# Sum02dean/GCN-STRING

Hardware: AMD Instinct MI355X
Metric: graphs/sec (fwd+bwd) on E.coli-sized batches; GCNConv SpMM achieved HBM GB/s (higher is better)
Workload: dtype f32; 1 GPU; config2: E. coli-shaped DisjointLoader batch, B=32 graphs per GPU, F=128, fp32, 2-layer GCNConv(relu)+GlobalSumPool+Dense softmax, CCE (from-logits form of tf.function), SGD; global_graphs=32, nodes_per_gpu=22576, nnz_per_gpu=333676, features=128, hidden=128, parallelism=dp1 (graphs sharded, RCCL all-reduce of 33284 fp32), hip_graph=False, gemm_precision=f32, cce=logits, activation_storage=fp32

## Files before the change

gcn-string_amd/csrc/fused.hip:

```cpp
#include "common.h"

namespace {

typedef float f32x4v __attribute__((ext_vector_type(4)));
typedef float f32x2 __attribute__((ext_vector_type(2)));
typedef __bf16 fbf16x8 __attribute__((ext_vector_type(8)));

constexpr int kFRows = 32;
constexpr int kFCap = 1024;

struct FusedArgs {
  const int32_t* rowptr; const int32_t* colidx; const float* vals;
  const float* x; int64_t ldx;
  int32_t n;
  const float* w; int32_t ldw;
  int32_t nc;
  const float* bias; int act;
  float* s; int64_t lds;
  float* wt_out;
  int w_t;
  float* out; int64_t ldo;
  const int32_t* node_graph; const int32_t* gp; const float* dp; int64_t lddp; int avg;
  const float* mask; int64_t ldmask;
  float* dz2; int64_t lddz2;
  float* colpart;
  float* tp_part; float* tp_cnt;
  const float* hd_part; const float* hd_cnt; int hd_rows; int hd_b;
  float* hd_psum; float* hd_csum;
  const float* hd_w; const float* hd_bias; const float* hd_y; int hd_c; float hd_denom; int hd_fl;
  int dbg;
};

__device__ __forceinline__ float4 fbuf4(__amdgpu_buffer_rsrc_t rs, unsigned off) {
  const f32x4v r = __builtin_bit_cast(f32x4v, __builtin_amdgcn_raw_buffer_load_b128(rs, off, 0, 0));
  return make_float4(r.x, r.y, r.z, r.w);
}
__device__ __forceinline__ float4 f4fma(float v, float4 h, float4 a) {
  const f32x2 w = {v, v};
  const f32x2 lo = __builtin_elementwise_fma(w, f32x2{h.x, h.y}, f32x2{a.x, a.y});
  const f32x2 hi = __builtin_elementwise_fma(w, f32x2{h.z, h.w}, f32x2{a.z, a.w});
  return make_float4(lo[0], lo[1], hi[0], hi[1]);
}
__device__ __forceinline__ float4 f4step(float4 a) {
  const f32x2 big = {0x1p127f, 0x1p127f};
  f32x2 lo = {a.x, a.y}, hi = {a.z, a.w}, t0, t1;
  asm("v_pk_mul_f32 %0, %1, %2" : "=v"(t0) : "v"(lo), "v"(big));
  asm("v_pk_mul_f32 %0, %1, %2" : "=v"(t1) : "v"(hi), "v"(big));
  asm("v_pk_mul_f32 %0, %1, %2 clamp" : "=v"(lo) : "v"(t0), "v"(big));
  asm("v_pk_mul_f32 %0, %1, %2 clamp" : "=v"(hi) : "v"(t1), "v"(big));
  return make_float4(lo[0], lo[1], hi[0], hi[1]);
}

__device__ __forceinline__ void f4acc(float4& a, const float4 q) { a.x += q.x; a.y += q.y; a.z += q.z; a.w += q.w; }

template <int LPR>
__device__ __forceinline__ float2 fused_head_dlogits(const FusedArgs& p, float4 pv, int rows, float4 w0, float4 w1, float b0,
                                                     float b1, float y0, float y1) {
  float sc = 1.0f;
  if (p.avg) { sc = 1.0f / (float)max(rows, 1); pv.x *= sc; pv.y *= sc; pv.z *= sc; pv.w *= sc; }
  const bool two = p.hd_c > 1;
  float z0 = fmaf(pv.w, w0.w, fmaf(pv.z, w0.z, fmaf(pv.y, w0.y, pv.x * w0.x)));
  float z1 = fmaf(pv.w, w1.w, fmaf(pv.z, w1.z, fmaf(pv.y, w1.y, pv.x * w1.x)));
#pragma unroll
  for (int off = 1; off < LPR; off <<= 1) { z0 += __shfl_xor(z0, off); z1 += __shfl_xor(z1, off); }
  z0 += b0;
  z1 = two ? z1 + b1 : -INFINITY;
  const float m = fmaxf(z0, z1), e0 = expf(z0 - m), e1 = expf(z1 - m), sum = e0 + e1;
  const float p0 = e0 / sum, p1 = e1 / sum;
  const bool k0 = p.hd_fl || (p0 > 1e-7f && p0 < 1.0f - 1e-7f), k1 = two && (p.hd_fl || (p1 > 1e-7f && p1 < 1.0f - 1e-7f));
  const float ymsum = (k0 ? y0 : 0.f) + (k1 ? y1 : 0.f);
  const float dl0 = (p0 * ymsum - (k0 ? y0 : 0.f)) / p.hd_denom, dl1 = two ? (p1 * ymsum - (k1 ? y1 : 0.f)) / p.hd_denom : 0.f;
  return make_float2(dl0 * sc, dl1 * sc);
}

template <int K, bool WEIGHTED, bool BWD, bool X3 = false>
__global__ __launch_bounds__(512, 6) void gcn_conv_fused_kernel(FusedArgs p) {
  constexpr int LPR = K / 4;
  constexpr int GW = 64 / LPR;
  constexpr int NG = 8 * GW;
  constexpr int RPG = NG >= kFRows ? 1 : kFRows / NG;
  constexpr int U = 4;
  static_assert(K == 32 || K == 64 || K == 128, "gather width");
  __shared__ __attribute__((aligned(16))) float tile[kFRows][K + 4];
  __shared__ __attribute__((aligned(8))) int2 s_ent[kFCap + 2 * U];
  __shared__ int32_t s_rp[kFRows + 1];
  __shared__ unsigned char s_mb[BWD ? kFRows * 32 : 1];
  __shared__ float2 s_dl[BWD ? kFRows : 1];
  __shared__ __attribute__((aligned(16))) float s_w3[BWD ? 2 : 1][K];
  __shared__ float s_b3[2];
  __shared__ int32_t s_g[BWD ? 1 : kFRows];
  static_assert(!BWD || sizeof(float) * kFRows * (K + 4) >= sizeof(float4) * 2 * 8 * 2 * LPR, "the head's wave partials alias the tile");
#ifdef GCNX_TUNING
  const int dbg = p.dbg;
#else
  constexpr int dbg = 0;
#endif

  const int tid = threadIdx.x, lane = tid & 63, wave = tid >> 6;
  const int ntiles = gridDim.x;
  const int t = gcnx_xcd_remap(blockIdx.x, ntiles);
  const int r0 = t * kFRows, nr = min(p.n - r0, kFRows);
  if (tid <= nr) s_rp[tid] = p.rowptr[r0 + tid];
  if (!BWD && p.tp_part && tid < kFRows)
    s_g[tid] = tid < nr ? min(max(p.node_graph[r0 + tid], 0), p.hd_b - 1) : -1;
  const int e0 = p.rowptr[r0], e1 = p.rowptr[r0 + nr];
  const int staged = min(e1 - e0, kFCap);
  const unsigned ld4 = (unsigned)p.ldx * 4u;
  for (int i = tid; i < staged + 2 * U; i += 512) {
    int2 en = make_int2(0, 0);
    if (i < staged) {
      en.x = (int)((unsigned)p.colidx[e0 + i] * ld4);
      en.y = WEIGHTED ? __float_as_int(p.vals[e0 + i]) : 0x3f800000;
    }
    s_ent[i] = en;
  }
  const int gid = wave * GW + lane / LPR, sub = lane % LPR;
  const __amdgpu_buffer_rsrc_t xr =
      __builtin_amdgcn_make_buffer_rsrc((void*)p.x, (short)0, (int)((unsigned)p.n * (unsigned)p.ldx * 4u), 0x00020000);
  int grow[RPG];
  if (BWD) {
#pragma unroll
    for (int j = 0; j < RPG; ++j) {
      const int r = gid + j * NG;
      grow[j] = (r < nr && gid < kFRows) ? p.node_graph[r0 + r] : -1;
    }
  }
  float4 mrow[2];
  const int mlanes = p.nc >> 2;
  if (BWD) {
#pragma unroll
    for (int q = 0; q < 2; ++q) {
      const int i = tid + 512 * q, row = i / mlanes, c4 = i - row * mlanes;
      mrow[q] = make_float4(0.f, 0.f, 0.f, 0.f);
      if (row < nr && !(dbg & 16)) mrow[q] = *reinterpret_cast<const float4*>(p.mask + (int64_t)(r0 + row) * p.ldmask + 4 * c4);
    }
  }
  float4 (*s_pv)[2][2][LPR] = reinterpret_cast<float4 (*)[2][2][LPR]>(&tile[0][0]);
  const int hsel = lane / LPR, hsub = lane % LPR;
  int g_first = 0;
  if (BWD && p.hd_part) {
    g_first = min(max(__builtin_amdgcn_readfirstlane(p.node_graph[r0]), 0), p.hd_b - 1);
    const int g_last = min(max(__builtin_amdgcn_readfirstlane(p.node_graph[r0 + nr - 1]), g_first), min(g_first + kFRows, p.hd_b) - 1);
    for (int i = tid; i < 2 * K; i += 512) {
      const int cls = i / K, k = i - cls * K;
      s_w3[cls][k] = cls < p.hd_c ? p.hd_w[(int64_t)k * p.hd_c + cls] : 0.f;
    }
    if (tid >= 2 * K && tid < 2 * K + 2) s_b3[tid - 2 * K] = (p.hd_bias && tid - 2 * K < p.hd_c) ? p.hd_bias[tid - 2 * K] : 0.f;
    const unsigned bytes = (unsigned)p.hd_rows * (unsigned)K * 4u;
    const __amdgpu_buffer_rsrc_t pr = __builtin_amdgcn_make_buffer_rsrc((void*)p.hd_part, (short)0, (int)bytes, 0x00020000);
    const __amdgpu_buffer_rsrc_t cr = __builtin_amdgcn_make_buffer_rsrc((void*)p.hd_cnt, (short)0, (int)bytes, 0x00020000);
    for (int gb = g_first; gb <= g_last; gb += 2) {
      if (gb > g_first) __syncthreads();
      int hd_g = 0, hd_n = 0;
      bool hd_desig = false;
      float y0 = 0.f, y1 = 0.f;
      if (hsel < 2) {
        hd_g = min(gb + hsel, g_last);
        const int hd_a = p.gp[hd_g];
        hd_n = p.gp[hd_g + 1] - hd_a;
        hd_desig = hd_a >= r0 && hd_n > 0;
        const int tlo = hd_a / kFRows, thi = hd_n > 0 ? (hd_a + hd_n - 1) / kFRows : tlo - 1;
        float4 ps = make_float4(0.f, 0.f, 0.f, 0.f), pc = ps;
        for (int tb = tlo + wave; __builtin_amdgcn_ballot_w64(tb <= thi) != 0; tb += 32) {
          float4 q[4], c[4];
#pragma unroll
          for (int u = 0; u < 4; ++u) {
            const int tt = tb + 8 * u;
            const unsigned off = tt <= thi ? ((unsigned)(tt + hd_g) * (unsigned)K + (unsigned)hsub * 4u) * 4u : 0xFFFFFFF0u;
            q[u] = fbuf4(pr, off);
            c[u] = fbuf4(cr, hd_desig ? off : 0xFFFFFFF0u);
          }
#pragma unroll
          for (int u = 0; u < 4; ++u) { f4acc(ps, q[u]); f4acc(pc, c[u]); }
        }
        s_pv[wave][0][hsel][hsub] = ps;
        s_pv[wave][1][hsel][hsub] = pc;
        if (wave == 0) {
          y0 = p.hd_y[(int64_t)hd_g * p.hd_c];
          y1 = p.hd_c > 1 ? p.hd_y[(int64_t)hd_g * p.hd_c + 1] : 0.f;
        }
      }
      __syncthreads();
      if (wave == 0 && hsel < 2) {
        float4 pv = make_float4(0.f, 0.f, 0.f, 0.f), pc = pv;
#pragma unroll 2
        for (int w = 0; w < 8; ++w) { f4acc(pv, s_pv[w][0][hsel][hsub]); f4acc(pc, s_pv[w][1][hsel][hsub]); }
        if (hd_desig) {
          *reinterpret_cast<float4*>(p.hd_psum + (int64_t)hd_g * K + hsub * 4) = pv;
          *reinterpret_cast<float4*>(p.hd_csum + (int64_t)hd_g * K + hsub * 4) = pc;
        }
        const float2 dl = fused_head_dlogits<LPR>(p, pv, hd_n, *reinterpret_cast<const float4*>(&s_w3[0][hsub * 4]),
                                                  *reinterpret_cast<const float4*>(&s_w3[1][hsub * 4]),
                                                  s_b3[0], s_b3[1], y0, y1);
        if (hsub == 0) s_dl[hd_g - g_first] = dl;
      }
    }
  } else {
    __syncthreads();
  }
  if (BWD) {
#pragma unroll
    for (int q = 0; q < 2; ++q) {
      const int i = tid + 512 * q, row = i / mlanes, c4 = i - row * mlanes;
      if (row < kFRows)
        s_mb[row * 32 + c4] = (unsigned char)((mrow[q].x > 0.f ? 1u : 0u) | (mrow[q].y > 0.f ? 2u : 0u) | (mrow[q].z > 0.f ? 4u : 0u) |
                                              (mrow[q].w > 0.f ? 8u : 0u));
    }
  }
  float4 acc[RPG];
  int ea[RPG], eb[RPG], ebf[RPG];
  int len = 0;
#pragma unroll
  for (int j = 0; j < RPG; ++j) {
    const int r = gid + j * NG;
    acc[j] = make_float4(0.f, 0.f, 0.f, 0.f);
    const bool live = r < nr && gid < kFRows;
    ea[j] = live ? s_rp[r] - e0 : 0;
    eb[j] = live ? s_rp[r + 1] - e0 : 0;
    ebf[j] = min(eb[j], kFCap);
    ea[j] = min(ea[j], kFCap);
    len = max(len, ebf[j] - ea[j]);
  }
  if (dbg & 1) len = 0;
  const unsigned sub16 = (unsigned)sub * 16u;
  for (int tt = 0; __builtin_amdgcn_ballot_w64(tt < len) != 0; tt += U) {
    float4 hv[RPG][U];
    float wv[RPG][U];
#pragma unroll
    for (int j = 0; j < RPG; ++j) {
      const int eb_ = min(ea[j] + tt, ebf[j]);
#pragma unroll
      for (int u = 0; u < U; ++u) {
        const int e = eb_ + u;
        const int2 en = s_ent[e];
        wv[j][u] = __int_as_float(en.y);
        hv[j][u] = fbuf4(xr, e < ebf[j] ? (unsigned)en.x + sub16 : 0xFFFFFFF0u);
      }
    }
    __builtin_amdgcn_sched_barrier(0);
#pragma unroll
    for (int j = 0; j < RPG; ++j)
#pragma unroll
      for (int u = 0; u < U; ++u) acc[j] = f4fma(wv[j][u], (BWD && !(dbg & 64)) ? f4step(hv[j][u]) : hv[j][u], acc[j]);
  }
  if (e1 - e0 > kFCap) {
#pragma unroll
    for (int j = 0; j < RPG; ++j)
      for (int e = max(eb[j] > 0 ? s_rp[gid + j * NG] - e0 : 0, kFCap); e < eb[j]; ++e) {
        const int c = p.colidx[e0 + e];
        const float v = WEIGHTED ? p.vals[e0 + e] : 1.0f;
        const float4 h = fbuf4(xr, (unsigned)c * ld4 + sub16);
        acc[j] = f4fma(v, BWD ? f4step(h) : h, acc[j]);
      }
  }
  float4 own[RPG], dscale[RPG];
  if (BWD) {
#pragma unroll
    for (int j = 0; j < RPG; ++j) {
      const int r = gid + j * NG;
      own[j] = dscale[j] = make_float4(0.f, 0.f, 0.f, 0.f);
      if (grow[j] >= 0 && (dbg & 32)) dscale[j] = make_float4(1.f, 1.f, 1.f, 1.f);
      if (grow[j] >= 0 && !(dbg & 32) && !p.hd_part) {
        float4 d = *reinterpret_cast<const float4*>(p.dp + (int64_t)grow[j] * p.lddp + sub * 4);
        if (p.avg) {
          const float sc = 1.0f / (float)(p.gp[grow[j] + 1] - p.gp[grow[j]]);
          d.x *= sc; d.y *= sc; d.z *= sc; d.w *= sc;
        }
        dscale[j] = d;
      }
      if (grow[j] >= 0 && p.dz2) own[j] = *reinterpret_cast<const float4*>(p.x + (int64_t)(r0 + r) * p.ldx + sub * 4);
    }
    if (p.hd_part && !(dbg & 32)) {
      __syncthreads();
      const float4 w0 = *reinterpret_cast<const float4*>(&s_w3[0][sub * 4]), w1 = *reinterpret_cast<const float4*>(&s_w3[1][sub * 4]);
#pragma unroll
      for (int j = 0; j < RPG; ++j) {
        if (grow[j] < 0) continue;
        const float2 dl = s_dl[(grow[j] - g_first) & (kFRows - 1)];
        dscale[j] = make_float4(fmaf(dl.y, w1.x, dl.x * w0.x), fmaf(dl.y, w1.y, dl.x * w0.y), fmaf(dl.y, w1.z, dl.x * w0.z),
                                fmaf(dl.y, w1.w, dl.x * w0.w));
      }
    }
  }
  const int c16 = lane & 15, kq = lane >> 4;
  const bool wave_on = 16 * wave < p.nc;
  auto k_of = [&](int e) { return X3 ? 32 * (e / 8) + 8 * kq + (e % 8) : 4 * e + kq; };
  float wreg[K / 4];
  if (wave_on && !(dbg & 4)) {
#pragma unroll
    for (int e = 0; e < K / 4; ++e)
      wreg[e] = (BWD && !p.w_t) ? p.w[(int64_t)(16 * wave + c16) * p.ldw + k_of(e)]
                                : p.w[(int64_t)k_of(e) * p.ldw + 16 * wave + c16];
    if (!BWD && p.wt_out && (int)blockIdx.x < K / 4) {
#pragma unroll
      for (int e = 0; e < K / 4; ++e)
        if (e % ntiles == (int)blockIdx.x) p.wt_out[(int64_t)(16 * wave + c16) * K + k_of(e)] = wreg[e];
    }
  }
  fbf16x8 wh[X3 ? K / 32 : 1], wl[X3 ? K / 32 : 1];
  if (X3) {
#pragma unroll
    for (int st = 0; st < K / 32; ++st)
#pragma unroll
      for (int j = 0; j < 8; ++j) {
        const float v = wave_on ? wreg[st * 8 + j] : 0.f;
        const __bf16 h = (__bf16)v;
        wh[st][j] = h;
        wl[st][j] = (__bf16)(v - (float)h);
      }
  }
  if (gid < kFRows) {
#pragma unroll
    for (int j = 0; j < RPG; ++j) {
      const int r = gid + j * NG;
      float4 a = acc[j];
      if (BWD) {
        a.x *= dscale[j].x; a.y *= dscale[j].y; a.z *= dscale[j].z; a.w *= dscale[j].w;
        if (p.dz2 && r < nr && !(dbg & 8)) {
          const float4 m = f4step(own[j]);
          *reinterpret_cast<float4*>(p.dz2 + (int64_t)(r0 + r) * p.lddz2 + sub * 4) =
              make_float4(m.x * dscale[j].x, m.y * dscale[j].y, m.z * dscale[j].z, m.w * dscale[j].w);
        }
      } else if (p.s && r < nr) {
        *reinterpret_cast<float4*>(p.s + (int64_t)(r0 + r) * p.lds + sub * 4) = a;
      }
      *reinterpret_cast<float4*>(&tile[r][sub * 4]) = a;
    }
  }
  __syncthreads();
  if (!wave_on) return;
  const int col = 16 * wave + c16;
  float mk[8];
  if (BWD) {
#pragma unroll
    for (int r = 0; r < 8; ++r) {
      const int row = 16 * (r >> 2) + 4 * kq + (r & 3);
      mk[r] = (dbg & 16) ? 1.f : (float)((s_mb[row * 32 + (col >> 2)] >> (col & 3)) & 1u);
    }
  }
  const float bcol = (!BWD && p.bias) ? p.bias[col] : 0.f;
  f32x4v c0 = {0.f, 0.f, 0.f, 0.f}, c1 = c0;
  if (X3) {
    if (!(dbg & 2))
#pragma unroll
    for (int st = 0; st < K / 32; ++st) {
#pragma unroll
      for (int hf = 0; hf < 2; ++hf) {
        const float* ap = &tile[16 * hf + c16][32 * st + 8 * kq];
        const float4 x0 = *reinterpret_cast<const float4*>(ap), x1 = *reinterpret_cast<const float4*>(ap + 4);
        const float xv[8] = {x0.x, x0.y, x0.z, x0.w, x1.x, x1.y, x1.z, x1.w};
        fbf16x8 ah, al;
#pragma unroll
        for (int j = 0; j < 8; ++j) {
          const __bf16 h = (__bf16)xv[j];
          ah[j] = h;
          al[j] = (__bf16)(xv[j] - (float)h);
        }
        f32x4v& cc = hf ? c1 : c0;
        cc = __builtin_amdgcn_mfma_f32_16x16x32_bf16(ah, wl[st], cc, 0, 0, 0);
        cc = __builtin_amdgcn_mfma_f32_16x16x32_bf16(al, wh[st], cc, 0, 0, 0);
        cc = __builtin_amdgcn_mfma_f32_16x16x32_bf16(ah, wh[st], cc, 0, 0, 0);
      }
    }
  } else if (!(dbg & 2)) {
#pragma unroll
    for (int kk = 0; kk < K / 4; ++kk) {
      const float a0 = tile[c16][4 * kk + kq];
      const float a1 = tile[16 + c16][4 * kk + kq];
      c0 = __builtin_amdgcn_mfma_f32_16x16x4f32(a0, wreg[kk], c0, 0, 0, 0);
      c1 = __builtin_amdgcn_mfma_f32_16x16x4f32(a1, wreg[kk], c1, 0, 0, 0);
    }
  }
  float cs = 0.f;
  float vout[8];
#pragma unroll
  for (int r = 0; r < 8; ++r) {
    const int row = 16 * (r >> 2) + 4 * kq + (r & 3);
    float v = r < 4 ? c0[r & 3] : c1[r & 3];
    if (BWD) v = mk[r] > 0.f ? v : 0.f;
    else { v += bcol; if (p.act == GCNX_ACT_RELU) v = fmaxf(v, 0.f); }
    if (row < nr) p.out[(int64_t)(r0 + row) * p.ldo + col] = v;
    cs += v;
    vout[r] = v;
  }
  if (!BWD && p.tp_part) {
    int gr[8];
#pragma unroll
    for (int r = 0; r < 8; ++r) gr[r] = s_g[16 * (r >> 2) + 4 * kq + (r & 3)];
    const int g_lo = s_g[0], g_hi = s_g[nr - 1];
    for (int g = g_lo; g <= g_hi; ++g) {
      float sm = 0.f, cn = 0.f;
#pragma unroll
      for (int r = 0; r < 8; ++r) {
        const bool mine = gr[r] == g;
        sm += mine ? vout[r] : 0.f;
        cn += (mine && vout[r] > 0.f) ? 1.f : 0.f;
      }
      sm += __shfl_xor(sm, 16); cn += __shfl_xor(cn, 16);
      sm += __shfl_xor(sm, 32); cn += __shfl_xor(cn, 32);
      if (lane < 16) {
        p.tp_part[(int64_t)(t + g) * p.nc + col] = sm;
        p.tp_cnt[(int64_t)(t + g) * p.nc + col] = cn;
      }
    }
  }
  if (BWD && p.colpart) {
    cs += __shfl_xor(cs, 16);
    cs += __shfl_xor(cs, 32);
    if (lane < 16) p.colpart[(int64_t)t * p.nc + col] = cs;
  }
}

template <bool BWD>
int launch_fused(gcnx_ctx* ctx, const FusedArgs& a_in, int k, bool x3) {
  FusedArgs a = a_in;
#ifdef GCNX_TUNING
  if (const char* e = getenv("GCNX_FUSED_DBG")) a.dbg = atoi(e);
#endif
  const int tiles = gcnx_cdiv(a.n, kFRows);
  int dyn = 0;
#ifdef GCNX_TUNING
  if (const char* e = getenv("GCNX_FUSED_LDS")) dyn = atoi(e);
#endif
#define GCNX_FUSED_LAUNCH(K_)                                                                                         \
  do {                                                                                                                \
    if (x3) {                                                                                                         \
      if (a.vals) hipLaunchKernelGGL((gcn_conv_fused_kernel<K_, true, BWD, true>), dim3(tiles), dim3(512), dyn, ctx->stream, a); \
      else hipLaunchKernelGGL((gcn_conv_fused_kernel<K_, false, BWD, true>), dim3(tiles), dim3(512), dyn, ctx->stream, a);      \
    } else if (a.vals) hipLaunchKernelGGL((gcn_conv_fused_kernel<K_, true, BWD>), dim3(tiles), dim3(512), dyn, ctx->stream, a); \
    else hipLaunchKernelGGL((gcn_conv_fused_kernel<K_, false, BWD>), dim3(tiles), dim3(512), dyn, ctx->stream, a);      \
  } while (0)
  if (k == 128) GCNX_FUSED_LAUNCH(128);
  else if (k == 64) GCNX_FUSED_LAUNCH(64);
  else GCNX_FUSED_LAUNCH(32);
#undef GCNX_FUSED_LAUNCH
  GCNX_LAUNCH_OK(ctx);
  return GCNX_OK;
}

inline bool fal16(const void* p) { return (reinterpret_cast<uintptr_t>(p) & 15) == 0; }
inline int64_t tiles_of(int64_t n) { return (n + kFRows - 1) / kFRows; }

bool fused_shape_ok(int64_t n, int32_t k, int32_t nc, int64_t ldx) {
  return n > 0 && (k == 32 || k == 64 || k == 128) && nc >= 16 && nc <= 128 && nc % 16 == 0 && ldx >= k && ldx % 4 == 0 &&
         (uint64_t)n * (uint64_t)ldx * 4u < 0xFFFFFFF0ull;
}

}

extern "C" {

int gcnx_gcn_conv_fused_ok(int64_t n, int32_t fi, int32_t fo, int64_t ldx) { return fused_shape_ok(n, fi, fo, ldx) ? 1 : 0; }

int gcnx_gcn_conv_fwd_pool(gcnx_ctx* ctx, const int32_t* rowptr, const int32_t* colidx, const float* vals, const float* x,
                           int64_t ldx, int32_t n, int32_t fi, const float* w, int32_t fo, const float* bias, int act, float* s,
                           int64_t lds, float* out, int64_t ldo, float* wt_out, int prec, const int32_t* node_graph, int32_t b,
                           float* tile_part, float* tile_cnt) {
  GCNX_CHECK_CTX(ctx);
  GCNX_RANGE(ctx, "GCNConv forward (one launch)");
  GCNX_REQUIRE(ctx, (!tile_part && !tile_cnt) || (tile_part && tile_cnt && node_graph && b > 0 && fal16(tile_part) && fal16(tile_cnt)),
               "gcnx_gcn_conv_fwd_pool: the pool's partial sums need node_graph, b > 0 and two 16-byte aligned outputs");
  GCNX_REQUIRE(ctx, n >= 0 && fi >= 0 && fo >= 0, "gcnx_gcn_conv_fwd: negative size");
  if (prec != GCNX_PREC_F32 && prec != GCNX_PREC_BF16X3)
    return gcnx_fail(ctx, GCNX_ERR_UNSUPPORTED, "gcnx_gcn_conv_fwd: precision %d (GCNX_PREC_F32 or GCNX_PREC_BF16X3 here)", prec);
  GCNX_REQUIRE(ctx, act == GCNX_ACT_NONE || act == GCNX_ACT_RELU, "gcnx_gcn_conv_fwd: activation %d not supported here", act);
  if (n == 0 || fo == 0) return GCNX_OK;
  if (!fused_shape_ok(n, fi, fo, ldx))
    return gcnx_fail(ctx, GCNX_ERR_UNSUPPORTED, "gcnx_gcn_conv_fwd: needs fi in {32, 64, 128}, fo a multiple of 16 up to 128 and "
                     "n * ldx * 4 < 2^32 (got n=%d fi=%d fo=%d): use gcnx_gemm + gcnx_spmm_csr", n, fi, fo);
  GCNX_REQUIRE(ctx, rowptr && colidx && x && w && out, "gcnx_gcn_conv_fwd: NULL pointer");
  GCNX_REQUIRE(ctx, ldo >= fo && ldo % 4 == 0 && fal16(x) && fal16(out) && (!bias || fal16(bias)) &&
                        (!s || (lds >= fi && lds % 4 == 0 && fal16(s))),
               "gcnx_gcn_conv_fwd: operands must be 16-byte aligned with leading dimensions in multiples of 4 floats");
  GCNX_REQUIRE(ctx, x != out && x != s, "gcnx_gcn_conv_fwd: in-place aggregation is not possible");
  FusedArgs a{};
  a.rowptr = rowptr; a.colidx = colidx; a.vals = vals; a.x = x; a.ldx = ldx; a.n = n; a.w = w; a.ldw = fo; a.nc = fo;
  a.bias = bias; a.act = act; a.s = s; a.lds = lds; a.out = out; a.ldo = ldo; a.wt_out = wt_out;
  a.node_graph = node_graph; a.tp_part = tile_part; a.tp_cnt = tile_cnt; a.hd_b = b;
  return launch_fused<false>(ctx, a, fi, prec == GCNX_PREC_BF16X3);
}

int gcnx_gcn_conv_fwd(gcnx_ctx* ctx, const int32_t* rowptr, const int32_t* colidx, const float* vals, const float* x,
                      int64_t ldx, int32_t n, int32_t fi, const float* w, int32_t fo, const float* bias, int act, float* s,
                      int64_t lds, float* out, int64_t ldo, float* wt_out, int prec) {
  return gcnx_gcn_conv_fwd_pool(ctx, rowptr, colidx, vals, x, ldx, n, fi, w, fo, bias, act, s, lds, out, ldo, wt_out, prec,
                                nullptr, 0, nullptr, nullptr);
}

int64_t gcnx_gcn_conv_bwd_scratch_floats(int64_t n, int32_t f1) { return n <= 0 || f1 <= 0 ? 0 : (int64_t)gcnx_cdiv(n, kFRows) * f1; }

int gcnx_gcn_conv_bwd_pool(gcnx_ctx* ctx, const int32_t* rowptr_t, const int32_t* colidx_t, const float* vals_t,
                           const float* y2, int64_t ldy2, const int32_t* node_graph, const int32_t* graph_ptr, int32_t b,
                           const float* dpooled, int64_t lddp, int mode, int32_t n, int32_t f2, const float* w2, int32_t f1,
                           int w2_transposed, const float* y1, int64_t ldy1, float* dz2, int64_t lddz2, float* dz1, int64_t lddz1, float* db1,
                           float* scratch, int64_t scratch_floats, gcnx_pending_reduce* pending, int prec,
                           const gcnx_head_args* head) {
  GCNX_CHECK_CTX(ctx);
  GCNX_RANGE(ctx, "GCNConv backward (one launch)");
  if (prec != GCNX_PREC_F32 && prec != GCNX_PREC_BF16X3)
    return gcnx_fail(ctx, GCNX_ERR_UNSUPPORTED, "gcnx_gcn_conv_bwd_pool: precision %d (GCNX_PREC_F32 or GCNX_PREC_BF16X3 here)", prec);
  if (pending) *pending = gcnx_pending_reduce{nullptr, 0, 0, nullptr, nullptr, 0, 0, nullptr};
  GCNX_REQUIRE(ctx, n >= 0 && f1 >= 0 && f2 >= 0 && b >= 0, "gcnx_gcn_conv_bwd_pool: negative size");
  GCNX_REQUIRE(ctx, mode == GCNX_POOL_SUM || mode == GCNX_POOL_AVG,
               "gcnx_gcn_conv_bwd_pool: pool mode %d has no folded form", mode);
  if (n == 0 || f1 == 0) {
    if (db1 && f1 > 0) GCNX_HIP(ctx, hipMemsetAsync(db1, 0, (size_t)f1 * 4, ctx->stream));
    return GCNX_OK;
  }
  if (!fused_shape_ok(n, f2, f1, ldy2))
    return gcnx_fail(ctx, GCNX_ERR_UNSUPPORTED, "gcnx_gcn_conv_bwd_pool: needs f2 in {32, 64, 128}, f1 a multiple of 16 up to 128 "
                     "and n * ldy2 * 4 < 2^32 (got n=%d f1=%d f2=%d)", n, f1, f2);
  GCNX_REQUIRE(ctx, b > 0 && rowptr_t && colidx_t && y2 && node_graph && graph_ptr && (dpooled || head) && w2 && y1 && dz1,
               "gcnx_gcn_conv_bwd_pool: NULL pointer");
  GCNX_REQUIRE(ctx, (head || (lddp >= f2 && lddp % 4 == 0 && fal16(dpooled))) && ldy1 >= f1 && ldy1 % 4 == 0 && lddz1 >= f1 &&
                        lddz1 % 4 == 0 && fal16(y2) && fal16(y1) && fal16(dz1) &&
                        (!dz2 || (fal16(dz2) && lddz2 >= f2 && lddz2 % 4 == 0)),
               "gcnx_gcn_conv_bwd_pool: operands must be 16-byte aligned with leading dimensions in multiples of 4 floats");
  if (head) {
    GCNX_REQUIRE(ctx, head->tile_part && head->tile_cnt && head->pool_sum && head->pool_cnt && head->w && head->y &&
                          head->tile_rows >= tiles_of(n) + b && head->tile_rows * f2 * 4 < 0xFFFFFFF0ll && head->b == b &&
                          head->h == f2 && head->c >= 1 && head->denom > 0.f && fal16(head->tile_part) && fal16(head->tile_cnt) &&
                          fal16(head->pool_sum) && fal16(head->pool_cnt) && head->pool_mode == mode &&
                          (head->cce_mode == GCNX_CCE_PROBS || head->cce_mode == GCNX_CCE_LOGITS),
                 "gcnx_gcn_conv_bwd_pool: inconsistent head arguments");
    if (head->c > 2)
      return gcnx_fail(ctx, GCNX_ERR_UNSUPPORTED, "gcnx_gcn_conv_bwd_pool: the in-kernel head serves one or two classes (got %d)", head->c);
  }
  GCNX_REQUIRE(ctx, y2 != dz1 && y2 != dz2 && y1 != dz1, "gcnx_gcn_conv_bwd_pool: outputs must not alias the saved activations");
  const int64_t tiles = gcnx_cdiv(n, kFRows);
  float* colpart = nullptr;
  bool defer = false;
  if (db1) {
    GCNX_REQUIRE(ctx, fal16(db1) && f1 % 4 == 0, "gcnx_gcn_conv_bwd_pool: db1 must be 16-byte aligned");
    defer = pending && scratch && fal16(scratch) && scratch_floats >= tiles * f1 && tiles <= 4096;
    if (defer) colpart = scratch;
    else {
      int rc = gcnx_ws_reserve(ctx, gcnx_colsum_partials_ws(tiles, f1));
      if (rc) return rc;
      colpart = (float*)ctx->ws;
    }
  }
  FusedArgs a{};
  a.rowptr = rowptr_t; a.colidx = colidx_t; a.vals = vals_t; a.x = y2; a.ldx = ldy2; a.n = n; a.w = w2; a.ldw = w2_transposed ? f1 : f2; a.w_t = w2_transposed ? 1 : 0; a.nc = f1;
  a.out = dz1; a.ldo = lddz1; a.node_graph = node_graph; a.gp = graph_ptr; a.dp = dpooled; a.lddp = lddp;
  a.avg = mode == GCNX_POOL_AVG ? 1 : 0; a.mask = y1; a.ldmask = ldy1; a.dz2 = dz2; a.lddz2 = lddz2; a.colpart = colpart;
  if (head) {
    a.hd_part = head->tile_part; a.hd_cnt = head->tile_cnt; a.hd_rows = (int)head->tile_rows; a.hd_b = head->b;
    a.hd_psum = head->pool_sum; a.hd_csum = head->pool_cnt; a.hd_w = head->w; a.hd_bias = head->bias; a.hd_y = head->y;
    a.hd_c = head->c; a.hd_denom = head->denom; a.hd_fl = head->cce_mode == GCNX_CCE_LOGITS ? 1 : 0;
  }
  int rc = launch_fused<true>(ctx, a, f2, prec == GCNX_PREC_BF16X3);
  if (rc) return rc;
  if (db1) {
    if (defer) *pending = gcnx_pending_reduce{colpart, tiles, f1, db1, nullptr, 0, 0, nullptr};
    else return gcnx_colsum_partials(ctx, tiles, f1, db1);
  }
  return GCNX_OK;
}

}
```

gcn-string_amd/gcnx/_lib.py:

```python
from __future__ import annotations

import ctypes as C
import os

_HERE = os.path.dirname(os.path.abspath(__file__))
LIB_PATH = os.environ.get("GCNX_LIB") or os.path.join(_HERE, "libgcnx.so")

OK = 0
ERR_UNSUPPORTED = 5
ACT_NONE, ACT_RELU, ACT_PRELU, ACT_PRELU_SHARED = 0, 1, 2, 3
POOL_SUM, POOL_AVG, POOL_MAX = 0, 1, 2
PREC_F32, PREC_BF16, PREC_BF16X3 = 0, 1, 2
NORM_SPEKTRAL, NORM_PYG = 0, 1
RED_SUM, RED_MAX = 0, 1
CCE_PROBS, CCE_LOGITS = 0, 1
CSR_SYMMETRIC, CSR_BLOCK_DIAGONAL, CSR_GRAPH_PTR_OK = 1, 2, 4
UNIQUE_ID_BYTES = 128

ACTS = {None: ACT_NONE, "linear": ACT_NONE, "none": ACT_NONE, "relu": ACT_RELU, "prelu": ACT_PRELU,
        "prelu_shared": ACT_PRELU_SHARED}
POOLS = {"sum": POOL_SUM, "avg": POOL_AVG, "mean": POOL_AVG, "max": POOL_MAX}
CCES = {"probs": CCE_PROBS, "eager": CCE_PROBS, "logits": CCE_LOGITS, "graph": CCE_LOGITS}
PRECS = {"f32": PREC_F32, "fp32": PREC_F32, "bf16": PREC_BF16, "bf16x3": PREC_BF16X3}

_vp, _i32, _i64, _f32, _sz = C.c_void_p, C.c_int32, C.c_int64, C.c_float, C.c_size_t
_int = C.c_int

SIGNATURES = {
    "gcnx_version": [],
    "gcnx_set_lr_source": [_vp, _vp],
    "gcnx_device_count": [C.POINTER(_int)],
    "gcnx_ctx_create": [_int, C.POINTER(_vp)],
    "gcnx_ctx_destroy": [_vp],
    "gcnx_last_error": [_vp],
    "gcnx_device_info": [_vp, C.c_char_p, _int, C.POINTER(_int), C.POINTER(_sz)],
    "gcnx_malloc": [_vp, _sz, C.POINTER(_vp)],
    "gcnx_free": [_vp, _vp],
    "gcnx_memset": [_vp, _vp, _int, _sz],
    "gcnx_h2d": [_vp, _vp, _vp, _sz],
    "gcnx_h2d_async": [_vp, _vp, _vp, _sz],
    "gcnx_d2h": [_vp, _vp, _vp, _sz],
    "gcnx_d2d": [_vp, _vp, _vp, _sz],
    "gcnx_sync": [_vp],
    "gcnx_side_begin": [_vp],
    "gcnx_side_end": [_vp],
    "gcnx_side_join": [_vp],
    "gcnx_event_create": [_vp, C.POINTER(_vp)],
    "gcnx_event_record": [_vp, _vp],
    "gcnx_event_elapsed_ms": [_vp, _vp, _vp, C.POINTER(_f32)],
    "gcnx_event_destroy": [_vp, _vp],
    "gcnx_capture_begin": [_vp],
    "gcnx_capture_end": [_vp, C.POINTER(_vp)],
    "gcnx_graph_launch": [_vp, _vp],
    "gcnx_graph_destroy": [_vp, _vp],
    "gcnx_coo_to_csr": [_vp, _vp, _vp, _i64, _i64, _vp, _vp],
    "gcnx_collate": [_vp, _vp, _i32, _vp, _vp, _vp, _vp, _vp, _i64, _i32, _vp, _i32, _vp, _vp, _vp, _vp, _i64, _vp, _vp, _vp],
    "gcnx_gcn_norm": [_vp, _vp, _vp, _vp, _i32, _int, _vp],
    "gcnx_set_tuning": [_vp, C.c_char_p, _int],
    "gcnx_csr_inspect": [_vp, _vp, _vp, _vp, _i32, _vp, _i32, C.POINTER(C.c_int)],
    "gcnx_csr_transpose": [_vp, _vp, _vp, _vp, _i32, _i32, _vp, _vp, _vp],
    "gcnx_csr_transpose_perm": [_vp, _vp, _vp, _i32, _i32, _vp, _vp, _vp],
    "gcnx_ecc_expand": [_vp, _vp, _vp, _vp, _vp, _i64, _i32, _vp, _i64, _i32, _vp, _i64, _i32, _i32, _int],
    "gcnx_ecc_bwd": [_vp, _vp, _vp, _vp, _i64, _i32, _vp, _i64, _vp, _i64, _vp, _i64, _i32, _vp, _i64, _vp, _i64, _i32, _i32],
    "gcnx_gemm": [_vp, _vp, _i64, _vp, _vp, _vp, _i64, _i64, _i32, _i32, _int, _int, _vp],
    "gcnx_spmm_plan_create": [_vp, _vp, _i32, C.POINTER(_vp)],
    "gcnx_spmm_plan_destroy": [_vp, _vp],
    "gcnx_spmm_plan_bind": [_vp, _vp, _vp, _i32],
    "gcnx_spmm_csr": [_vp, _vp, _vp, _vp, _vp, _i64, _vp, _vp, _i64, _i32, _i32, _int, _vp],
    "gcnx_segment_pool": [_vp, _vp, _vp, _i64, _vp, _i32, _i32, _int, _vp],
    "gcnx_softmax_cce": [_vp, _vp, _vp, _i32, _i32, _f32, _vp, _vp, _vp, _int],
    "gcnx_dense_softmax_cce": [_vp, _vp, _i64, _vp, _vp, _vp, _i32, _i32, _i32, _f32, _vp, _vp, _vp, _vp, _vp, _i64, _int],
    "gcnx_pool_dense_softmax_cce": [_vp, _vp, _vp, _i64, _int, _vp, _vp, _i64, _vp, _vp, _vp, _i32, _i32, _i32, _f32, _vp,
                                    _vp, _vp, _vp, _vp, _i64, _vp, _int],
    "gcnx_act_bias_grad": [_vp, _vp, _i64, _vp, _i64, _vp, _i64, _i64, _i32, _int, _vp, _vp, _vp],
    "gcnx_gemm_dw": [_vp, _vp, _i64, _vp, _i64, _vp, _i64, _i32, _i32, _int],
    "gcnx_wimage_elems": [_i32, _i32, _int, _int],
    "gcnx_wimage_prepare": [_vp, _i32, _vp],
    "gcnx_gemm_wimage": [_vp, _vp, _i64, _vp, _i32, _i32, _int, _vp, _vp, _i64, _i64, _int, _int, _vp, _vp],
    "gcnx_gemm_wimage_parts": [_vp, _i64],
    "gcnx_bn_finalize_parts": [_vp, _vp, _i32, _i32, _f32, _f32, _vp, _vp, _vp, _vp],
    "gcnx_gemm_dx": [_vp, _vp, _i64, _vp, _vp, _i64, _i64, _i32, _i32, _int, _int, _vp, _i64, _vp],
    "gcnx_gemm_relu_bits": [_vp, _vp, _i64, _vp, _vp, _vp, _i64, _i64, _i32, _i32, _int, _vp],
    "gcnx_gemm_dx_bits": [_vp, _vp, _i64, _vp, _vp, _i64, _i64, _i32, _i32, _int, _vp, _vp],
    "gcnx_spmm_csr_bf16out": [_vp, _vp, _vp, _vp, _vp, _i64, _vp, _vp, _i64, _i32, _i32, _int, _vp],
    "gcnx_spmm_csr_pool_bwd_bf16out": [_vp, _vp, _vp, _vp, _vp, _i64, _vp, _i32, _vp, _i64, _vp, _i64, _i32, _i32, _int, _vp, _vp],
    "gcnx_gemm_fwd_bf16": [_vp, _vp, _i64, _vp, _vp, _vp, _i64, _int, _i64, _i32, _i32, _int, _vp, _vp],
    "gcnx_gemm_dx_bf16": [_vp, _vp, _i64, _vp, _vp, _i64, _int, _i64, _i32, _i32, _vp, _vp, _vp],
    "gcnx_gemm_stream_images": [_vp, _i32, _vp],
    "gcnx_gemm_dw_bf16": [_vp, _vp, _i64, _vp, _i64, _vp, _i64, _i32, _i32],
    "gcnx_dense_bwd": [_vp, _vp, _i64, _vp, _i64, _vp, _i64, _i32, _i32, _int, _vp, _i64, _vp, _i64, _vp, _vp],
    "gcnx_segment_pool_bwd": [_vp, _vp, _vp, _vp, _i64, _i32, _i32, _i32, _int, _vp, _vp, _i64, _vp],
    "gcnx_spmm_csr_pool_bwd": [_vp, _vp, _vp, _vp, _vp, _i64, _vp, _i32, _vp, _i64, _vp, _i64, _i32, _i32, _int, _vp, _vp],
    "gcnx_spmm_csr_relu_bits": [_vp, _vp, _vp, _vp, _vp, _i64, _vp, _vp, _i64, _i32, _i32, _vp, _vp],
    "gcnx_pooled_dense_softmax_cce": [_vp, _vp, _int, _vp, _i64, _vp, _vp, _vp, _vp, _i32, _i32, _i32, _f32, _vp, _vp, _vp, _vp, _vp, _i64, _vp, _int],
    "gcnx_spmm_csr_relu_bits_pool": [_vp, _vp, _vp, _vp, _vp, _i64, _vp, _vp, _i64, _i32, _i32, _vp, _vp, _vp, _i32, _int, _vp, _i64, _vp],
    "gcnx_pool_bwd_colsum": [_vp, _vp, _i32, _vp, _i64, _vp, _i64, _i32, _int, _vp],
    "gcnx_bn_stats": [_vp, _vp, _i64, _i64, _i32, _vp, _vp],
    "gcnx_bn_finalize": [_vp, _vp, _f32, _i32, _f32, _f32, _vp, _vp, _vp, _vp, _vp],
    "gcnx_bn_moments": [_vp, _vp, _i64, _i64, _i32, _f32, _f32, _vp, _vp, _vp, _vp],
    "gcnx_bn_act": [_vp, _vp, _i64, _i64, _i32, _vp, _vp, _vp, _vp, _int, _vp, _vp, _i64],
    "gcnx_bn_act_bwd": [_vp, _vp, _i64, _vp, _i64, _i64, _i32, _vp, _vp, _vp, _vp, _int, _vp, _int, _vp, _i64, _vp, _vp, _vp,
                        _vp],
    "gcnx_bn_act_bwd_stats": [_vp, _vp, _i64, _vp, _i64, _i64, _i32, _vp, _vp, _vp, _vp, _int, _vp, _vp, _vp, _vp, _vp],
    "gcnx_bn_act_bwd_apply": [_vp, _vp, _i64, _vp, _i64, _i64, _i32, _vp, _vp, _vp, _vp, _int, _vp, _vp, _f32, _int, _vp, _i64],
    "gcnx_bn_act_pool": [_vp, _vp, _i32, _vp, _i64, _i32, _vp, _vp, _vp, _vp, _int, _vp, _int, _vp, _i64, _vp],
    "gcnx_bn_act_pool_bwd": [_vp, _vp, _i32, _vp, _i64, _vp, _vp, _i64, _i64, _i32, _vp, _vp, _vp, _vp, _int, _vp, _int, _vp, _i64,
                             _vp, _vp, _vp],
    "gcnx_bce_head_scratch_floats": [_i32, _i32],
    "gcnx_bn_prelu_bce_head": [_vp, _vp],
    "gcnx_bn_act_pool_bwd_stats": [_vp, _vp, _i32, _vp, _i64, _vp, _vp, _i64, _i32, _vp, _vp, _vp, _vp, _int, _vp, _int, _vp,
                                   _vp, _vp, _vp],
    "gcnx_bn_act_pool_bwd_apply": [_vp, _vp, _i32, _vp, _i64, _vp, _vp, _i64, _i32, _vp, _vp, _vp, _vp, _int, _vp, _int, _vp,
                                   _f32, _vp, _i64],
    "gcnx_bce_head_phase_scratch_floats": [_i32, _i32],
    "gcnx_bce_head_phase_red_floats": [_i32],
    "gcnx_bce_head_phase": [_vp, _vp, _i32, _f32, _vp],
    "gcnx_sgd": [_vp, _vp, _vp, _i64, _f32],
    "gcnx_dropout": [_vp, _vp, _i64, _i64, _i32, _f32, C.c_uint32, C.c_uint32, _vp, _vp, _i64],
    "gcnx_counter_add": [_vp, _vp, C.c_uint32],
    "gcnx_add": [_vp, _vp, _i64, _vp, _i64, _vp, _i64, _i64, _i32],
    "gcnx_spmm_csr_minmax": [_vp, _vp, _vp, _vp, _i64, _vp, _i64, _vp, _i64, _i32, _i32, _int],
    "gcnx_spmm_csr_minmax_bwd": [_vp, _vp, _vp, _vp, _i64, _vp, _i64, _vp, _i64, _vp, _i64, _vp, _i64, _i32, _i32],
    "gcnx_spmm_csr_prod": [_vp, _vp, _vp, _vp, _i64, _vp, _i64, _vp, _i64, _i32, _i32],
    "gcnx_spmm_csr_prod_bwd": [_vp, _vp, _vp, _vp, _i64, _vp, _i64, _vp, _i64, _vp, _i64, _vp, _i64, _i32, _i32],
    "gcnx_gemm_dw_sgd": [_vp, _vp, _i64, _vp, _i64, _vp, _i64, _i32, _i32, _int, _vp, _vp, _i64, _f32, _vp],
    "gcnx_dense_bwd_scratch_floats": [_vp, _i64, _i32, _i32],
    "gcnx_dense_bwd_deferred": [_vp, _vp, _i64, _vp, _i64, _vp, _i64, _i32, _i32, _int, _vp, _i64, _vp, _i64, _vp, _vp, _vp,
                                _i64, _vp],
    "gcnx_gcn_conv_fused_ok": [_i64, _i32, _i32, _i64],
    "gcnx_gcn_conv_fwd": [_vp, _vp, _vp, _vp, _vp, _i64, _i32, _i32, _vp, _i32, _vp, _int, _vp, _i64, _vp, _i64, _vp, _int],
    "gcnx_gcn_conv_bwd_scratch_floats": [_i64, _i32],
    "gcnx_gcn_conv_bwd_pool": [_vp, _vp, _vp, _vp, _vp, _i64, _vp, _vp, _i32, _vp, _i64, _int, _i32, _i32, _vp, _i32, _int, _vp, _i64,
                               _vp, _i64, _vp, _i64, _vp, _vp, _i64, _vp, _int, _vp],
    "gcnx_spmm_csr_bf16": [_vp, _vp, _vp, _vp, _vp, _i64, _vp, _vp, _i64, _i32, _i32, _int],
    "gcnx_f32_to_bf16": [_vp, _vp, _vp, _i64],
    "gcnx_bf16_to_f32": [_vp, _vp, _vp, _i64],
    "gcnx_gcn_conv_fwd_pool": [_vp, _vp, _vp, _vp, _vp, _i64, _i32, _i32, _vp, _i32, _vp, _int, _vp, _i64, _vp, _i64, _vp, _int,
                               _vp, _i32, _vp, _vp],
    "gcnx_gemm_dw2": [_vp, _vp, _i64, _vp, _i64, _vp, _i32, _i32, _vp, _i64, _vp, _i64, _vp, _i32, _i32, _i64, _int, _vp, _vp,
                      _i64, _f32, _vp, _vp],
    "gcnx_comm_unique_id": [C.c_char_p],
    "gcnx_comm_init_rank": [_vp, C.c_char_p, _int, _int, C.POINTER(_vp)],
    "gcnx_comm_destroy": [_vp],
    "gcnx_allreduce_f32": [_vp, _vp, _vp, _i64, _int],
}
_RESTYPE = {"gcnx_last_error": C.c_char_p, "gcnx_dense_bwd_scratch_floats": C.c_int64, "gcnx_bce_head_scratch_floats": C.c_int64,
            "gcnx_bce_head_phase_scratch_floats": C.c_int64, "gcnx_bce_head_phase_red_floats": C.c_int64,
            "gcnx_gcn_conv_bwd_scratch_floats": C.c_int64, "gcnx_wimage_elems": C.c_int64, "gcnx_gemm_wimage_parts": C.c_int64}


class WimageJob(C.Structure):
    _fields_ = [("w", C.c_void_p), ("img", C.c_void_p), ("fi", C.c_int32), ("fo", C.c_int32), ("transpose", C.c_int32),
                ("prec", C.c_int32)]


class StreamImageJob(C.Structure):
    _fields_ = [("w", C.c_void_p), ("fi", C.c_int32), ("fo", C.c_int32), ("transpose", C.c_int32), ("img", C.c_void_p)]


STREAM_IMAGE_BYTES = 131072


class PendingReduce(C.Structure):
    _fields_ = [("colpart", C.c_void_p), ("crows", C.c_int64), ("cf", C.c_int32), ("cout", C.c_void_p),
                ("slabs", C.c_void_p), ("total", C.c_int64), ("nsplit", C.c_int32), ("out", C.c_void_p)]

class HeadArgs(C.Structure):
    _fields_ = [("tile_part", C.c_void_p), ("tile_cnt", C.c_void_p), ("tile_rows", C.c_int64),
                ("pool_sum", C.c_void_p), ("pool_cnt", C.c_void_p),
                ("graph_ptr", C.c_void_p), ("b", C.c_int32), ("h", C.c_int32), ("pool_mode", C.c_int),
                ("w", C.c_void_p), ("bias", C.c_void_p), ("y", C.c_void_p), ("c", C.c_int32), ("denom", C.c_float), ("cce_mode", C.c_int),
                ("probs", C.c_void_p), ("loss_acc", C.c_void_p), ("dw", C.c_void_p), ("db", C.c_void_p), ("db_relu", C.c_void_p),
                ("pooled", C.c_void_p), ("dpooled", C.c_void_p)]


class BceHeadArgs(C.Structure):
    _fields_ = [("pooled", C.c_void_p), ("ldp", C.c_int64), ("b", C.c_int32), ("h", C.c_int32),
                ("w3", C.c_void_p), ("b3", C.c_void_p), ("gamma3", C.c_void_p), ("beta3", C.c_void_p), ("alpha3", C.c_void_p),
                ("w4", C.c_void_p), ("b4", C.c_void_p), ("gamma4", C.c_void_p), ("beta4", C.c_void_p), ("alpha4", C.c_void_p),
                ("eps", C.c_float), ("denom", C.c_float),
                ("y", C.c_void_p), ("y_stride", C.c_int32), ("y_col", C.c_int32), ("grads", C.c_int32),
                ("out", C.c_void_p), ("probs", C.c_void_p), ("loss_acc", C.c_void_p),
                ("dpooled", C.c_void_p), ("lddp", C.c_int64),
                ("dw3", C.c_void_p), ("db3", C.c_void_p), ("dgamma3", C.c_void_p), ("dbeta3", C.c_void_p), ("dalpha3", C.c_void_p),
                ("dw4", C.c_void_p), ("db4", C.c_void_p), ("dgamma4", C.c_void_p), ("dbeta4", C.c_void_p), ("dalpha4", C.c_void_p),
                ("scratch", C.c_void_p), ("scratch_floats", C.c_int64)]


_lib = None


class GcnxError(RuntimeError):
    def __init__(self, code, message):
        super().__init__(f"libgcnx error {code}: {message}")
        self.code = code


def load():
    global _lib
    if _lib is not None:
        return _lib
    if not os.path.exists(LIB_PATH):
        raise GcnxError(-1, f"{LIB_PATH} not found: build it with `python __graft_entry__.py` "
                            "(make -C gcn-string_amd/csrc); there is no CPU fallback")
    lib = C.CDLL(LIB_PATH)
    for name, argtypes in SIGNATURES.items():
        try:
            fn = getattr(lib, name)
        except AttributeError:
            if os.environ.get("GCNX_LIB") and name in ("gcnx_spmm_plan_bind",):
                setattr(lib, name, lambda *a: OK)
                continue
            raise
        fn.argtypes = argtypes
        fn.restype = _RESTYPE.get(name, _int)
    _lib = lib
    return lib


def last_error(ctx_handle=None):
    msg = load().gcnx_last_error(ctx_handle)
    return msg.decode() if msg else ""


def check(rc, ctx_handle=None):
    if rc != OK:
        raise GcnxError(rc, last_error(ctx_handle))
```

gcn-string_amd/gcnx/device.py:

```python
from __future__ import annotations

import ctypes as C
import os

import numpy as np

from . import _lib as L


class _Side:
    def __init__(self, ctx):
        self.ctx = ctx

    def __enter__(self):
        self.ctx._ck(self.ctx.lib.gcnx_side_begin(self.ctx.h))
        return self

    def __exit__(self, *exc):
        self.ctx._ck(self.ctx.lib.gcnx_side_end(self.ctx.h))
        return False


_DEFAULT_CTX = None

# ... 302 lines not shown
                         self.symmetric, self.max_block_rows)

    def transpose(self):
        if self.symmetric:
            return self
        if self._t is None:
            ctx = self.ctx
            rp = ctx.empty(self.n + 1, np.int32)
            ci = ctx.empty(max(self.nnz, 1), np.int32)
            v = ctx.empty(max(self.nnz, 1), np.float32) if self.vals is not None else None
            ctx._ck(ctx.lib.gcnx_csr_transpose(ctx.h, self.rowptr.ptr, self.colidx.ptr,
                                               self.vals.ptr if self.vals is not None else None, self.n, self.nnz,
                                               rp.ptr, ci.ptr, v.ptr if v is not None else None))
            self._t = DeviceCSR(ctx, self.n, self.nnz, rp, ci, v, self.block_ptr, self.n_blocks, False, self.max_block_rows)
        return self._t

    def transpose_perm(self):
        if getattr(self, "_tperm", None) is None:
            ctx = self.ctx
            rp, ci, pm = ctx.empty(self.n + 1, np.int32), ctx.empty(max(self.nnz, 1), np.int32), ctx.empty(max(self.nnz, 1), np.int32)
            ctx._ck(ctx.lib.gcnx_csr_transpose_perm(ctx.h, self.rowptr.ptr, self.colidx.ptr, self.n, self.nnz, rp.ptr, ci.ptr, pm.ptr))
            self._tperm = (rp, ci, pm)
        return self._tperm

    def row_mean(self):
        if getattr(self, "_row_mean", None) is None:
            deg = np.diff(self.rowptr.numpy()).astype(np.int64)
            vals = np.repeat(np.where(deg > 0, 1.0 / np.maximum(deg, 1), 0.0).astype(np.float32), deg)
            self._row_mean = DeviceCSR(self.ctx, self.n, self.nnz, self.rowptr, self.colidx, self.ctx.to_device(vals), self.block_ptr,
                                       self.n_blocks, False, self.max_block_rows)
        return self._row_mean

    def unweighted(self):
        if self.vals is None:
            return self
        if getattr(self, "_unweighted", None) is None:
            self._unweighted = DeviceCSR(self.ctx, self.n, self.nnz, self.rowptr, self.colidx, None, self.block_ptr, self.n_blocks,
                                         self.symmetric, self.max_block_rows)
        return self._unweighted


def _max_block(graph_ptr):
    gp = np.asarray(graph_ptr) if graph_ptr is not None else None
    return int(np.diff(gp).max()) if gp is not None and gp.size > 1 else 0


class _Plan:
    def __init__(self, ctx, h):
        self.ctx, self.h = ctx, h
        self.bound = set()

    def __del__(self):
        try:
            if self.h and self.ctx._live:
                self.ctx.lib.gcnx_spmm_plan_destroy(self.ctx.h, self.h)
        except Exception:
            pass


class Segments:

    def __init__(self, ctx, graph_ptr_host):
        gp = np.asarray(graph_ptr_host, dtype=np.int32)
        self.ctx, self.n_graphs, self.n = ctx, len(gp) - 1, int(gp[-1])
        self.host = gp
        self.dev = ctx.to_device(gp, np.int32)

    @classmethod
    def from_device(cls, ctx, dev, graph_ptr_host):
        self = cls.__new__(cls)
        gp = np.asarray(graph_ptr_host, dtype=np.int32)
        self.ctx, self.n_graphs, self.n, self.host, self.dev = ctx, len(gp) - 1, int(gp[-1]), gp, dev
        return self

    @property
    def has_empty(self):
        if getattr(self, "_has_empty", None) is None:
            self._has_empty = bool(self.n_graphs) and bool(np.any(np.diff(self.host) <= 0))
        return self._has_empty

    @property
    def ids(self):
        if getattr(self, "_ids", None) is None:
            self._ids = self.ctx.to_device(np.repeat(np.arange(self.n_graphs, dtype=np.int32), np.diff(self.host)), np.int32)
        return self._ids

    @classmethod
    def from_ids(cls, ctx, i, n_graphs=None):
        i = np.asarray(i)
        b = int(i.max()) + 1 if n_graphs is None and i.size else (n_graphs or 0)
        if i.size and np.any(np.diff(i) < 0):
            raise ValueError("segment ids must be sorted (DisjointLoader order)")
        gp = np.zeros(b + 1, dtype=np.int64)
        np.cumsum(np.bincount(i, minlength=b), out=gp[1:])
        return cls(ctx, gp)



def _p(a):
    if a is None:
        return None
    if a.dtype != np.float32 and a.dtype != np.int32:
        raise TypeError(f"libgcnx operands are float32/int32, got {a.dtype}")
    return a.ptr


def gemm(ctx, x, w, bias, out, act=None, prec="f32", alpha=None):
    n, fi = x.shape
    fo = w.shape[1]
    assert w.shape[0] == fi and out.shape == (n, fo)
    ctx._ck(ctx.lib.gcnx_gemm(ctx.h, _p(x), x.ld, _p(w), _p(bias), _p(out), out.ld, n, fi, fo, L.PRECS[prec],
                              L.ACTS[act], _p(alpha)))
    return out


def gemm_relu_bits(ctx, x, w, bias, out, bits, prec="bf16"):
    n, fi = x.shape
    fo = w.shape[1]
    assert w.shape[0] == fi and out.shape == (n, fo) and bits.nbytes >= n * 64
    rc = ctx.lib.gcnx_gemm_relu_bits(ctx.h, _p(x), x.ld, _p(w), _p(bias), _p(out), out.ld, n, fi, fo, L.PRECS[prec], bits.ptr)
    if rc == L.ERR_UNSUPPORTED:
        return False
    ctx._ck(rc)
    return True


def _is16(a):
    return a.dtype == np.uint16


def spmm_bf16out(ctx, a, h, bias, out16, act=None):
    n, f = h.shape
    assert a.n == n and out16.shape == (n, f) and _is16(out16)
    rc = ctx.lib.gcnx_spmm_csr_bf16out(ctx.h, a.rowptr.ptr, a.colidx.ptr, _p(a.vals), _p(h), h.ld, _p(bias), out16.ptr, out16.ld,
                                       n, f, L.ACTS[act], a.plan)
    if rc == L.ERR_UNSUPPORTED:
        return False
    ctx._ck(rc)
    return True


def spmm_pool_bwd_bf16out(ctx, at, y, seg, dpooled, out16, mode="sum", y_bits=None):
    n, f = y.shape
    assert at.n == n and out16.shape == (n, f) and _is16(out16) and dpooled.shape == (seg.n_graphs, f)
    if y_bits is None or at.n_blocks != seg.n_graphs:
        return False
    rc = ctx.lib.gcnx_spmm_csr_pool_bwd_bf16out(ctx.h, at.rowptr.ptr, at.colidx.ptr, _p(at.vals), _p(y), y.ld, seg.dev.ptr,
                                                seg.n_graphs, _p(dpooled), dpooled.ld, out16.ptr, out16.ld, n, f, L.POOLS[mode],
                                                at.plan, _p(y_bits))
    if rc == L.ERR_UNSUPPORTED:
        return False
    ctx._ck(rc)
    return True


def stream_images(ctx, jobs, storage):
    assert storage.dtype == np.uint16 and storage.size >= len(jobs) * (L.STREAM_IMAGE_BYTES // 2) and len(jobs) <= 4
    arr = (L.StreamImageJob * len(jobs))()
    ptrs = []
    for i, (w, tr) in enumerate(jobs):
        assert w.shape == (256, 256) and w.contiguous
        ptrs.append(storage.ptr + i * L.STREAM_IMAGE_BYTES)
        arr[i] = L.StreamImageJob(w.ptr, 256, 256, 1 if tr else 0, ptrs[-1])
    ctx._ck(ctx.lib.gcnx_gemm_stream_images(ctx.h, len(jobs), C.cast(arr, C.c_void_p)))
    return ptrs


def gemm_fwd_bf16(ctx, x16, w, bias, out, act=None, bits=None, wimg=None):
    n, fi = x16.shape
    fo = w.shape[1]
    assert _is16(x16) and w.shape[0] == fi and out.shape == (n, fo) and (bits is None or bits.nbytes >= n * 64)
    rc = ctx.lib.gcnx_gemm_fwd_bf16(ctx.h, x16.ptr, x16.ld, _p(w), _p(bias), out.ptr, out.ld, int(_is16(out)), n, fi, fo, L.ACTS[act],
                                    _p(bits), wimg)
    if rc == L.ERR_UNSUPPORTED:
        return False
    ctx._ck(rc)
    return True


def gemm_dx_bf16(ctx, dh16, w, dx, mask_bits=None, db=None, wimg=None):
    n, fo = dh16.shape
    fi = w.shape[0]
    assert _is16(dh16) and w.shape[1] == fo and dx.shape == (n, fi)
    rc = ctx.lib.gcnx_gemm_dx_bf16(ctx.h, dh16.ptr, dh16.ld, _p(w), dx.ptr, dx.ld, int(_is16(dx)), n, fi, fo, _p(mask_bits), _p(db), wimg)
    if rc == L.ERR_UNSUPPORTED:
        return False
    ctx._ck(rc)
    return True


def gemm_dw_bf16(ctx, x16, dh16, dw):
    n, fi = x16.shape
    fo = dh16.shape[1]
    assert _is16(x16) and _is16(dh16) and dh16.shape[0] == n and dw.shape == (fi, fo)
    rc = ctx.lib.gcnx_gemm_dw_bf16(ctx.h, x16.ptr, x16.ld, dh16.ptr, dh16.ld, _p(dw), n, fi, fo)
    if rc == L.ERR_UNSUPPORTED:
        return False
    ctx._ck(rc)
    return True


def spmm(ctx, a, h, bias, out, act=None):
    n, f = h.shape
    assert a.n == n and out.shape == (n, f)
    ctx._ck(ctx.lib.gcnx_spmm_csr(ctx.h, a.rowptr.ptr, a.colidx.ptr, _p(a.vals), _p(h), h.ld, _p(bias), _p(out),
                                  out.ld, n, f, L.ACTS[act], a.plan))
    return out


def ecc_expand(ctx, a, u, x, scat, root=False, identity_perm=False):
    n, f = x.shape
    sp = u.shape[1] if u is not None else 0
    assert a.n == n and scat.shape[0] == n and scat.shape[1] >= (sp + 1 + bool(root)) * f and (u is None or u.shape[0] == a.nnz)
    rp, ci, pm = (a.rowptr, a.colidx, None) if identity_perm else a.transpose_perm()
    ctx._ck(ctx.lib.gcnx_ecc_expand(ctx.h, rp.ptr, ci.ptr, pm.ptr if pm is not None else None, _p(u), u.ld if u is not None else 0, sp,
                                    _p(x), x.ld, f, _p(scat), scat.ld, n, a.nnz, 1 if root else 0))
    return scat


def ecc_bwd(ctx, a, u, x, dscat, dx_root=None, dx=None, du=None):
    n, f = a.n, (x.shape[1] if x is not None else dx.shape[1])
    sp = u.shape[1] if u is not None else 0
    assert dscat.shape == (n, (sp + 1) * f) and (du is None or du.shape == (a.nnz, sp))
    ctx._ck(ctx.lib.gcnx_ecc_bwd(ctx.h, a.rowptr.ptr, a.colidx.ptr, _p(u), u.ld if u is not None else 0, sp, _p(x),
                                 x.ld if x is not None else 0, _p(dscat), dscat.ld, _p(dx_root), dx_root.ld if dx_root is not None else 0,
                                 f, _p(dx), dx.ld if dx is not None else 0, _p(du), du.ld if du is not None else 0, n, a.nnz))
    return dx, du


def segment_pool(ctx, seg, x, pooled, mode="sum", argmax=None):
    ctx._ck(ctx.lib.gcnx_segment_pool(ctx.h, seg.dev.ptr, _p(x), x.ld, _p(pooled), seg.n_graphs, x.shape[1],
                                      L.POOLS[mode], _p(argmax)))
    return pooled


def segment_pool_bwd(ctx, seg, dpooled, dx, mode="sum", argmax=None, y=None, db=None):
    n, f = dx.shape
    ctx._ck(ctx.lib.gcnx_segment_pool_bwd(ctx.h, seg.dev.ptr, _p(dpooled), _p(dx), dx.ld, n, seg.n_graphs, f,
                                          L.POOLS[mode], _p(argmax), _p(y), y.ld if y is not None else 0, _p(db)))
    return dx


def pool_dense_softmax_cce(ctx, seg, x, pooled, w, bias, y, probs, loss_acc=None, denom=None, dw=None, db=None,
                           dpooled=None, mode="sum", argmax=None, db_relu=None, cce="logits"):
    b, h = pooled.shape
    c = w.shape[1]
    assert x.shape[1] == h and seg.n_graphs == b
    ctx._ck(ctx.lib.gcnx_pool_dense_softmax_cce(ctx.h, seg.dev.ptr, _p(x), x.ld, L.POOLS[mode], _p(argmax), _p(pooled),
                                                pooled.ld, _p(w), _p(bias), _p(y), b, h, c,
                                                float(denom if denom else max(b, 1)), _p(probs), _p(loss_acc), _p(dw),
                                                _p(db), _p(dpooled), dpooled.ld if dpooled is not None else 0,
                                                _p(db_relu), L.CCES[cce]))
    return probs


def pooled_dense_softmax_cce(ctx, seg, pooled, cnt, w, bias, y, probs, loss_acc=None, denom=None, dw=None, db=None, dpooled=None,
                             mode="sum", db_relu=None, cce="logits"):
    b, h = pooled.shape
    c = w.shape[1]
    assert seg.n_graphs == b and (cnt is None or cnt.shape == (b, h))
    ctx._ck(ctx.lib.gcnx_pooled_dense_softmax_cce(ctx.h, seg.dev.ptr, L.POOLS[mode], _p(pooled), pooled.ld, _p(cnt), _p(w), _p(bias), _p(y),
                                                  b, h, c, float(denom if denom else max(b, 1)), _p(probs), _p(loss_acc), _p(dw), _p(db),
                                                  _p(dpooled), dpooled.ld if dpooled is not None else 0, _p(db_relu), L.CCES[cce]))
    return probs


def spmm_relu_bits(ctx, a, h, bias, out, bits):
    n, f = h.shape
    assert a.n == n and out.shape == (n, f) and bits.size >= (f // 32) * n
    rc = ctx.lib.gcnx_spmm_csr_relu_bits(ctx.h, a.rowptr.ptr, a.colidx.ptr, _p(a.vals), _p(h), h.ld, _p(bias), _p(out), out.ld,
                                         n, f, a.plan, _p(bits))
    if rc == L.ERR_UNSUPPORTED:
        return False
    ctx._ck(rc)
    return True


def spmm_pool_bwd(ctx, at, y, seg, dpooled, out, mode="sum", y_bits=None):
    n, f = y.shape
    assert at.n == n and out.shape == (n, f) and dpooled.shape == (seg.n_graphs, f)
    ctx._ck(ctx.lib.gcnx_spmm_csr_pool_bwd(ctx.h, at.rowptr.ptr, at.colidx.ptr, _p(at.vals), _p(y), y.ld, seg.dev.ptr,
                                           seg.n_graphs, _p(dpooled), dpooled.ld, _p(out), out.ld, n, f, L.POOLS[mode],
                                           at.plan if at.n_blocks == seg.n_graphs else None, _p(y_bits)))
    return out


def spmm_relu_bits_pool(ctx, a, h, bias, out, bits, seg, pooled, cnt, mode="sum"):
    n, f = h.shape
    assert a.n == n and out.shape == (n, f) and pooled.shape == (seg.n_graphs, f) and cnt.shape == (seg.n_graphs, f)
    if a.plan is None or a.n_blocks != seg.n_graphs:
        return False
    rc = ctx.lib.gcnx_spmm_csr_relu_bits_pool(ctx.h, a.rowptr.ptr, a.colidx.ptr, _p(a.vals), _p(h), h.ld, _p(bias), _p(out), out.ld, n, f,
                                              a.plan, bits.ptr, seg.dev.ptr, seg.n_graphs, L.POOLS[mode], _p(pooled), pooled.ld, _p(cnt))
    if rc == L.ERR_UNSUPPORTED:
        return False
    ctx._ck(rc)
    return True


def gcn_conv_fused_ok(ctx, n, fi, fo, ldx=None):
    return bool(ctx.lib.gcnx_gcn_conv_fused_ok(int(n), int(fi), int(fo), int(ldx if ldx is not None else fi)))


def gcn_conv_fwd(ctx, a, x, w, bias, out, act="relu", s=None, wt=None, prec="f32", pool=None):
    n, fi = x.shape
    fo = w.shape[1]
    assert a.n == n and w.shape[0] == fi and w.contiguous and out.shape == (n, fo) and (s is None or s.shape == (n, fi))
    if pool is None:
        ctx._ck(ctx.lib.gcnx_gcn_conv_fwd(ctx.h, a.rowptr.ptr, a.colidx.ptr, _p(a.vals), _p(x), x.ld, n, fi, _p(w), fo, _p(bias),
                                          L.ACTS[act], _p(s), s.ld if s is not None else 0, _p(out), out.ld, _p(wt), L.PRECS[prec]))
        return out
    seg, tp, tc = pool
    assert tp.shape == tc.shape == (pool_tile_rows(n, seg.n_graphs), fo) and tp.contiguous and tc.contiguous
    ctx._ck(ctx.lib.gcnx_gcn_conv_fwd_pool(ctx.h, a.rowptr.ptr, a.colidx.ptr, _p(a.vals), _p(x), x.ld, n, fi, _p(w), fo, _p(bias),
                                           L.ACTS[act], _p(s), s.ld if s is not None else 0, _p(out), out.ld, _p(wt), L.PRECS[prec],
                                           seg.ids.ptr, seg.n_graphs, _p(tp), _p(tc)))
    return out


def to_bf16(ctx, x):
    assert x.contiguous and x.dtype == np.float32
    y = ctx.empty(x.shape, np.uint16)
    ctx._ck(ctx.lib.gcnx_f32_to_bf16(ctx.h, x.ptr, y.ptr, x.size))
    return y


def to_bf16_into(ctx, x, y16):
    assert x.contiguous and y16.contiguous and x.dtype == np.float32 and y16.dtype == np.uint16 and x.shape == y16.shape
    ctx._ck(ctx.lib.gcnx_f32_to_bf16(ctx.h, x.ptr, y16.ptr, x.size))
    return y16


def from_bf16(ctx, x):
    assert x.contiguous and x.dtype == np.uint16
    y = ctx.empty(x.shape, np.float32)
    ctx._ck(ctx.lib.gcnx_bf16_to_f32(ctx.h, x.ptr, y.ptr, x.size))
    return y


def spmm_bf16(ctx, a, h, bias, out, act=None):
    n, f = h.shape
    assert a.n == n and out.shape == (n, f) and h.dtype == np.uint16 and out.dtype == np.uint16
    ctx._ck(ctx.lib.gcnx_spmm_csr_bf16(ctx.h, a.rowptr.ptr, a.colidx.ptr, _p(a.vals), h.ptr, h.ld, _p(bias), out.ptr, out.ld, n, f,
                                       L.ACTS[act]))
    return out


def pool_tile_rows(n, b):
    return (int(n) + 31) // 32 + int(b)


def head_args(seg, tile_part, tile_cnt, pool_sum, pool_cnt, w, bias, y, denom, probs, loss_acc, dw, db, db_relu, pooled, dpooled,
              mode="sum", cce="logits"):
    b, h = seg.n_graphs, w.shape[0]
    c = w.shape[1]
    assert w.contiguous and pooled.contiguous and dpooled.contiguous and pooled.shape == (b, h) and dpooled.shape == (b, h)
    assert tile_part.shape[1] == h and tile_cnt.shape == tile_part.shape and tile_part.contiguous and tile_cnt.contiguous
    assert pool_sum.shape == (b, h) and pool_cnt.shape == (b, h) and pool_sum.contiguous and pool_cnt.contiguous
    return L.HeadArgs(_p(tile_part), _p(tile_cnt), tile_part.shape[0], _p(pool_sum), _p(pool_cnt), seg.dev.ptr, b, h, L.POOLS[mode],
                      _p(w), _p(bias), _p(y), c, float(denom), L.CCES[cce], _p(probs), _p(loss_acc), _p(dw), _p(db), _p(db_relu),
                      _p(pooled), _p(dpooled))


def gcn_conv_bwd_pool(ctx, at, y2, seg, dpooled, w2, y1, dz2, dz1, db1=None, mode="sum", scratch=None, w2t=None, prec="f32",
                      head=None):
    n, f2 = y2.shape
    f1 = w2.shape[0]
    assert at.n == n and w2.shape == (f1, f2) and w2.contiguous and y1.shape == (n, f1) and dz1.shape == (n, f1)
    assert (head is not None or dpooled.shape == (seg.n_graphs, f2)) and (dz2 is None or dz2.shape == (n, f2))
    pend = L.PendingReduce()
    ctx._ck(ctx.lib.gcnx_gcn_conv_bwd_pool(ctx.h, at.rowptr.ptr, at.colidx.ptr, _p(at.vals), _p(y2), y2.ld, seg.ids.ptr,
                                           seg.dev.ptr, seg.n_graphs, _p(dpooled), dpooled.ld if dpooled is not None else 0,
                                           L.POOLS[mode], n, f2,
                                           _p(w2t if w2t is not None else w2), f1, 1 if w2t is not None else 0, _p(y1), y1.ld, _p(dz2), dz2.ld if dz2 is not None else 0, _p(dz1), dz1.ld, _p(db1),
                                           _p(scratch), scratch.size if scratch is not None else 0,
                                           C.byref(pend) if scratch is not None else None, L.PRECS[prec],
                                           C.byref(head) if head is not None else None))
    return pend


def gcn_conv_bwd_scratch_floats(ctx, n, f1):
    return int(ctx.lib.gcnx_gcn_conv_bwd_scratch_floats(int(n), int(f1)))


def gemm_dw2(ctx, xa, dha, dwa, xb, dhb, dwb, prec="f32", params=None, grads=None, lr=0.0, pending=None, leaf=None):
    n, fia = xa.shape
    foa = dha.shape[1]
    fib, fob = xb.shape[1], dhb.shape[1]
    assert xb.shape[0] == n and dha.shape[0] == n and dhb.shape[0] == n and dwa.shape == (fia, foa) and dwb.shape == (fib, fob)
    ctx._ck(ctx.lib.gcnx_gemm_dw2(ctx.h, _p(xa), xa.ld, _p(dha), dha.ld, _p(dwa), fia, foa, _p(xb), xb.ld, _p(dhb), dhb.ld,
                                  _p(dwb), fib, fob, n, L.PRECS[prec], _p(params), _p(grads),
                                  params.size if params is not None else (grads.size if grads is not None else 0), float(lr),
                                  C.byref(pending) if pending is not None else None, C.byref(leaf) if leaf is not None else None))


def pool_bwd_colsum(ctx, seg, dpooled, y, db, mode="sum"):
    ctx._ck(ctx.lib.gcnx_pool_bwd_colsum(ctx.h, seg.dev.ptr, seg.n_graphs, _p(dpooled), dpooled.ld, _p(y), y.ld,
                                         y.shape[1], L.POOLS[mode], _p(db)))
    return db


def softmax_cce(ctx, logits, y, probs, loss_acc, dlogits=None, denom=None, cce="logits"):
    b, c = logits.shape
    ctx._ck(ctx.lib.gcnx_softmax_cce(ctx.h, _p(logits), _p(y), b, c, float(denom if denom else b), _p(probs),
                                     _p(loss_acc), _p(dlogits), L.CCES[cce]))


def dense_softmax_cce(ctx, pooled, w, bias, y, probs, loss_acc=None, denom=None, dw=None, db=None, dpooled=None,
                      cce="logits"):
    b, h = pooled.shape
    c = w.shape[1]
    ctx._ck(ctx.lib.gcnx_dense_softmax_cce(ctx.h, _p(pooled), pooled.ld, _p(w), _p(bias), _p(y), b, h, c,
                                           float(denom if denom else max(b, 1)), _p(probs), _p(loss_acc), _p(dw), _p(db),
                                           _p(dpooled), dpooled.ld if dpooled is not None else 0, L.CCES[cce]))
    return probs


def act_bias_grad(ctx, dy, y, dz, act, db=None, alpha=None, dalpha=None):
    n, f = dy.shape
    ctx._ck(ctx.lib.gcnx_act_bias_grad(ctx.h, _p(dy), dy.ld, _p(y), y.ld if y is not None else 0, _p(dz), dz.ld, n,
                                       f, L.ACTS[act], _p(alpha), _p(db), _p(dalpha)))
    return dz


def gemm_dw(ctx, x, dh, dw, prec="f32"):
    n, fi = x.shape
    fo = dh.shape[1]
    assert dh.shape[0] == n and dw.shape == (fi, fo) and dw.contiguous
    ctx._ck(ctx.lib.gcnx_gemm_dw(ctx.h, _p(x), x.ld, _p(dh), dh.ld, _p(dw), n, fi, fo, L.PRECS[prec]))
    return dw


def gemm_dx(ctx, dh, w, dx, prec="f32", accumulate=False, y_mask=None, db=None, mask_bits=None):
    n, fo = dh.shape
    fi = w.shape[0]
    assert w.shape[1] == fo and dx.shape == (n, fi)
    if mask_bits is not None:
        assert not accumulate
        ctx._ck(ctx.lib.gcnx_gemm_dx_bits(ctx.h, _p(dh), dh.ld, _p(w), _p(dx), dx.ld, n, fi, fo, L.PRECS[prec], mask_bits.ptr, _p(db)))
        return dx
    ctx._ck(ctx.lib.gcnx_gemm_dx(ctx.h, _p(dh), dh.ld, _p(w), _p(dx), dx.ld, n, fi, fo, L.PRECS[prec],
                                 1 if accumulate else 0, _p(y_mask), y_mask.ld if y_mask is not None else 0, _p(db)))
    return dx


def gemm_dw_sgd(ctx, x, dh, dw, params, grads, lr, prec="f32", pending=None):
    n, fi = x.shape
    fo = dh.shape[1]
    assert dh.shape[0] == n and dw.shape == (fi, fo) and dw.contiguous and params.size == grads.size
    ctx._ck(ctx.lib.gcnx_gemm_dw_sgd(ctx.h, _p(x), x.ld, _p(dh), dh.ld, _p(dw), n, fi, fo, L.PRECS[prec], _p(params),
                                     _p(grads), params.size, float(lr), C.byref(pending) if pending is not None else None))


def dense_bwd_scratch_floats(ctx, n, fi, fo):
    return int(ctx.lib.gcnx_dense_bwd_scratch_floats(ctx.h, n, fi, fo))


def dense_bwd_deferred(ctx, x, dh, w, dx, dw, scratch, prec="f32", y_mask=None, db_prev=None):
    n, fo = dh.shape
    fi = w.shape[0]
    assert w.shape[1] == fo and dx.shape == (n, fi) and x.shape == (n, fi) and dw.shape == (fi, fo) and w.contiguous
    pend = L.PendingReduce()
    ctx._ck(ctx.lib.gcnx_dense_bwd_deferred(ctx.h, _p(x), x.ld, _p(dh), dh.ld, _p(w), n, fi, fo, L.PRECS[prec], _p(dx), dx.ld,
                                            _p(y_mask), y_mask.ld if y_mask is not None else 0, _p(db_prev), _p(dw),
                                            _p(scratch), scratch.size if scratch is not None else 0, C.byref(pend)))
    return pend


def dense_bwd(ctx, x, dh, w, dx, dw, prec="f32", y_mask=None, db_prev=None):
    n, fo = dh.shape
    fi = w.shape[0]
    assert w.shape[1] == fo and dx.shape == (n, fi) and x.shape == (n, fi) and dw.shape == (fi, fo) and w.contiguous
    ctx._ck(ctx.lib.gcnx_dense_bwd(ctx.h, _p(x), x.ld, _p(dh), dh.ld, _p(w), n, fi, fo, L.PRECS[prec], _p(dx), dx.ld,
                                   _p(y_mask), y_mask.ld if y_mask is not None else 0, _p(db_prev), _p(dw)))
    return dx


def sgd(ctx, params, grads, lr):
    ctx._ck(ctx.lib.gcnx_sgd(ctx.h, _p(params), _p(grads), params.size, float(lr)))


BN_EPS, BN_MOMENTUM = 1e-3, 0.99


def bn_stats(ctx, z, sums, shift=None):
    n, f = z.shape
    ctx._ck(ctx.lib.gcnx_bn_stats(ctx.h, _p(z), z.ld, n, f, _p(shift), _p(sums)))


def bn_finalize(ctx, sums, count, mean, inv, moving_mean=None, moving_var=None, shift=None, momentum=BN_MOMENTUM, eps=BN_EPS):
    ctx._ck(ctx.lib.gcnx_bn_finalize(ctx.h, _p(sums), float(count), mean.size, momentum, eps, _p(shift), _p(mean), _p(inv),
                                     _p(moving_mean), _p(moving_var)))


def bn_moments(ctx, z, sums, mean, inv, moving_mean=None, moving_var=None, momentum=BN_MOMENTUM, eps=BN_EPS):
    n, f = z.shape
    ctx._ck(ctx.lib.gcnx_bn_moments(ctx.h, _p(z), z.ld, n, f, momentum, eps, _p(mean), _p(inv), _p(moving_mean),
                                    _p(moving_var)))


def wimage_elems(ctx, fi, fo, transpose, prec):
    return int(ctx.lib.gcnx_wimage_elems(int(fi), int(fo), 1 if transpose else 0, L.PRECS[prec]))


def wimage_prepare(ctx, jobs):
    if not jobs:
        return
    arr = (L.WimageJob * len(jobs))()
    for k, (w, img, transpose, prec) in enumerate(jobs):
        fi, fo = w.shape
        arr[k] = L.WimageJob(w.ptr, img.ptr, fi, fo, 1 if transpose else 0, L.PRECS[prec])
    ctx._ck(ctx.lib.gcnx_wimage_prepare(ctx.h, len(jobs), C.cast(arr, C.c_void_p)))


def gemm_wimage(ctx, x, img, fi, fo, out, transpose=False, bias=None, prec="bf16x3", accumulate=False, bn_parts=None):
    n = x.shape[0]
    nparts = C.c_int32(0)
    rc = ctx.lib.gcnx_gemm_wimage(ctx.h, _p(x), x.ld, img.ptr, int(fi), int(fo), 1 if transpose else 0, _p(bias), _p(out), out.ld, n,
                                  L.PRECS[prec], 1 if accumulate else 0, _p(bn_parts), C.byref(nparts) if bn_parts is not None else None)
    if rc == L.ERR_UNSUPPORTED:
        return None
    ctx._ck(rc)
    return nparts.value


def gemm_wimage_parts(ctx, n):
    return int(ctx.lib.gcnx_gemm_wimage_parts(ctx.h, int(n)))


def bn_finalize_parts(ctx, parts, nparts, mean, inv, moving_mean=None, moving_var=None, momentum=BN_MOMENTUM, eps=BN_EPS):
    ctx._ck(ctx.lib.gcnx_bn_finalize_parts(ctx.h, _p(parts), int(nparts), mean.size, momentum, eps, _p(mean), _p(inv),
                                           _p(moving_mean), _p(moving_var)))


def bn_act(ctx, z, mean, inv, gamma, beta, y, act=None, alpha=None):
    n, f = z.shape
    ctx._ck(ctx.lib.gcnx_bn_act(ctx.h, _p(z), z.ld, n, f, _p(mean), _p(inv), _p(gamma), _p(beta), L.ACTS[act], _p(alpha),
                                _p(y), y.ld))
    return y


def bn_act_bwd(ctx, dy, z, mean, inv, gamma, beta, dz, scratch, act=None, alpha=None, training=True, dgamma=None, dbeta=None,
               dalpha=None):
    n, f = z.shape
    ctx._ck(ctx.lib.gcnx_bn_act_bwd(ctx.h, _p(dy), dy.ld, _p(z), z.ld, n, f, _p(mean), _p(inv), _p(gamma), _p(beta),
                                    L.ACTS[act], _p(alpha), 1 if training else 0, _p(dz), dz.ld, _p(dgamma), _p(dbeta),
                                    _p(dalpha), _p(scratch)))
    return dz


def bn_act_bwd_stats(ctx, dy, z, mean, inv, gamma, beta, scratch, act=None, alpha=None, dgamma=None, dbeta=None, dalpha=None):
    n, f = z.shape
    ctx._ck(ctx.lib.gcnx_bn_act_bwd_stats(ctx.h, _p(dy), dy.ld, _p(z), z.ld, n, f, _p(mean), _p(inv), _p(gamma), _p(beta),
                                          L.ACTS[act], _p(alpha), _p(scratch), _p(dgamma), _p(dbeta), _p(dalpha)))


def bn_act_bwd_apply(ctx, dy, z, mean, inv, gamma, beta, sums, count, dz, act=None, alpha=None, training=True):
    n, f = z.shape
    ctx._ck(ctx.lib.gcnx_bn_act_bwd_apply(ctx.h, _p(dy), dy.ld, _p(z), z.ld, n, f, _p(mean), _p(inv), _p(gamma), _p(beta),
                                          L.ACTS[act], _p(alpha), _p(sums), float(count), 1 if training else 0, _p(dz), dz.ld))
    return dz


def dropout(ctx, x, rate, seed, stream_id, step=None, out=None):
    out = x if out is None else out
    n, f = x.shape
    assert out.shape == (n, f)
    ctx._ck(ctx.lib.gcnx_dropout(ctx.h, _p(x), x.ld, n, f, float(rate), int(seed) & 0xFFFFFFFF, int(stream_id) & 0xFFFFFFFF, _p(step),
                                 _p(out), out.ld))
    return out


def counter_add(ctx, counter, inc=1):
    ctx._ck(ctx.lib.gcnx_counter_add(ctx.h, _p(counter), int(inc)))


def add(ctx, a, b, out):
    n, f = a.shape
    assert b.shape == (n, f) and out.shape == (n, f)
    ctx._ck(ctx.lib.gcnx_add(ctx.h, _p(a), a.ld, _p(b), b.ld, _p(out), out.ld, n, f))
    return out


def spmm_minmax(ctx, a, h, out, cnt=None, mode="max"):
    n, f = h.shape
    assert a.n == n and out.shape == (n, f) and mode in ("max", "min", "prod")
    if mode == "prod":
        ctx._ck(ctx.lib.gcnx_spmm_csr_prod(ctx.h, a.rowptr.ptr, a.colidx.ptr, _p(h), h.ld, _p(out), out.ld, _p(cnt),
                                           cnt.ld if cnt is not None else 0, n, f))
        return out
    ctx._ck(ctx.lib.gcnx_spmm_csr_minmax(ctx.h, a.rowptr.ptr, a.colidx.ptr, _p(h), h.ld, _p(out), out.ld, _p(cnt),
                                         cnt.ld if cnt is not None else 0, n, f, 1 if mode == "min" else 0))
    return out


def spmm_minmax_bwd(ctx, at, h, out, cnt, dy, dh, mode="max"):
    n, f = h.shape
    assert at.n == n and out.shape == (n, f) and cnt.shape == (n, f) and dy.shape == (n, f) and dh.shape == (n, f)
    if mode == "prod":
        ctx._ck(ctx.lib.gcnx_spmm_csr_prod_bwd(ctx.h, at.rowptr.ptr, at.colidx.ptr, _p(h), h.ld, _p(out), out.ld, _p(cnt), cnt.ld,
                                               _p(dy), dy.ld, _p(dh), dh.ld, n, f))
        return dh
    ctx._ck(ctx.lib.gcnx_spmm_csr_minmax_bwd(ctx.h, at.rowptr.ptr, at.colidx.ptr, _p(h), h.ld, _p(out), out.ld, _p(cnt), cnt.ld,
                                             _p(dy), dy.ld, _p(dh), dh.ld, n, f))
    return dh


TORCH_BN_EPS = 1e-5


def bn_act_pool(ctx, seg, z, mean, inv, gamma, beta, pooled, argmax, act="prelu_shared", alpha=None, mode="max"):
    n, f = z.shape
    ctx._ck(ctx.lib.gcnx_bn_act_pool(ctx.h, seg.dev.ptr, seg.n_graphs, _p(z), z.ld, f, _p(mean), _p(inv), _p(gamma), _p(beta),
                                     L.ACTS[act], _p(alpha), L.POOLS[mode], _p(pooled), pooled.ld, argmax.ptr))
    return pooled


def bn_act_pool_bwd(ctx, seg, dpooled, argmax, z, mean, inv, gamma, beta, dz, act="prelu_shared", alpha=None, dgamma=None,
                    dbeta=None, dalpha=None, mode="max"):
    n, f = z.shape
    ctx._ck(ctx.lib.gcnx_bn_act_pool_bwd(ctx.h, seg.dev.ptr, seg.n_graphs, _p(dpooled), dpooled.ld, argmax.ptr, _p(z), z.ld, n, f,
                                         _p(mean), _p(inv), _p(gamma), _p(beta), L.ACTS[act], _p(alpha), L.POOLS[mode], _p(dz),
                                         dz.ld, _p(dgamma), _p(dbeta), _p(dalpha)))
    return dz


def bn_act_pool_bwd_stats(ctx, seg, dpooled, argmax, z, mean, inv, gamma, beta, sums, act="prelu_shared", alpha=None, dgamma=None,
                          dbeta=None, dalpha=None, mode="max"):
    f = z.shape[1]
    ctx._ck(ctx.lib.gcnx_bn_act_pool_bwd_stats(ctx.h, seg.dev.ptr, seg.n_graphs, _p(dpooled), dpooled.ld, argmax.ptr, _p(z), z.ld, f,
                                               _p(mean), _p(inv), _p(gamma), _p(beta), L.ACTS[act], _p(alpha), L.POOLS[mode],
                                               _p(sums), _p(dgamma), _p(dbeta), _p(dalpha)))


def bn_act_pool_bwd_apply(ctx, seg, dpooled, argmax, z, mean, inv, gamma, beta, sums, count, dz, act="prelu_shared", alpha=None,
                          mode="max"):
    f = z.shape[1]
    ctx._ck(ctx.lib.gcnx_bn_act_pool_bwd_apply(ctx.h, seg.dev.ptr, seg.n_graphs, _p(dpooled), dpooled.ld, argmax.ptr, _p(z), z.ld, f,
                                               _p(mean), _p(inv), _p(gamma), _p(beta), L.ACTS[act], _p(alpha), L.POOLS[mode],
                                               _p(sums), float(count), _p(dz), dz.ld))
    return dz


def bce_head_scratch_floats(ctx, b, h):
    return int(ctx.lib.gcnx_bce_head_scratch_floats(int(b), int(h)))


def bce_head_args(pooled, p, scratch, out, probs, y=None, loss_acc=None, denom=None, g=None, dpooled=None, eps=TORCH_BN_EPS):
    b, h = pooled.shape
    if y is not None:
        stride = y.shape[1] if len(y.shape) == 2 else 1
        col = 1 if stride == 2 else 0
        if stride > 2:
            raise ValueError(f"binary labels are [B], [B, 1] or one-hot [B, 2], got {tuple(y.shape)}")
    else:
        stride, col = 1, 0
    gp = (lambda k: _p(g[k])) if g is not None else (lambda k: None)
    return L.BceHeadArgs(
        _p(pooled), pooled.ld, b, h, _p(p["w3"]), _p(p["b3"]), _p(p["g3"]), _p(p["be3"]), _p(p["a3"]),
        _p(p["w4"]), _p(p["b4"]), _p(p["g4"]), _p(p["be4"]), _p(p["a4"]), float(eps), float(denom if denom else b),
        _p(y), stride, col, 1 if g is not None else 0, _p(out), _p(probs), _p(loss_acc),
        _p(dpooled), dpooled.ld if dpooled is not None else 0,
        gp("w3"), gp("b3"), gp("g3"), gp("be3"), gp("a3"), gp("w4"), gp("b4"), gp("g4"), gp("be4"), gp("a4"),
        _p(scratch), scratch.size)


def bn_prelu_bce_head(ctx, args):
    ctx._ck(ctx.lib.gcnx_bn_prelu_bce_head(ctx.h, C.byref(args)))


def bce_head_phase_scratch_floats(ctx, b, h):
    return int(ctx.lib.gcnx_bce_head_phase_scratch_floats(int(b), int(h)))


# ... 11 lines not shown
```

gcn-string_amd/gcnx/models.py:

```python
from __future__ import annotations

import os

import numpy as np

from . import device as D
from .layers import glorot_uniform
from .loader import SparseTensor


class DeviceBatch:

    _next_uid = 0

    def __init__(self, ctx, x, a, seg, y=None, e=None):
        self.ctx, self.x, self.a, self.seg, self.y, self.e = ctx, x, a, seg, y, e
        DeviceBatch._next_uid += 1
        self.uid = DeviceBatch._next_uid
        self.n, self.f = x.shape
        self.n_graphs = seg.n_graphs

    @classmethod
    def from_host(cls, ctx, inputs, y=None, normalize=None, weighted=True, symmetric=None):
        e = None
        if len(inputs) == 4:
            x, a, e, i = inputs
        else:
            x, a, i = inputs
        n = x.shape[0]
        seg = i if isinstance(i, D.Segments) else D.Segments.from_ids(ctx, i)
        dx = ctx.to_device(x, np.float32)
        if isinstance(a, D.DeviceCSR):
            csr = a
        else:
            if not isinstance(a, SparseTensor):
                from .loader import sp_matrix_to_sp_tensor
                a = sp_matrix_to_sp_tensor(a)
            csr = D.DeviceCSR.from_coo(ctx, a.indices, a.values, n, graph_ptr=seg.host, symmetric=symmetric,
                                       weighted=weighted)
        if normalize:
            csr = csr.gcn_norm(normalize)
        dy = ctx.to_device(y, np.float32) if y is not None else None
        de = None
        if e is not None:
            e = np.asarray(e)
            if e.ndim != 2 or e.shape[0] != csr.nnz:
                raise ValueError(f"edge features e have shape {e.shape}: expected one row per stored entry of the adjacency "
                                 f"({csr.nnz} entries, row-major; from_networkx(use_edge_data='entries') builds them so)")
            de = ctx.to_device(e, np.float32) if e.shape[0] else ctx.empty((0, e.shape[1]))
        return cls(ctx, dx, csr, seg, dy, de)


def _without_e(inputs):
    return (inputs[0], inputs[1], inputs[-1]) if len(inputs) == 4 else inputs


class _Capacity:

    def __init__(self, ctx):
        self.ctx, self.store = ctx, {}

    def view(self, name, rows, width, dtype=np.float32, zero=False):
        need = int(rows) * int(width)
        cur = self.store.get(name)
        if cur is None or cur.size < need or cur.dtype != np.dtype(dtype):
            size = max(need, int(1.25 * cur.size) if cur is not None else 0, 1)
            cur = (self.ctx.zeros if zero else self.ctx.empty)(size, dtype)
            self.store[name] = cur
        return D.DeviceArray._view(cur, 0, (int(rows), int(width)))


class _GraphRunner:

    use_graph = True

    def _bind(self, batch):
        if getattr(self, "_bound_uid", None) != batch.uid:
            for tag in [t for t in self._graphs if t[0] != "sgd"]:
                g = self._graphs.pop(tag)
                if not isinstance(g, str):
                    g.destroy()
            self._bound_uid = batch.uid

    def _run(self, tag, fn):
        if not self.use_graph:
            fn()
            return
        st = self._graphs.get(tag)
        if st is None:
            fn()
            self._graphs[tag] = "warm"
        elif st == "warm":
            self._graphs[tag] = self.ctx.capture(fn)
            self._graphs[tag].launch()
        else:
            st.launch()

    _MRING = 1024

    def stash_metrics(self, n_graphs):
        if getattr(self, "_mring", None) is None:
            self._mring, self._mcount, self._mdone = self.ctx.zeros(2 * self._MRING), [], []
        if len(self._mcount) == self._MRING:
            self._mdone.extend(self._read_ring())
        k = len(self._mcount)
        self.ctx._ck(self.ctx.lib.gcnx_d2d(self.ctx.h, self._mring.ptr + 8 * k, self.loss_acc.ptr, 8))
        self._mcount.append(float(n_graphs))

    def _read_ring(self):
        la = self._mring.numpy().reshape(-1, 2)[:len(self._mcount)]
        out = [(float(l), float(h) / n) for (l, h), n in zip(la, self._mcount)]
        self._mcount = []
        return out

    def collect_metrics(self):
        if getattr(self, "_mring", None) is None:
            return []
        out = self._mdone + self._read_ring()
        self._mdone = []
        return out

    lr_on_device = os.environ.get("GCNX_LR_DEVICE", "1") != "0"

    def _lr_key(self, lr):
        if not self.lr_on_device or lr is None:
            self.ctx.set_lr_source(None)
            return lr
        if getattr(self, "_lr_buf", None) is None:
            self._lr_buf, self._lr_val = self.ctx.zeros(1), None
        self.ctx.set_lr_source(self._lr_buf)
        if self._lr_val != float(lr):
            self._lr_buf.copy_from_host(np.asarray([lr], np.float32), wait=False)
            self._lr_val = float(lr)
        return "dev"

    def _drop_graphs(self):
        for g in getattr(self, "_graphs", {}).values():
            if not isinstance(g, str):
                g.destroy()
        self._graphs = {}


class GCN2(_GraphRunner):
    PARAM_ORDER = ("w1", "b1", "w2", "b2", "w3", "b3")

    @D.with_default_context
    def __init__(self, ctx, n_labels=2, hidden=None, pool="sum", prec="f32", seed=0, comm=None, use_graph="auto",
                 cce_train="logits", cce_eval="probs"):
        self.ctx, self.n_labels, self.hidden, self.pool, self.prec = ctx, int(n_labels), hidden, pool, prec
        self.cce_train, self.cce_eval = cce_train, cce_eval
        self.comm = comm
        self._graph_opt = use_graph
        self.use_graph = use_graph is not False
        self._knob = {"fold": os.environ.get("GCNX_FOLD", "1") != "0", "duo": os.environ.get("GCNX_DUO", "1") != "0",
                      "fused": os.environ.get("GCNX_FUSED", "1") != "0", "side": int(os.environ.get("GCNX_SIDE", "1")),
                      "head_late": os.environ.get("GCNX_HEAD_LATE", "1") != "0",
                      "s_order": os.environ.get("GCNX_S_ORDER", "1") != "0",
                      "buckets": os.environ.get("GCNX_COMM_BUCKETS", "1") != "0",
                      "act16": os.environ.get("GCNX_ACT16", "1") != "0",
                      "pool_in_spmm": os.environ.get("GCNX_POOL_IN_SPMM", "1") != "0"}
        self._rng = np.random.default_rng(seed)
        self.built = False
        self._bufs = None
        self._graphs = {}

    def build(self, f_in):
        h = self.hidden or f_in
        c = self.n_labels
        self.f_in, self.hidden = f_in, h
        shapes = {"w1": (f_in, h), "b1": (h,), "w2": (h, h), "b2": (h,), "w3": (h, c), "b3": (c,)}
        self.n_params = sum(int(np.prod(s)) for s in shapes.values())
        self.flat_p = self.ctx.zeros(self.n_params)
        self.flat_g = self.ctx.zeros(self.n_params + 2)
        self.p, self.g = {}, {}
        off = 0
        for k in self.PARAM_ORDER:
            n = int(np.prod(shapes[k]))
            self.p[k] = self.flat_p.flat(off, n, shapes[k])
            self.g[k] = self.flat_g.flat(off, n, shapes[k])
            off += n
        self.loss_acc = self.flat_g.flat(off, 2)
        init = {"w1": glorot_uniform(self._rng, f_in, h), "w2": glorot_uniform(self._rng, h, h),
                "w3": glorot_uniform(self._rng, h, c)}
        for k, v in init.items():
            self.p[k].copy_from_host(v)
        self.built = True

    def get_weights(self):
        return [self.p[k].numpy() for k in self.PARAM_ORDER]

    def set_weights(self, weights):
        for k, w in zip(self.PARAM_ORDER, weights):
            self.p[k].copy_from_host(np.asarray(w, np.float32).reshape(self.p[k].shape))

    @property
    def trainable_variables(self):
        return [self.p[k] for k in self.PARAM_ORDER]

    @property
    def losses(self):
        return []

    def _ensure(self, batch):
        if not self.built:
            self.build(batch.f)
        key = (batch.n, batch.n_graphs)
        if self._bufs is not None and self._bufs["key"] == key:
            return self._bufs
        n, b, h, c = batch.n, batch.n_graphs, self.hidden, self.n_labels
        self._drop_graphs()
        if getattr(self, "_cap", None) is None:
            self._cap = _Capacity(self.ctx)
        v = self._cap.view
        self._bufs = {"key": key}
        for k in ("h", "y1", "y2", "dz", "h2", "dz2"):
            self._bufs[k] = v(k, n, h)
        if self._fused(batch):
            self._bufs["s1"], self._bufs["s2"] = v("s1", n, self.f_in), v("s2", n, h)
            self._bufs["w2t"] = v("w2t", h, h)
            tr = D.pool_tile_rows(n, b)
            self._bufs["tp_part"], self._bufs["tp_cnt"] = v("tp_part", tr, h), v("tp_cnt", tr, h)
            self._bufs["pool_sum"], self._bufs["pool_cnt"] = v("pool_sum", b, h), v("pool_cnt", b, h)
        elif self._s_order():
            self._bufs["s1"] = v("s1", n, self.f_in)
        for k, w in (("pooled", h), ("probs", c), ("dpooled", h)):
            self._bufs[k] = v(k, b, w)
        self._bufs["arg"] = v("arg", b, h, np.int32) if self.pool == "max" else None
        return self._bufs

    def _forward(self, batch, bufs, with_loss, denom):
        ctx, p, prec = self.ctx, self.p, self.prec
        if self._fused(batch):
            keep = with_loss == "grads"
            late = keep and self._head_late(batch)
            D.gcn_conv_fwd(ctx, batch.a, batch.x, p["w1"], p["b1"], bufs["y1"], act="relu", s=bufs["s1"] if keep else None,
                           prec=prec)
            D.gcn_conv_fwd(ctx, batch.a, bufs["y1"], p["w2"], p["b2"], bufs["y2"], act="relu", s=bufs["s2"] if keep else None,
                           wt=bufs["w2t"] if keep else None, prec=prec,
                           pool=(batch.seg, bufs["tp_part"], bufs["tp_cnt"]) if late else None)
        else:
            bufs["act16"] = False
            if self._s_order() and self._act16_try(batch, with_loss):
                s16 = self._cap.view("s1_16", batch.n, self.f_in, np.uint16)
                if D.spmm_bf16out(ctx, batch.a, batch.x, None, s16):
                    y16 = self._cap.view("y1_16", batch.n, self.hidden, np.uint16)
                    bufs["y1bits"] = self._cap.view("y1bits", batch.n, 16, np.int32) if with_loss == "grads" else None
                    bufs["wimg"] = D.stream_images(ctx, [(p["w1"], True), (p["w2"], True), (p["w2"], False)],
                                                   self._cap.view("wimg", 3, 65536, np.uint16))
                    if not (D.gemm_fwd_bf16(ctx, s16, p["w1"], p["b1"], y16, act="relu", bits=bufs["y1bits"], wimg=bufs["wimg"][0])
                            and D.gemm_fwd_bf16(ctx, y16, p["w2"], None, bufs["h"], wimg=bufs["wimg"][1])):
                        raise RuntimeError("gcnx: the streaming bf16 GEMM refused a shape the bf16-storage path was chosen for")
                    bufs["act16"], bufs["y1bits_ok"], bufs["s1_16"], bufs["y1_16"] = True, with_loss == "grads", s16, y16
            if bufs["act16"]:
                pass
            elif self._s_order():
                D.spmm(ctx, batch.a, batch.x, None, bufs["s1"])
                bufs["y1bits_ok"] = False
                if (with_loss == "grads" and prec in ("bf16", "bf16x3") and self.hidden == 256 and self.f_in == 256
                        and batch.n >= 32768):
                    bufs["y1bits"] = self._cap.view("y1bits", batch.n, 16, np.int32)
                    bufs["y1bits_ok"] = D.gemm_relu_bits(ctx, bufs["s1"], p["w1"], p["b1"], bufs["y1"], bufs["y1bits"], prec=prec)
                if not bufs["y1bits_ok"]:
                    D.gemm(ctx, bufs["s1"], p["w1"], p["b1"], bufs["y1"], act="relu", prec=prec)
            else:
                D.gemm(ctx, batch.x, p["w1"], None, bufs["h"], prec=prec)
                D.spmm(ctx, batch.a, bufs["h"], p["b1"], bufs["y1"], act="relu")
            if not bufs["act16"]:
                D.gemm(ctx, bufs["y1"], p["w2"], None, bufs["h"], prec=prec)
            bufs["y2bits_ok"] = bufs["pool_done"] = False
            if (self._fold(batch) and batch.a.plan is not None and self.hidden % 32 == 0
                    and (with_loss == "grads" or self._knob["pool_in_spmm"])):
                bufs["y2bits"] = self._cap.view("y2bits", batch.n, self.hidden // 32, np.int32)
                if self._knob["pool_in_spmm"] and not self._head_late(batch):
                    bufs["pool_cnt2"] = self._cap.view("pool_cnt2", batch.n_graphs, self.hidden)
                    bufs["pool_done"] = D.spmm_relu_bits_pool(ctx, batch.a, bufs["h"], p["b2"], bufs["y2"], bufs["y2bits"], batch.seg,
                                                              bufs["pooled"], bufs["pool_cnt2"], self.pool)
                bufs["y2bits_ok"] = bufs["pool_done"] or (with_loss == "grads" and
                                                          D.spmm_relu_bits(ctx, batch.a, bufs["h"], p["b2"], bufs["y2"], bufs["y2bits"]))
            if not bufs["y2bits_ok"]:
                D.spmm(ctx, batch.a, bufs["h"], p["b2"], bufs["y2"], act="relu")
        head = dict(mode=self.pool, argmax=bufs["arg"])
        bufs["_head_late"] = None
        if with_loss == "grads" and self._head_late(batch):
            bufs["_head_late"] = D.head_args(batch.seg, bufs["tp_part"], bufs["tp_cnt"], bufs["pool_sum"], bufs["pool_cnt"], p["w3"],
                                             p["b3"], batch.y, denom, bufs["probs"], self.loss_acc, self.g["w3"], self.g["b3"],
                                             self.g["b2"], bufs["pooled"], bufs["dpooled"], mode=self.pool, cce=self.cce_train)
        elif with_loss == "grads" and bufs.get("pool_done"):
            D.pooled_dense_softmax_cce(ctx, batch.seg, bufs["pooled"], bufs["pool_cnt2"], p["w3"], p["b3"], batch.y, bufs["probs"],
                                       self.loss_acc, denom, dw=self.g["w3"], db=self.g["b3"], dpooled=bufs["dpooled"], mode=self.pool,
                                       db_relu=self.g["b2"], cce=self.cce_train)
        elif with_loss == "grads":
            D.pool_dense_softmax_cce(ctx, batch.seg, bufs["y2"], bufs["pooled"], p["w3"], p["b3"], batch.y, bufs["probs"],
                                     self.loss_acc, denom, dw=self.g["w3"], db=self.g["b3"], dpooled=bufs["dpooled"],
                                     db_relu=self.g["b2"] if self._fold(batch) else None, cce=self.cce_train, **head)
        elif bufs.get("pool_done"):
            D.pooled_dense_softmax_cce(ctx, batch.seg, bufs["pooled"], None, p["w3"], p["b3"], batch.y if with_loss else None, bufs["probs"],
                                       self.loss_acc if with_loss else None, denom, mode=self.pool, cce=self.cce_eval)
        elif with_loss:
            D.pool_dense_softmax_cce(ctx, batch.seg, bufs["y2"], bufs["pooled"], p["w3"], p["b3"], batch.y, bufs["probs"],
                                     self.loss_acc, denom, cce=self.cce_eval, **head)
        else:
            D.pool_dense_softmax_cce(ctx, batch.seg, bufs["y2"], bufs["pooled"], p["w3"], p["b3"], None, bufs["probs"], **head)

    def _backward(self, batch, bufs, lr=None, buckets=False):
        ctx, p, g, prec = self.ctx, self.p, self.g, self.prec
        self._reduced_in_backward = False
        at = batch.a.transpose()
        side = self._knob["side"]
        if side != 1:
            return self._backward_knob(batch, bufs, 0 if side == 0 else 7)
        fold = self._fold(batch)
        if self._fused(batch):
            ha = bufs.get("_head_late")
            pend = D.gcn_conv_bwd_pool(ctx, at, bufs["y2"], batch.seg, None if ha is not None else bufs["dpooled"], p["w2"], bufs["y1"],
                                       bufs["dz"], bufs["dz2"], db1=g["b1"], mode=self.pool, scratch=self._defer_scratch(batch),
                                       w2t=bufs["w2t"], prec=prec, head=ha)
            if lr is None:
                D.gemm_dw2(ctx, bufs["s1"], bufs["dz2"], g["w1"], bufs["s2"], bufs["dz"], g["w2"], prec="f32",
                           grads=self.flat_g.flat(0, self.n_params), pending=pend, leaf=ha)
                return False
            D.gemm_dw2(ctx, bufs["s1"], bufs["dz2"], g["w1"], bufs["s2"], bufs["dz"], g["w2"], prec="f32", params=self.flat_p,
                       grads=self.flat_g.flat(0, self.n_params), lr=lr, pending=pend, leaf=ha)
            return True
        act16 = bool(bufs.get("act16"))
        dh16 = self._cap.view("dh2_16", batch.n, self.hidden, np.uint16) if act16 else None
        dh16_done = False
        if fold and act16 and bufs.get("y2bits_ok"):
            dh16_done = D.spmm_pool_bwd_bf16out(ctx, at, bufs["y2"], batch.seg, bufs["dpooled"], dh16, self.pool, y_bits=bufs["y2bits"])
        if dh16_done:
            pass
        elif fold:
            D.spmm_pool_bwd(ctx, at, bufs["y2"], batch.seg, bufs["dpooled"], bufs["h"], self.pool,
                            y_bits=bufs["y2bits"] if bufs.get("y2bits_ok") else None)
        else:
            D.segment_pool_bwd(ctx, batch.seg, bufs["dpooled"], bufs["dz"], self.pool, bufs["arg"], y=bufs["y2"])
            D.spmm(ctx, at, bufs["dz"], None, bufs["h"])
        if fold and batch.a.plan is None and self._knob["duo"]:
            if lr is None:
                D.dense_bwd(ctx, bufs["y1"], bufs["h"], p["w2"], bufs["dz2"], g["w2"], prec=prec, y_mask=bufs["y1"],
                            db_prev=g["b1"])
                if buckets:
                    self._allreduce_tail_bucket()
                xs, dh1 = self._layer1_dw_operands(batch, bufs, at)
                D.gemm_dw(ctx, xs, dh1, g["w1"], prec=prec)
                if buckets:
                    self._allreduce_head_bucket()
                return False
            pend = D.dense_bwd_deferred(ctx, bufs["y1"], bufs["h"], p["w2"], bufs["dz2"], g["w2"], self._defer_scratch(batch),
                                        prec=prec, y_mask=bufs["y1"], db_prev=g["b1"])
            xs, dh1 = self._layer1_dw_operands(batch, bufs, at)
            D.gemm_dw_sgd(ctx, xs, dh1, g["w1"], self.flat_p, self.flat_g.flat(0, self.n_params), lr, prec=prec,
                          pending=pend)
            return True
        import contextlib
        if act16 and not dh16_done:
            D.to_bf16_into(ctx, bufs["h"], dh16)
        with (contextlib.nullcontext() if "s1" in bufs else ctx.side()):
            if not fold:
                D.act_bias_grad(ctx, bufs["dz"], None, bufs["dz"], None, db=g["b2"])
            if act16:
                self._must(D.gemm_dw_bf16(ctx, bufs["y1_16"], dh16, g["w2"]))
            else:
                D.gemm_dw(ctx, bufs["y1"], bufs["h"], g["w2"], prec=prec)
        if buckets:
            ctx.join()
            self._allreduce_tail_bucket()
        if act16:
            dz16 = self._cap.view("dz1_16", batch.n, self.hidden, np.uint16)
            self._must(D.gemm_dx_bf16(ctx, dh16, p["w2"], dz16, mask_bits=bufs["y1bits"], db=g["b1"], wimg=bufs["wimg"][2]))
            self._must(D.gemm_dw_bf16(ctx, bufs["s1_16"], dz16, g["w1"]))
        else:
            D.gemm_dx(ctx, bufs["h"], p["w2"], bufs["dz2"], prec=prec, y_mask=bufs["y1"], db=g["b1"],
                      mask_bits=bufs["y1bits"] if bufs.get("y1bits_ok") else None)
            xs, dh1 = self._layer1_dw_operands(batch, bufs, at)
            D.gemm_dw(ctx, xs, dh1, g["w1"], prec=prec)
        ctx.join()
        if buckets:
            self._allreduce_head_bucket()

    @staticmethod
    def _must(ok):
        if not ok:
            raise RuntimeError("gcnx: a bf16-storage kernel refused a shape its producer had accepted")

    def _act16_try(self, batch, with_loss):
        return (self.prec == "bf16" and self._knob["act16"] and self.hidden == 256 and self.f_in == 256
                and batch.n >= 32768 and batch.a.plan is not None and batch.a.vals is not None and self._knob["side"] == 1)

    def _allreduce_tail_bucket(self):
        import contextlib
        off = self._bucket_split()
        tail = self.flat_g.flat(off, self.n_params + 2 - off)
        with (self.ctx.side() if getattr(self.comm, "capturable", False) else contextlib.nullcontext()):
            self.comm.allreduce_sum(tail)

    def _allreduce_head_bucket(self):
        self.ctx.join()
        self.comm.allreduce_sum(self.flat_g.flat(0, self._bucket_split()))
        self._reduced_in_backward = True

    def _bucket_split(self):
        return int(np.prod(self.p["w1"].shape)) + int(np.prod(self.p["b1"].shape))

    def _s_order(self):
        return self._knob["s_order"] and self.built and self.f_in <= self.hidden

    def _layer1_dw_operands(self, batch, bufs, at):
        if "s1" in bufs and not self._fused(batch):
            return bufs["s1"], bufs["dz2"]
        D.spmm(self.ctx, at, bufs["dz2"], None, bufs["h2"])
        return batch.x, bufs["h2"]

    def _defer_scratch(self, batch):
        need = max(D.dense_bwd_scratch_floats(self.ctx, batch.n, self.hidden, self.hidden),
                   D.gcn_conv_bwd_scratch_floats(self.ctx, batch.n, self.hidden))
        cur = getattr(self, "_defer_buf", None)
        if cur is None or cur.size < need:
            self._defer_buf = self.ctx.empty(max(need, 4))
        return self._defer_buf

    def _fold(self, batch):
        return (self.pool in ("sum", "avg") and self.hidden % 4 == 0 and (batch.a.plan is None or self.hidden % 32 == 0)
                and self._knob["fold"] and self._knob["side"] == 1)

    def _fused(self, batch):
        route = batch.__dict__.setdefault("_route", {})
        key = ("fused", id(self), self.prec, self.built, batch.a.plan is None)
        if key not in route:
            route[key] = bool(self.built and self._fold(batch) and self.prec in ("f32", "bf16x3") and self._knob["fused"]
                              and self._knob["duo"] and self.f_in in (32, 64, 128) and self.hidden in (32, 64, 128)
                              and D.gcn_conv_fused_ok(self.ctx, batch.n, self.f_in, self.hidden)
                              and D.gcn_conv_fused_ok(self.ctx, batch.n, self.hidden, self.hidden))
        return route[key]

    def _head_late(self, batch):
        return (self._knob["head_late"] and self._fused(batch) and self.n_labels <= 2 and batch.y is not None
                and not batch.seg.has_empty)

    def _backward_knob(self, batch, bufs, side):
        import contextlib
        ctx, p, g, prec = self.ctx, self.p, self.g, self.prec
        at = batch.a.transpose()
        sec = lambda on: ctx.side() if on else contextlib.nullcontext()
        D.segment_pool_bwd(ctx, batch.seg, bufs["dpooled"], bufs["dz"], self.pool, bufs["arg"], y=bufs["y2"])
        with sec(side & 1):
            D.act_bias_grad(ctx, bufs["dz"], None, bufs["dz"], None, db=g["b2"])
        D.spmm(ctx, at, bufs["dz"], None, bufs["h"])
        ctx.join()
        with sec(side & 2):
            D.gemm_dw(ctx, bufs["y1"], bufs["h"], g["w2"], prec=prec)
        D.gemm_dx(ctx, bufs["h"], p["w2"], bufs["dz"], prec=prec, y_mask=bufs["y1"])
        ctx.join()
        with sec(side & 4):
            D.act_bias_grad(ctx, bufs["dz"], None, bufs["dz"], None, db=g["b1"])
        D.spmm(ctx, at, bufs["dz"], None, bufs["h"])
        D.gemm_dw(ctx, batch.x, bufs["h"], g["w1"], prec=prec)
        ctx.join()

    def _world(self):
        return self.comm.world_size if self.comm is not None else 1

    def _as_batch(self, inputs, target=None):
        if isinstance(inputs, DeviceBatch):
            if target is not None and inputs.y is None:
                inputs.y = self.ctx.to_device(target, np.float32)
            return inputs
        return DeviceBatch.from_host(self.ctx, _without_e(inputs), target)

    def __call__(self, inputs, training=False):
        batch = self._as_batch(inputs)
        bufs = self._ensure(batch)
        self._bind(batch)
        self._run(("fwd", batch.uid), lambda: self._forward(batch, bufs, False, None))
        return bufs["probs"].numpy()

    def _comm_in_graph(self):
        return (self.use_graph and self._world() > 1 and getattr(self.comm, "capturable", False)
                and not getattr(self, "_comm_capture_failed", False))

    def loss_and_grads(self, inputs, target, global_batch=None, _lr=None):
        batch = self._as_batch(inputs, target)
        bufs = self._ensure(batch)
        denom = float(global_batch or batch.n_graphs)
        multi = self._world() > 1
        if self._graph_opt == "auto":
            self.use_graph = bool(multi or not (self._fused(batch) and self._head_late(batch)))
        fused_comm = multi and _lr is not None and self._comm_in_graph()

        buckets = multi and self._knob["buckets"] and (fused_comm or not self.use_graph)

        def seq():
            self._forward(batch, bufs, "grads", denom)
            if self._backward(batch, bufs, None if multi else _lr, buckets=buckets):
                return
            if fused_comm and not self._reduced_in_backward:
                self.comm.allreduce_sum(self.flat_g)
            if _lr is not None and (fused_comm or not multi):
                D.sgd(self.ctx, self.flat_p, self.flat_g.flat(0, self.n_params), _lr)
        self._bind(batch)
        self._step_applied = fused_comm or not multi
        lr_key = self._lr_key(_lr)
        try:
            self._run(("grad", batch.uid, denom, lr_key if self._step_applied else None), seq)
        except Exception as e:
            if not fused_comm:
                raise
            import sys
            print(f"gcnx: RCCL all-reduce could not be captured into the step graph ({e}); falling back to an eager "
                  f"collective between two graphs", file=sys.stderr)
            self._comm_capture_failed = True
            self._drop_graphs()
            return self.loss_and_grads(batch, None, global_batch, _lr)
        if multi and not fused_comm and not self._reduced_in_backward:
            self.comm.allreduce_sum(self.flat_g)
        self._last_batch = batch
        self.ctx.set_lr_source(None)
        return batch

    def train_step(self, inputs, target=None, lr=0.02, global_batch=None, fetch=True):
        batch = self.loss_and_grads(inputs, target, global_batch, _lr=float(lr))
        if not self._step_applied:
            self._run(("sgd", self._lr_key(float(lr))), lambda: D.sgd(self.ctx, self.flat_p, self.flat_g.flat(0, self.n_params), lr))
            self.ctx.set_lr_source(None)
        if fetch == "stash":
            self.stash_metrics(global_batch or batch.n_graphs)
            return None
        if not fetch:
            return None
        return self.fetch_metrics(global_batch or batch.n_graphs)

    def fetch_metrics(self, n_graphs):
        la = self.loss_acc.numpy()
        return float(la[0]), float(la[1]) / float(n_graphs)

    def evaluate_batch(self, inputs, target):
        batch = self._as_batch(inputs, target)
        bufs = self._ensure(batch)
        self._forward(batch, bufs, True, float(batch.n_graphs))
        la = self.loss_acc.numpy()
        return float(la[0]), float(la[1]) / batch.n_graphs, bufs["probs"].numpy()

    def gradients(self):
        return {k: self.g[k].numpy() for k in self.PARAM_ORDER}


def evaluate(model, loader, normalize=None):
    from .train import evaluate as _evaluate
    return _evaluate(model, loader, normalize)


class GeneralGNN(_GraphRunner):

    @D.with_default_context
    def __init__(self, ctx, output, activation=None, hidden=256, message_passing=4, pre_process=2, post_process=2,
                 connectivity="cat", batch_norm=True, dropout=0.0, aggregate="sum", hidden_activation="prelu", pool="sum",
                 prec="f32", seed=0, use_graph=True, comm=None, cce_train="logits", cce_eval="probs"):
        self.use_graph, self._graphs = use_graph, {}
        self.cce_train, self.cce_eval = cce_train, cce_eval
        self.comm = comm
        if activation == "linear":
            activation = None
        if activation not in ("softmax", None):
            raise NotImplementedError(f"GeneralGNN(activation={activation!r}): 'softmax' (gcn.py:320) and None are built")
        self.activation = activation
        if activation is None:
            self.cce_train = self.cce_eval = "logits"
        if connectivity not in ("cat", "sum"):
            raise NotImplementedError(f"GeneralGNN(connectivity={connectivity!r}): 'cat' (gcn.py:320) and 'sum' are built")
        if hidden_activation == "linear":
            hidden_activation = None
        if hidden_activation not in ("prelu", "relu", None):
            raise NotImplementedError(f"GeneralGNN(hidden_activation={hidden_activation!r}): 'prelu' (gcn.py:320), 'relu' and None are built")
        if not 0.0 <= float(dropout) < 1.0:
            raise ValueError(f"GeneralGNN(dropout={dropout!r}): a rate in [0, 1)")
        self.connectivity, self.batch_norm, self.dropout = connectivity, bool(batch_norm), float(dropout)
        self.hidden_activation, self.seed = hidden_activation, int(seed)
        if aggregate not in ("sum", "mean", "max", "min", "prod"):
            raise ValueError(f"GeneralGNN(aggregate={aggregate!r}): Spektral's aggregations are 'sum' (gcn.py:320), 'mean', 'max', 'min', 'prod'")
        if pool not in ("sum", "avg", "max"):
            raise NotImplementedError(f"GeneralGNN(pool={pool!r}): 'sum' (gcn.py:320), 'avg' and 'max' are built")
        self.aggregate, self.pool = aggregate, pool
        self.ctx, self.output, self.hidden, self.mp = ctx, int(output), int(hidden), int(message_passing)
        self.n_pre, self.n_post, self.prec = int(pre_process), int(post_process), prec
        self._rng = np.random.default_rng(seed)
        self.built = False
        self._bufs = None
        self._images_fresh, self._img_jobs = False, []

    def build(self, f_in):
        h, mp = self.hidden, self.mp
        dims = []
        w = f_in
        for _ in range(self.n_pre):
            dims.append(("pre", w, h, True)); w = h
        cat, bn, prelu = self.connectivity == "cat", self.batch_norm, self.hidden_activation == "prelu"
        for k in range(mp):
            dims.append(("gnn", h * (k + 1) if cat else h, h, True))
        w = self._wpool = h * (mp + 1) if cat else h
        for k in range(self.n_post):
            last = k == self.n_post - 1
            dims.append(("post", w, self.output if last else h, not last)); w = h
        n_train = sum(fi * fo + fo + (2 * fo if bn else 0) + (fo if pr and prelu else 0) for _, fi, fo, pr in dims)
        n_state = sum(2 * fo for _, _, fo, _ in dims) if bn else 0
        self.n_params = n_train
        ctx = self.ctx
        self.flat_p, self.flat_g = ctx.zeros(n_train), ctx.zeros(n_train + 2)
        self.flat_s = ctx.zeros(max(n_state, 1))
        self.loss_acc = self.flat_g.flat(n_train, 2)
        self.layers = []
        self._step_dev = ctx.zeros(1, np.int32)
        off = soff = 0
        for grp, fi, fo, pr in dims:
            L = {"group": grp, "fi": fi, "fo": fo, "act": self.hidden_activation if pr else None, "index": len(self.layers)}
            for name, shape in (("kernel", (fi, fo)), ("bias", (fo,))) + ((("gamma", (fo,)), ("beta", (fo,))) if bn else ()) + \
                    ((("alpha", (fo,)),) if pr and prelu else ()):
                n = int(np.prod(shape))
                L[name] = self.flat_p.flat(off, n, shape)
                L["g_" + name] = self.flat_g.flat(off, n, shape)
                off += n
            L["sums"], L["scratch"] = ctx.zeros(2 * fo), ctx.zeros(3 * fo)
            from .layers import glorot_uniform
            L["kernel"].copy_from_host(glorot_uniform(self._rng, fi, fo))
            if bn:
                L["moving_mean"] = self.flat_s.flat(soff, fo); L["moving_var"] = self.flat_s.flat(soff + fo, fo); soff += 2 * fo
                L["mean"], L["inv"] = ctx.zeros(fo), ctx.zeros(fo)
                L["gamma"].copy_from_host(np.ones(fo, np.float32))
                L["moving_var"].copy_from_host(np.ones(fo, np.float32))
                L["bn_gamma"], L["bn_beta"], L["bn_g_gamma"], L["bn_g_beta"] = L["gamma"], L["beta"], L["g_gamma"], L["g_beta"]
            else:
                L["mean"], L["inv"] = ctx.zeros(fo), ctx.to_device(np.ones(fo, np.float32))
                L["bn_gamma"], L["bn_beta"] = L["inv"], L["mean"]
                L["bn_g_gamma"], L["bn_g_beta"] = ctx.zeros(fo), ctx.zeros(fo)
            self.layers.append(L)
        self.f_in, self.built = f_in, True
        self._alloc_images()

    def _alloc_images(self):
        self._img_jobs = []
        self._img_prec = self.prec
        if self.prec == "f32":
            return
        ctx = self.ctx
        for i, L in enumerate(self.layers):
            L.pop("img_fwd", None); L.pop("img_bwd", None)
            if L["group"] == "post" or L["fo"] % 16 or L["fi"] % 4:
                continue
            ef = D.wimage_elems(ctx, L["fi"], L["fo"], False, self.prec)
            L["img_fwd"] = ctx.empty(ef, np.uint16)
            self._img_jobs.append((L["kernel"], L["img_fwd"], False, self.prec))
            if i > 0 and L["fi"] % 16 == 0:
                L["img_bwd"] = ctx.empty(D.wimage_elems(ctx, L["fi"], L["fo"], True, self.prec), np.uint16)
                self._img_jobs.append((L["kernel"], L["img_bwd"], True, self.prec))

    WEIGHT_ORDER = ("kernel", "bias", "gamma", "beta", "moving_mean", "moving_var", "alpha")
    GNN_ORDERS = {"layer": WEIGHT_ORDER,
                  "keras": ("kernel", "bias", "alpha", "gamma", "beta", "moving_mean", "moving_var"),
                  "keras_children_first": ("alpha", "gamma", "beta", "kernel", "bias", "moving_mean", "moving_var")}

    def _weight_keys(self, L, order):
        keys = self.GNN_ORDERS[order] if L["group"] == "gnn" else self.WEIGHT_ORDER
        return [k for k in keys if k in L]

    def get_weights(self, order="keras"):
        return [L[k].numpy() for L in self.layers for k in self._weight_keys(L, order)]

    def set_weights(self, weights, order="keras"):
        it = iter(weights)
        for L in self.layers:
            for k in self._weight_keys(L, order):
                L[k].copy_from_host(np.asarray(next(it), np.float32).reshape(L[k].shape))

    @property
    def trainable_variables(self):
        return [L[k] for L in self.layers for k in ("kernel", "bias", "gamma", "beta", "alpha") if k in L]

    @property
    def losses(self):
        return []

    def _ensure(self, batch):
        if not self.built:
            self.build(batch.f)
        key = (batch.n, batch.n_graphs)
        if self._bufs is not None and self._bufs["key"] == key:
            return self._bufs
        ctx, n, b, h = self.ctx, batch.n, batch.n_graphs, self.hidden
        self._drop_graphs()
        wcat = h * (self.mp + 1)
        if getattr(self, "_cap", None) is None:
            self._cap = _Capacity(ctx)
        v = self._cap.view
        wp = self._wpool
        bufs = {"key": key, "cat": v("cat", n, wcat), "dcat": v("dcat", n, wcat), "h": v("h", n, h), "dh": v("dh", n, h),
                "pooled": v("pooled", b, wp), "dpooled": v("dpooled", b, wp), "probs": v("probs", b, self.output),
                "dlogits": v("dlogits", b, self.output), "zy": v("zy", b, self.output, zero=True)}
        for i, L in enumerate(self.layers):
            rows = b if L["group"] == "post" else n
            bufs[f"z{i}"] = v(f"z{i}", rows, L["fo"])
            bufs[f"y{i}"] = v(f"y{i}", rows, L["fo"])
        self._bufs = bufs
        return bufs

    def _multi(self):
        return self.comm is not None and self.comm.world_size > 1

    def _drop(self, L, t):
        seed = self.seed + (0x9E37 * self.comm.rank if self._multi() else 0)
        D.dropout(self.ctx, t, self.dropout, seed, L["index"], self._step_dev)

    def _dense_bn(self, L, x, z, y, training):
        self._dense_bn_core(L, x, z, y, training)
        if training and self.dropout > 0.0:
            self._drop(L, y)

    def _dense_bn_core(self, L, x, z, y, training):
        ctx = self.ctx
        if not self.batch_norm:
            if not ("img_fwd" in L and self._images_fresh and
                    D.gemm_wimage(ctx, x, L["img_fwd"], L["fi"], L["fo"], z, bias=L["bias"], prec=self.prec) is not None):
                D.gemm(ctx, x, L["kernel"], L["bias"], z, prec=self._prec_of(L))
            D.bn_act(ctx, z, L["mean"], L["inv"], L["bn_gamma"], L["bn_beta"], y, act=L["act"], alpha=L.get("alpha"))
            return
        if "img_fwd" in L and self._images_fresh:
            fused_bn = training and not self._multi() and L["fo"] <= 256
            parts = self._bn_parts(x.shape[0], L["fo"]) if fused_bn else None
            nparts = D.gemm_wimage(ctx, x, L["img_fwd"], L["fi"], L["fo"], z, bias=L["bias"], prec=self.prec, bn_parts=parts)
            if nparts is not None:
                if fused_bn:
                    D.bn_finalize_parts(ctx, parts, nparts, L["mean"], L["inv"], L["moving_mean"], L["moving_var"])
                    D.bn_act(ctx, z, L["mean"], L["inv"], L["gamma"], L["beta"], y, act=L["act"], alpha=L.get("alpha"))
                    return
            else:
                D.gemm(ctx, x, L["kernel"], L["bias"], z, prec=self._prec_of(L))
        else:
            D.gemm(ctx, x, L["kernel"], L["bias"], z, prec=self._prec_of(L))
        if training and self._multi():
            count = self._counts["b" if L["group"] == "post" else "n"]
            D.bn_stats(ctx, z, L["sums"])
            self.comm.allreduce_sum(L["sums"])
            D.bn_finalize(ctx, L["sums"], count, L["mean"], L["inv"])
            D.bn_stats(ctx, z, L["sums"], shift=L["mean"])
            self.comm.allreduce_sum(L["sums"])
            D.bn_finalize(ctx, L["sums"], count, L["mean"], L["inv"], L["moving_mean"], L["moving_var"], shift=L["mean"])
        elif training:
            D.bn_moments(ctx, z, L["sums"], L["mean"], L["inv"], L["moving_mean"], L["moving_var"])
        else:
            D.bn_finalize(ctx, None, 1, L["mean"], L["inv"], L["moving_mean"], L["moving_var"])
        D.bn_act(ctx, z, L["mean"], L["inv"], L["gamma"], L["beta"], y, act=L["act"], alpha=L.get("alpha"))

    def _agg_operator(self, batch):
        return batch.a.row_mean() if self.aggregate == "mean" else batch.a.unweighted()

    def _forward(self, batch, bufs, training):
        h, mp = self.hidden, self.mp
        cat = bufs["cat"]
        a = self._agg_operator(batch)
        x = batch.x
        li = 0
        for k in range(self.n_pre):
            L = self.layers[li]
            y = cat.cols(mp * h, (mp + 1) * h) if k == self.n_pre - 1 else bufs[f"y{li}"]
            self._dense_bn(L, x, bufs[f"z{li}"], y, training)
            x = y; li += 1
        sumc = self.connectivity == "sum"
        for k in range(mp):
            L = self.layers[li]
            inp = cat.cols((mp - k) * h, (mp - k + 1) * h if sumc else (mp + 1) * h)
            minmax = self.aggregate in ("max", "min", "prod")
            hk = self._tmp(bufs, f"msg{li}", (batch.n, h)) if minmax else bufs["h"]
            self._dense_bn(L, inp, bufs[f"z{li}"], hk, training)
            new = cat.cols((mp - k - 1) * h, (mp - k) * h)
            if minmax:
                ck = self._tmp(bufs, f"aggcnt{li}", (batch.n, h))
                zk = self._tmp(bufs, f"agg{li}", (batch.n, h)) if sumc else new
                D.spmm_minmax(self.ctx, a, hk, zk, ck, self.aggregate)
                if sumc:
                    D.add(self.ctx, zk, inp, new)
            else:
                D.spmm(self.ctx, a, bufs["h"], None, new)
                if sumc:
                    D.add(self.ctx, new, inp, new)
            li += 1
        if self.pool == "max":
            if getattr(self, "_cap", None) is None:
                self._cap = _Capacity(self.ctx)
            bufs["pool_arg"] = self._cap.view("pool_arg", bufs["pooled"].shape[0], bufs["pooled"].shape[1], np.int32)
        D.segment_pool(self.ctx, batch.seg, cat.cols(0, h) if sumc else cat, bufs["pooled"], self.pool,
                       bufs.get("pool_arg") if self.pool == "max" else None)
        x = bufs["pooled"]
        for k in range(self.n_post):
            L = self.layers[li]
            self._dense_bn(L, x, bufs[f"z{li}"], bufs[f"y{li}"], training)
            x = bufs[f"y{li}"]; li += 1
        return x

# ... 711 lines not shown
```

include/gcnx.h:

```cpp
#ifndef GCNX_H
#define GCNX_H

#include <stddef.h>
#include <stdint.h>

#if defined(__GNUC__)
#define GCNX_API __attribute__((visibility("default")))
#else
#define GCNX_API
#endif

#ifdef __cplusplus
extern "C" {
#endif

typedef struct gcnx_ctx gcnx_ctx;
typedef struct gcnx_comm gcnx_comm;
typedef struct gcnx_graph gcnx_graph;
typedef struct gcnx_event gcnx_event;
typedef struct gcnx_spmm_plan gcnx_spmm_plan;

typedef enum {
  GCNX_OK = 0,
  GCNX_ERR_INVALID = 1,
  GCNX_ERR_HIP = 2,
  GCNX_ERR_RCCL = 3,
  GCNX_ERR_NOMEM = 4,
  GCNX_ERR_UNSUPPORTED = 5,
  GCNX_ERR_DATA = 6
} gcnx_status;

typedef enum { GCNX_ACT_NONE = 0, GCNX_ACT_RELU = 1, GCNX_ACT_PRELU = 2, GCNX_ACT_PRELU_SHARED = 3 } gcnx_act;
typedef enum { GCNX_POOL_SUM = 0, GCNX_POOL_AVG = 1, GCNX_POOL_MAX = 2 } gcnx_pool;
typedef enum { GCNX_PREC_F32 = 0, GCNX_PREC_BF16 = 1, GCNX_PREC_BF16X3 = 2 } gcnx_prec;
typedef enum { GCNX_NORM_SPEKTRAL = 0, GCNX_NORM_PYG = 1 } gcnx_norm_mode;
typedef enum { GCNX_RED_SUM = 0, GCNX_RED_MAX = 1 } gcnx_redop;
typedef enum { GCNX_CCE_PROBS = 0, GCNX_CCE_LOGITS = 1 } gcnx_cce_mode;

#define GCNX_UNIQUE_ID_BYTES 128

GCNX_API int gcnx_version(void);
GCNX_API int gcnx_device_count(int* n);
GCNX_API int gcnx_ctx_create(int device, gcnx_ctx** out);
GCNX_API int gcnx_ctx_destroy(gcnx_ctx* ctx);
GCNX_API const char* gcnx_last_error(gcnx_ctx* ctx);
GCNX_API int gcnx_device_info(gcnx_ctx* ctx, char* name, int len, int* cus, size_t* hbm_bytes);

GCNX_API int gcnx_set_tuning(gcnx_ctx* ctx, const char* key, int value);

GCNX_API int gcnx_malloc(gcnx_ctx* ctx, size_t bytes, void** dptr);
GCNX_API int gcnx_free(gcnx_ctx* ctx, void* dptr);
GCNX_API int gcnx_memset(gcnx_ctx* ctx, void* dptr, int value, size_t bytes);
GCNX_API int gcnx_h2d(gcnx_ctx* ctx, void* dst, const void* src, size_t bytes);
GCNX_API int gcnx_h2d_async(gcnx_ctx* ctx, void* dst, const void* src, size_t bytes);
GCNX_API int gcnx_d2h(gcnx_ctx* ctx, void* dst, const void* src, size_t bytes);
GCNX_API int gcnx_d2d(gcnx_ctx* ctx, void* dst, const void* src, size_t bytes);
GCNX_API int gcnx_sync(gcnx_ctx* ctx);
GCNX_API int gcnx_side_begin(gcnx_ctx* ctx);
GCNX_API int gcnx_side_end(gcnx_ctx* ctx);
GCNX_API int gcnx_side_join(gcnx_ctx* ctx);

GCNX_API int gcnx_event_create(gcnx_ctx* ctx, gcnx_event** out);
GCNX_API int gcnx_event_record(gcnx_ctx* ctx, gcnx_event* ev);
GCNX_API int gcnx_event_elapsed_ms(gcnx_ctx* ctx, gcnx_event* start, gcnx_event* stop, float* ms);
GCNX_API int gcnx_event_destroy(gcnx_ctx* ctx, gcnx_event* ev);

GCNX_API int gcnx_capture_begin(gcnx_ctx* ctx);
GCNX_API int gcnx_capture_end(gcnx_ctx* ctx, gcnx_graph** out);
GCNX_API int gcnx_graph_launch(gcnx_ctx* ctx, gcnx_graph* g);
GCNX_API int gcnx_graph_destroy(gcnx_ctx* ctx, gcnx_graph* g);

GCNX_API int gcnx_coo_to_csr(gcnx_ctx* ctx, const int64_t* rows, const int64_t* cols, int64_t nnz,
                    int64_t n, int32_t* rowptr, int32_t* colidx);
GCNX_API int gcnx_collate(gcnx_ctx* ctx, const int32_t* desc, int32_t b, const int32_t* node_ptr, const int32_t* rowptr,
                 const int32_t* colidx, const float* vals, const float* x, int64_t ldx, int32_t f, const float* y,
                 int32_t c, int32_t* o_rowptr, int32_t* o_colidx, float* o_vals, float* o_x, int64_t ldo, float* o_y,
                 int32_t* o_graph_ptr, int32_t* o_node_graph);
GCNX_API int gcnx_gcn_norm(gcnx_ctx* ctx, const int32_t* rowptr, const int32_t* colidx,
                  const float* vals_in, int32_t n, int mode, float* vals_out);
#define GCNX_CSR_SYMMETRIC 1
#define GCNX_CSR_BLOCK_DIAGONAL 2
#define GCNX_CSR_GRAPH_PTR_OK 4
GCNX_API int gcnx_csr_inspect(gcnx_ctx* ctx, const int32_t* rowptr, const int32_t* colidx, const float* vals, int32_t n,
                     const int32_t* graph_ptr, int32_t b, int* props);
GCNX_API int gcnx_csr_transpose(gcnx_ctx* ctx, const int32_t* rowptr, const int32_t* colidx,
                       const float* vals, int32_t n, int32_t nnz, int32_t* rowptr_t,
                       int32_t* colidx_t, float* vals_t);
GCNX_API int gcnx_csr_transpose_perm(gcnx_ctx* ctx, const int32_t* rowptr, const int32_t* colidx, int32_t n, int32_t nnz,
                            int32_t* rowptr_t, int32_t* colidx_t, int32_t* perm_t);

GCNX_API int gcnx_ecc_expand(gcnx_ctx* ctx, const int32_t* rowptr_t, const int32_t* colidx_t, const int32_t* eperm, const float* u,
                    int64_t ldu, int32_t sp, const float* x, int64_t ldx, int32_t f, float* scat, int64_t ld, int32_t n,
                    int32_t nnz, int root);
GCNX_API int gcnx_ecc_bwd(gcnx_ctx* ctx, const int32_t* rowptr, const int32_t* colidx, const float* u, int64_t ldu, int32_t sp,
                 const float* x, int64_t ldx, const float* dscat, int64_t ldd, const float* dx_root, int64_t lddr, int32_t f,
                 float* dx, int64_t lddx, float* du, int64_t lddu, int32_t n, int32_t nnz);

GCNX_API int gcnx_gemm(gcnx_ctx* ctx, const float* x, int64_t ldx, const float* w, const float* bias,
              float* out, int64_t ldo, int64_t n, int32_t fi, int32_t fo, int prec, int act,
              const float* alpha);
typedef struct gcnx_wimage_job {
  const float* w;
  void* img;
  int32_t fi, fo;
  int32_t transpose, prec;
} gcnx_wimage_job;
GCNX_API int64_t gcnx_wimage_elems(int32_t fi, int32_t fo, int transpose, int prec);
GCNX_API int gcnx_wimage_prepare(gcnx_ctx* ctx, int32_t njobs, const gcnx_wimage_job* jobs);
GCNX_API int gcnx_gemm_wimage(gcnx_ctx* ctx, const float* x, int64_t ldx, const void* img, int32_t fi, int32_t fo, int transpose,
                     const float* bias, float* out, int64_t ldo, int64_t n, int prec, int accumulate, float* bn_parts,
                     int32_t* n_parts);
GCNX_API int64_t gcnx_gemm_wimage_parts(gcnx_ctx* ctx, int64_t n);
GCNX_API int gcnx_bn_finalize_parts(gcnx_ctx* ctx, const float* parts, int32_t nparts, int32_t f, float momentum, float eps,
                           float* mean, float* inv, float* moving_mean, float* moving_var);
GCNX_API int gcnx_spmm_plan_create(gcnx_ctx* ctx, const int32_t* block_ptr, int32_t nblocks,
                                   gcnx_spmm_plan** out);
GCNX_API int gcnx_spmm_plan_destroy(gcnx_ctx* ctx, gcnx_spmm_plan* plan);
GCNX_API int gcnx_spmm_plan_bind(gcnx_ctx* ctx, gcnx_spmm_plan* plan, const int32_t* rowptr, int32_t n);
GCNX_API int gcnx_spmm_csr(gcnx_ctx* ctx, const int32_t* rowptr, const int32_t* colidx,
                  const float* vals, const float* h, int64_t ldh, const float* bias, float* out,
                  int64_t ldo, int32_t n, int32_t f, int act, const gcnx_spmm_plan* plan);
GCNX_API int gcnx_segment_pool(gcnx_ctx* ctx, const int32_t* graph_ptr, const float* x, int64_t ldx,
                      float* pooled, int32_t b, int32_t f, int mode, int32_t* argmax);
GCNX_API int gcnx_softmax_cce(gcnx_ctx* ctx, const float* logits, const float* y, int32_t b, int32_t c,
                     float denom, float* probs, float* loss_acc, float* dlogits, int cce_mode);

GCNX_API int gcnx_dense_softmax_cce(gcnx_ctx* ctx, const float* pooled, int64_t ldp, const float* w, const float* bias,
                           const float* y, int32_t b, int32_t h, int32_t c, float denom, float* probs,
                           float* loss_acc, float* dw, float* db, float* dpooled, int64_t lddp, int cce_mode);

GCNX_API int gcnx_pool_dense_softmax_cce(gcnx_ctx* ctx, const int32_t* graph_ptr, const float* x, int64_t ldx, int pool_mode,
                                int32_t* argmax, float* pooled, int64_t ldp, const float* w, const float* bias,
                                const float* y, int32_t b, int32_t h, int32_t c, float denom, float* probs,
                                float* loss_acc, float* dw, float* db, float* dpooled, int64_t lddp,
                                float* db_relu, int cce_mode);

GCNX_API int gcnx_act_bias_grad(gcnx_ctx* ctx, const float* dy, int64_t lddy, const float* y, int64_t ldy,
                       float* dz, int64_t lddz, int64_t n, int32_t f, int act,
                       const float* alpha, float* db, float* dalpha);
GCNX_API int gcnx_gemm_dw(gcnx_ctx* ctx, const float* x, int64_t ldx, const float* dh, int64_t lddh,
                 float* dw, int64_t n, int32_t fi, int32_t fo, int prec);
GCNX_API int gcnx_spmm_csr_bf16out(gcnx_ctx* ctx, const int32_t* rowptr, const int32_t* colidx, const float* vals, const float* h,
                          int64_t ldh, const float* bias, void* out16, int64_t ldo, int32_t n, int32_t f, int act,
                          const gcnx_spmm_plan* plan);
GCNX_API int gcnx_spmm_csr_pool_bwd_bf16out(gcnx_ctx* ctx, const int32_t* rowptr, const int32_t* colidx, const float* vals,
                          const float* y, int64_t ldy, const int32_t* graph_ptr, int32_t b, const float* dpooled, int64_t lddp,
                          void* out16, int64_t ldo, int32_t n, int32_t f, int mode, const gcnx_spmm_plan* plan, const void* y_bits);
GCNX_API int gcnx_gemm_fwd_bf16(gcnx_ctx* ctx, const void* x16, int64_t ldx, const float* w, const float* bias, void* out, int64_t ldo,
                          int out_bf16, int64_t n, int32_t fi, int32_t fo, int act, void* relu_bits, const void* wimg);
GCNX_API int gcnx_gemm_dx_bf16(gcnx_ctx* ctx, const void* dh16, int64_t lddh, const float* w, void* dx, int64_t lddx, int dx_bf16,
                          int64_t n, int32_t fi, int32_t fo, const void* mask_bits, float* db, const void* wimg);
#define GCNX_STREAM_IMAGE_BYTES 131072
typedef struct gcnx_stream_image_job {
  const float* w; int32_t fi, fo;
  int32_t transpose;
  void* img;
} gcnx_stream_image_job;
GCNX_API int gcnx_gemm_stream_images(gcnx_ctx* ctx, int32_t njobs, const gcnx_stream_image_job* jobs);
GCNX_API int gcnx_gemm_dw_bf16(gcnx_ctx* ctx, const void* x16, int64_t ldx, const void* dh16, int64_t lddh, float* dw, int64_t n,
                          int32_t fi, int32_t fo);
GCNX_API int gcnx_gemm_relu_bits(gcnx_ctx* ctx, const float* x, int64_t ldx, const float* w, const float* bias, float* out,
                        int64_t ldo, int64_t n, int32_t fi, int32_t fo, int prec, void* bits);
GCNX_API int gcnx_gemm_dx_bits(gcnx_ctx* ctx, const float* dh, int64_t lddh, const float* w, float* dx, int64_t lddx,
                      int64_t n, int32_t fi, int32_t fo, int prec, const void* mask_bits, float* db);
GCNX_API int gcnx_gemm_dx(gcnx_ctx* ctx, const float* dh, int64_t lddh, const float* w, float* dx,
                 int64_t lddx, int64_t n, int32_t fi, int32_t fo, int prec, int accumulate,
                 const float* y_mask, int64_t ldy, float* db);
GCNX_API int gcnx_dense_bwd(gcnx_ctx* ctx, const float* x, int64_t ldx, const float* dh, int64_t lddh, const float* w,
                   int64_t n, int32_t fi, int32_t fo, int prec, float* dx, int64_t lddx, const float* y_mask,
                   int64_t ldy, float* db_prev, float* dw);
GCNX_API int gcnx_segment_pool_bwd(gcnx_ctx* ctx, const int32_t* graph_ptr, const float* dpooled,
                          float* dx, int64_t lddx, int32_t n, int32_t b, int32_t f, int mode,
                          const int32_t* argmax, const float* y, int64_t ldy, float* db);

GCNX_API int gcnx_spmm_csr_pool_bwd(gcnx_ctx* ctx, const int32_t* rowptr, const int32_t* colidx, const float* vals,
                           const float* y, int64_t ldy, const int32_t* graph_ptr, int32_t b,
                           const float* dpooled, int64_t lddp, float* out, int64_t ldo, int32_t n, int32_t f,
                           int mode, const gcnx_spmm_plan* plan, const void* y_bits);
GCNX_API int gcnx_spmm_csr_relu_bits(gcnx_ctx* ctx, const int32_t* rowptr, const int32_t* colidx, const float* vals,
                           const float* h, int64_t ldh, const float* bias, float* out, int64_t ldo, int32_t n, int32_t f,
                           const gcnx_spmm_plan* plan, void* relu_bits);
GCNX_API int gcnx_spmm_csr_relu_bits_pool(gcnx_ctx* ctx, const int32_t* rowptr, const int32_t* colidx, const float* vals, const float* h,
                        int64_t ldh, const float* bias, float* out, int64_t ldo, int32_t n, int32_t f, const gcnx_spmm_plan* plan,
                        void* relu_bits, const int32_t* graph_ptr, int32_t b, int pool_mode, float* pooled, int64_t ldp, float* cnt);
GCNX_API int gcnx_pooled_dense_softmax_cce(gcnx_ctx* ctx, const int32_t* graph_ptr, int pool_mode, const float* pooled, int64_t ldp,
                        const float* cnt, const float* w, const float* bias, const float* y, int32_t b, int32_t h, int32_t c,
                        float denom, float* probs, float* loss_acc, float* dw, float* db, float* dpooled, int64_t lddp,
                        float* db_relu, int cce_mode);
GCNX_API int gcnx_pool_bwd_colsum(gcnx_ctx* ctx, const int32_t* graph_ptr, int32_t b, const float* dpooled,
                         int64_t lddp, const float* y, int64_t ldy, int32_t f, int mode, float* db);

GCNX_API int gcnx_bn_stats(gcnx_ctx* ctx, const float* z, int64_t ldz, int64_t n, int32_t f, const float* shift,
                           float* sums);
GCNX_API int gcnx_bn_finalize(gcnx_ctx* ctx, const float* sums, float count, int32_t f, float momentum,
                              float eps, const float* shift, float* mean, float* inv, float* moving_mean,
                              float* moving_var);
GCNX_API int gcnx_bn_moments(gcnx_ctx* ctx, const float* z, int64_t ldz, int64_t n, int32_t f, float momentum, float eps,
                    float* mean, float* inv, float* moving_mean, float* moving_var);
GCNX_API int gcnx_bn_act(gcnx_ctx* ctx, const float* z, int64_t ldz, int64_t n, int32_t f, const float* mean,
                         const float* inv, const float* gamma, const float* beta, int act, const float* alpha,
                         float* y, int64_t ldy);
GCNX_API int gcnx_bn_act_bwd(gcnx_ctx* ctx, const float* dy, int64_t lddy, const float* z, int64_t ldz, int64_t n,
                             int32_t f, const float* mean, const float* inv, const float* gamma, const float* beta,
                             int act, const float* alpha, int training, float* dz, int64_t lddz, float* dgamma,
                             float* dbeta, float* dalpha, float* sums_scratch);
GCNX_API int gcnx_bn_act_bwd_stats(gcnx_ctx* ctx, const float* dy, int64_t lddy, const float* z, int64_t ldz, int64_t n,
                          int32_t f, const float* mean, const float* inv, const float* gamma, const float* beta, int act,
                          const float* alpha, float* sums_scratch, float* dgamma, float* dbeta, float* dalpha);
GCNX_API int gcnx_bn_act_bwd_apply(gcnx_ctx* ctx, const float* dy, int64_t lddy, const float* z, int64_t ldz, int64_t n,
                          int32_t f, const float* mean, const float* inv, const float* gamma, const float* beta, int act,
                          const float* alpha, const float* sums, float count, int training, float* dz, int64_t lddz);

GCNX_API int gcnx_bn_act_pool(gcnx_ctx* ctx, const int32_t* graph_ptr, int32_t b, const float* z, int64_t ldz, int32_t f,
                     const float* mean, const float* inv, const float* gamma, const float* beta, int act, const float* alpha,
                     int pool_mode, float* pooled, int64_t ldp, int32_t* argmax);
GCNX_API int gcnx_bn_act_pool_bwd(gcnx_ctx* ctx, const int32_t* graph_ptr, int32_t b, const float* dpooled, int64_t lddp,
                         const int32_t* argmax, const float* z, int64_t ldz, int64_t n, int32_t f, const float* mean,
                         const float* inv, const float* gamma, const float* beta, int act, const float* alpha, int pool_mode,
                         float* dz, int64_t lddz, float* dgamma, float* dbeta, float* dalpha);
GCNX_API int gcnx_bn_act_pool_bwd_stats(gcnx_ctx* ctx, const int32_t* graph_ptr, int32_t b, const float* dpooled, int64_t lddp,
                         const int32_t* argmax, const float* z, int64_t ldz, int32_t f, const float* mean, const float* inv,
                         const float* gamma, const float* beta, int act, const float* alpha, int pool_mode, float* sums,
                         float* dgamma, float* dbeta, float* dalpha);
GCNX_API int gcnx_bn_act_pool_bwd_apply(gcnx_ctx* ctx, const int32_t* graph_ptr, int32_t b, const float* dpooled, int64_t lddp,
                         const int32_t* argmax, const float* z, int64_t ldz, int32_t f, const float* mean, const float* inv,
                         const float* gamma, const float* beta, int act, const float* alpha, int pool_mode, const float* sums,
                         float count, float* dz, int64_t lddz);
typedef struct gcnx_bce_head_args {
  const float* pooled; int64_t ldp; int32_t b; int32_t h;
  const float* w3; const float* b3; const float* gamma3; const float* beta3; const float* alpha3;
  const float* w4; const float* b4; const float* gamma4; const float* beta4; const float* alpha4;
  float eps; float denom;
  const float* y; int32_t y_stride; int32_t y_col; int32_t grads;
  float* out; float* probs; float* loss_acc;
  float* dpooled; int64_t lddp;
  float* dw3; float* db3; float* dgamma3; float* dbeta3; float* dalpha3;
  float* dw4; float* db4; float* dgamma4; float* dbeta4; float* dalpha4;
  float* scratch; int64_t scratch_floats;
} gcnx_bce_head_args;
GCNX_API int64_t gcnx_bce_head_scratch_floats(int32_t b, int32_t h);
GCNX_API int gcnx_bn_prelu_bce_head(gcnx_ctx* ctx, const gcnx_bce_head_args* args);
GCNX_API int64_t gcnx_bce_head_phase_scratch_floats(int32_t b, int32_t h);
GCNX_API int64_t gcnx_bce_head_phase_red_floats(int32_t h);
GCNX_API int gcnx_bce_head_phase(gcnx_ctx* ctx, const gcnx_bce_head_args* args, int32_t phase, float count, float* red);

GCNX_API int gcnx_dropout(gcnx_ctx* ctx, const float* x, int64_t ldx, int64_t n, int32_t f, float rate, uint32_t seed,
                          uint32_t stream_id, const uint32_t* step, float* out, int64_t ldo);
GCNX_API int gcnx_counter_add(gcnx_ctx* ctx, uint32_t* counter, uint32_t inc);
GCNX_API int gcnx_add(gcnx_ctx* ctx, const float* a, int64_t lda, const float* b, int64_t ldb, float* out, int64_t ldo,
                      int64_t n, int32_t f);

GCNX_API int gcnx_spmm_csr_minmax(gcnx_ctx* ctx, const int32_t* rowptr, const int32_t* colidx, const float* h, int64_t ldh,
                                  float* out, int64_t ldo, float* cnt, int64_t ldc, int32_t n, int32_t f, int is_min);
GCNX_API int gcnx_spmm_csr_minmax_bwd(gcnx_ctx* ctx, const int32_t* rowptr_t, const int32_t* colidx_t, const float* h, int64_t ldh,
                                      const float* out, int64_t ldo, const float* cnt, int64_t ldc, const float* dy, int64_t lddy,
                                      float* dh, int64_t lddh, int32_t n, int32_t f);

GCNX_API int gcnx_spmm_csr_prod(gcnx_ctx* ctx, const int32_t* rowptr, const int32_t* colidx, const float* h, int64_t ldh, float* out,
                                int64_t ldo, float* aux, int64_t lda, int32_t n, int32_t f);
GCNX_API int gcnx_spmm_csr_prod_bwd(gcnx_ctx* ctx, const int32_t* rowptr_t, const int32_t* colidx_t, const float* h, int64_t ldh,
                                    const float* out, int64_t ldo, const float* aux, int64_t lda, const float* dy, int64_t lddy,
                                    float* dh, int64_t lddh, int32_t n, int32_t f);

GCNX_API int gcnx_sgd(gcnx_ctx* ctx, float* params, const float* grads, int64_t n, float lr);
GCNX_API int gcnx_set_lr_source(gcnx_ctx* ctx, const float* lr_dev);
typedef struct gcnx_pending_reduce {
  const float* colpart; int64_t crows; int32_t cf; float* cout;
  const float* slabs; int64_t total; int32_t nsplit; float* out;
} gcnx_pending_reduce;

GCNX_API int64_t gcnx_dense_bwd_scratch_floats(gcnx_ctx* ctx, int64_t n, int32_t fi, int32_t fo);
GCNX_API int gcnx_dense_bwd_deferred(gcnx_ctx* ctx, const float* x, int64_t ldx, const float* dh, int64_t lddh,
                            const float* w, int64_t n, int32_t fi, int32_t fo, int prec, float* dx, int64_t lddx,
                            const float* y_mask, int64_t ldy, float* db_prev, float* dw, float* scratch,
                            int64_t scratch_floats, gcnx_pending_reduce* pending);

GCNX_API int gcnx_gemm_dw_sgd(gcnx_ctx* ctx, const float* x, int64_t ldx, const float* dh, int64_t lddh, float* dw,
                     int64_t n, int32_t fi, int32_t fo, int prec, float* params, float* grads, int64_t n_params,
                     float lr, const gcnx_pending_reduce* pending);

GCNX_API int gcnx_gcn_conv_fused_ok(int64_t n, int32_t fi, int32_t fo, int64_t ldx);
GCNX_API int gcnx_gcn_conv_fwd(gcnx_ctx* ctx, const int32_t* rowptr, const int32_t* colidx, const float* vals,
                      const float* x, int64_t ldx, int32_t n, int32_t fi, const float* w, int32_t fo,
                      const float* bias, int act, float* s, int64_t lds, float* out, int64_t ldo, float* wt_out,
                      int prec);
GCNX_API int gcnx_gcn_conv_fwd_pool(gcnx_ctx* ctx, const int32_t* rowptr, const int32_t* colidx, const float* vals,
                      const float* x, int64_t ldx, int32_t n, int32_t fi, const float* w, int32_t fo,
                      const float* bias, int act, float* s, int64_t lds, float* out, int64_t ldo, float* wt_out,
                      int prec, const int32_t* node_graph, int32_t b, float* tile_part, float* tile_cnt);
typedef struct gcnx_head_args {
  const float* tile_part; const float* tile_cnt; int64_t tile_rows;
  float* pool_sum; float* pool_cnt;
  const int32_t* graph_ptr; int32_t b; int32_t h; int pool_mode;
  const float* w; const float* bias; const float* y; int32_t c; float denom; int cce_mode;
  float* probs; float* loss_acc; float* dw; float* db; float* db_relu; float* pooled; float* dpooled;
} gcnx_head_args;

GCNX_API int64_t gcnx_gcn_conv_bwd_scratch_floats(int64_t n, int32_t f1);
GCNX_API int gcnx_gcn_conv_bwd_pool(gcnx_ctx* ctx, const int32_t* rowptr_t, const int32_t* colidx_t, const float* vals_t,
                      const float* y2, int64_t ldy2, const int32_t* node_graph, const int32_t* graph_ptr, int32_t b,
                      const float* dpooled, int64_t lddp, int mode, int32_t n, int32_t f2, const float* w2, int32_t f1,
                      int w2_transposed, const float* y1, int64_t ldy1, float* dz2, int64_t lddz2, float* dz1, int64_t lddz1, float* db1,
                      float* scratch, int64_t scratch_floats, gcnx_pending_reduce* pending, int prec,
                      const gcnx_head_args* head);
GCNX_API int gcnx_gemm_dw2(gcnx_ctx* ctx, const float* xa, int64_t ldxa, const float* dha, int64_t lddha, float* dwa,
                      int32_t fia, int32_t foa, const float* xb, int64_t ldxb, const float* dhb, int64_t lddhb,
                      float* dwb, int32_t fib, int32_t fob, int64_t n, int prec, float* params, float* grads,
                      int64_t n_params, float lr, const gcnx_pending_reduce* pending, const gcnx_head_args* leaf);

GCNX_API int gcnx_spmm_csr_bf16(gcnx_ctx* ctx, const int32_t* rowptr, const int32_t* colidx, const float* vals,
                      const uint16_t* h, int64_t ldh, const float* bias, uint16_t* out, int64_t ldo, int32_t n, int32_t f,
                      int act);
GCNX_API int gcnx_f32_to_bf16(gcnx_ctx* ctx, const float* x, uint16_t* y, int64_t count);
GCNX_API int gcnx_bf16_to_f32(gcnx_ctx* ctx, const uint16_t* x, float* y, int64_t count);

GCNX_API int gcnx_comm_unique_id(char id[GCNX_UNIQUE_ID_BYTES]);
GCNX_API int gcnx_comm_init_rank(gcnx_ctx* ctx, const char id[GCNX_UNIQUE_ID_BYTES], int nranks,
                        int rank, gcnx_comm** out);
GCNX_API int gcnx_comm_destroy(gcnx_comm* comm);
GCNX_API int gcnx_allreduce_f32(gcnx_ctx* ctx, gcnx_comm* comm, float* buf, int64_t n, int op);

#ifdef __cplusplus
}
#endif
#endif
```

Measured before the change: 335,800 graphs/s.

## Store layer-2 ReLU mask as bytes and gather it in backward SpMM

The forward of the second GCNConv writes a uint8 ReLU mask (0/1 per element). During training with the late head it can skip writing the fp32 y2 output entirely. The backward fused kernel gets an M8 variant that gathers 16-byte mask chunks per neighbour instead of fp32 rows with a step function. This cuts the gather traffic of the backward SpMM about fourfold and removes the y2 store. The cost is a new kernel path with a different lane mapping, and a mask buffer that must stay consistent with y2 whenever y2 is still needed.

```diff
diff --git a/gcn-string_amd/csrc/fused.hip b/gcn-string_amd/csrc/fused.hip
--- a/gcn-string_amd/csrc/fused.hip
+++ b/gcn-string_amd/csrc/fused.hip
@@ -28,6 +28,7 @@
   const float* hd_part; const float* hd_cnt; int hd_rows; int hd_b;
   float* hd_psum; float* hd_csum;
   const float* hd_w; const float* hd_bias; const float* hd_y; int hd_c; float hd_denom; int hd_fl;
+  unsigned char* m8_out; const unsigned char* m8; int64_t ldm8;
   int dbg;
 };
 
@@ -49,6 +50,19 @@
   asm("v_pk_mul_f32 %0, %1, %2 clamp" : "=v"(lo) : "v"(t0), "v"(big));
   asm("v_pk_mul_f32 %0, %1, %2 clamp" : "=v"(hi) : "v"(t1), "v"(big));
   return make_float4(lo[0], lo[1], hi[0], hi[1]);
+}
+
+constexpr int kM8B = 16;
+constexpr int kM8U = 4;
+typedef unsigned m8x16 __attribute__((ext_vector_type(4)));
+__device__ __forceinline__ m8x16 m8load(__amdgpu_buffer_rsrc_t rs, unsigned off) {
+  return __builtin_bit_cast(m8x16, __builtin_amdgcn_raw_buffer_load_b128(rs, off, 0, 0));
+}
+__device__ __forceinline__ void m8fma(float v, m8x16 m, float (&a)[kM8B]) {
+#pragma unroll
+  for (int d = 0; d < kM8B / 4; ++d)
+#pragma unroll
+    for (int k = 0; k < 4; ++k) a[4 * d + k] = fmaf(v, (float)((m[d] >> (8 * k)) & 0xffu), a[4 * d + k]);
 }
 
 __device__ __forceinline__ void f4acc(float4& a, const float4 q) { a.x += q.x; a.y += q.y; a.z += q.z; a.w += q.w; }
@@ -73,23 +87,29 @@
   return make_float2(dl0 * sc, dl1 * sc);
 }
 
-template <int K, bool WEIGHTED, bool BWD, bool X3 = false>
+template <int K, bool WEIGHTED, bool BWD, bool X3 = false, bool M8 = false>
 __global__ __launch_bounds__(512, 6) void gcn_conv_fused_kernel(FusedArgs p) {
-  constexpr int LPR = K / 4;
+  constexpr int MLB = kM8B, UM = kM8U;
+  constexpr int HL = K / 4;
+  constexpr int LPR = M8 ? K / MLB : K / 4;
+  constexpr int CPL = K / LPR;
   constexpr int GW = 64 / LPR;
   constexpr int NG = 8 * GW;
   constexpr int RPG = NG >= kFRows ? 1 : kFRows / NG;
   constexpr int U = 4;
+  constexpr int SL = 2 * U;
+  static_assert(UM <= SL, "the mask gather reads up to UM - 1 entries past a row's end");
   static_assert(K == 32 || K == 64 || K == 128, "gather width");
+  static_assert(!M8 || (BWD && RPG == 1), "the byte-image gather is a backward form, one row per lane group");
   __shared__ __attribute__((aligned(16))) float tile[kFRows][K + 4];
-  __shared__ __attribute__((aligned(8))) int2 s_ent[kFCap + 2 * U];
+  __shared__ __attribute__((aligned(8))) int2 s_ent[kFCap + SL];
   __shared__ int32_t s_rp[kFRows + 1];
   __shared__ unsigned char s_mb[BWD ? kFRows * 32 : 1];
   __shared__ float2 s_dl[BWD ? kFRows : 1];
   __shared__ __attribute__((aligned(16))) float s_w3[BWD ? 2 : 1][K];
   __shared__ float s_b3[2];
   __shared__ int32_t s_g[BWD ? 1 : kFRows];
-  static_assert(!BWD || sizeof(float) * kFRows * (K + 4) >= sizeof(float4) * 2 * 8 * 2 * LPR, "the head's wave partials alias the tile");
+  static_assert(!BWD || sizeof(float) * kFRows * (K + 4) >= sizeof(float4) * 2 * 8 * 2 * HL, "the head's wave partials alias the tile");
 #ifdef GCNX_TUNING
   const int dbg = p.dbg;
 #else
@@ -105,8 +125,8 @@
     s_g[tid] = tid < nr ? min(max(p.node_graph[r0 + tid], 0), p.hd_b - 1) : -1;
   const int e0 = p.rowptr[r0], e1 = p.rowptr[r0 + nr];
   const int staged = min(e1 - e0, kFCap);
-  const unsigned ld4 = (unsigned)p.ldx * 4u;
-  for (int i = tid; i < staged + 2 * U; i += 512) {
+  const unsigned ld4 = M8 ? (unsigned)p.ldm8 : (unsigned)p.ldx * 4u;
+  for (int i = tid; i < staged + SL; i += 512) {
     int2 en = make_int2(0, 0);
     if (i < staged) {
       en.x = (int)((unsigned)p.colidx[e0 + i] * ld4);
@@ -116,7 +136,7 @@
   }
   const int gid = wave * GW + lane / LPR, sub = lane % LPR;
   const __amdgpu_buffer_rsrc_t xr =
-      __builtin_amdgcn_make_buffer_rsrc((void*)p.x, (short)0, (int)((unsigned)p.n * (unsigned)p.ldx * 4u), 0x00020000);
+      __builtin_amdgcn_make_buffer_rsrc(M8 ? (void*)p.m8 : (void*)p.x, (short)0, (int)((unsigned)p.n * ld4), 0x00020000);
   int grow[RPG];
   if (BWD) {
 #pragma unroll
@@ -135,8 +155,8 @@
       if (row < nr && !(dbg & 16)) mrow[q] = *reinterpret_cast<const float4*>(p.mask + (int64_t)(r0 + row) * p.ldmask + 4 * c4);
     }
   }
-  float4 (*s_pv)[2][2][LPR] = reinterpret_cast<float4 (*)[2][2][LPR]>(&tile[0][0]);
-  const int hsel = lane / LPR, hsub = lane % LPR;
+  float4 (*s_pv)[2][2][HL] = reinterpret_cast<float4 (*)[2][2][HL]>(&tile[0][0]);
+  const int hsel = lane / HL, hsub = lane % HL;
   int g_first = 0;
   if (BWD && p.hd_part) {
     g_first = min(max(__builtin_amdgcn_readfirstlane(p.node_graph[r0]), 0), p.hd_b - 1);
@@ -189,7 +209,7 @@
           *reinterpret_cast<float4*>(p.hd_psum + (int64_t)hd_g * K + hsub * 4) = pv;
           *reinterpret_cast<float4*>(p.hd_csum + (int64_t)hd_g * K + hsub * 4) = pc;
         }
-        const float2 dl = fused_head_dlogits<LPR>(p, pv, hd_n, *reinterpret_cast<const float4*>(&s_w3[0][hsub * 4]),
+        const float2 dl = fused_head_dlogits<HL>(p, pv, hd_n, *reinterpret_cast<const float4*>(&s_w3[0][hsub * 4]),
                                                   *reinterpret_cast<const float4*>(&s_w3[1][hsub * 4]),
                                                   s_b3[0], s_b3[1], y0, y1);
         if (hsub == 0) s_dl[hd_g - g_first] = dl;
@@ -223,6 +243,34 @@
   }
   if (dbg & 1) len = 0;
   const unsigned sub16 = (unsigned)sub * 16u;
+  float am[M8 ? CPL : 1] = {};
+  if constexpr (M8) {
+    const unsigned subb = (unsigned)sub * (unsigned)MLB;
+    for (int tt = 0; __builtin_amdgcn_ballot_w64(tt < len) != 0; tt += UM) {
+      m8x16 hv[UM];
+      float wv[UM];
+      const int eb_ = min(ea[0] + tt, ebf[0]);
+#pragma unroll
+      for (int u = 0; u < UM; ++u) {
+        const int e = eb_ + u;
+        const int2 en = s_ent[e];
+        wv[u] = __int_as_float(en.y);
+        hv[u] = m8load(xr, e < ebf[0] ? (unsigned)en.x + subb : 0xFFFFFFF0u);
+      }
+      __builtin_amdgcn_sched_barrier(0);
+#pragma unroll
+      for (int u = 0; u < UM; ++u) {
+        m8fma(wv[u], hv[u], am);
+        if (u + 1 < UM) asm volatile("" : "+v"(hv[u + 1]), "+v"(am[0]));
+      }
+    }
+    if (e1 - e0 > kFCap) {
+      for (int e = max(eb[0] > 0 ? s_rp[gid] - e0 : 0, kFCap); e < eb[0]; ++e) {
+        const float v = WEIGHTED ? p.vals[e0 + e] : 1.0f;
+        m8fma(v, m8load(xr, (unsigned)p.colidx[e0 + e] * ld4 + subb), am);
+      }
+    }
+  } else {
   for (int tt = 0; __builtin_amdgcn_ballot_w64(tt < len) != 0; tt += U) {
     float4 hv[RPG][U];
     float wv[RPG][U];
@@ -253,7 +301,13 @@
         acc[j] = f4fma(v, BWD ? f4step(h) : h, acc[j]);
       }
   }
+  }
   float4 own[RPG], dscale[RPG];
+  m8x16 ownm = {};
+  if constexpr (M8) {
+    if (grow[0] >= 0 && p.dz2) ownm = *reinterpret_cast<const m8x16*>(p.m8 + (int64_t)(r0 + gid) * p.ldm8 + sub * MLB);
+    if (p.hd_part && !(dbg & 32)) __syncthreads();
+  } else
   if (BWD) {
 #pragma unroll
     for (int j = 0; j < RPG; ++j) {
@@ -309,6 +363,36 @@
         wl[st][j] = (__bf16)(v - (float)h);
       }
   }
+  if constexpr (M8) {
+    if (gid < kFRows) {
+      const int r = gid, g = grow[0];
+      float2 dl = make_float2(0.f, 0.f);
+      float sc = 1.0f;
+      if (g >= 0 && p.hd_part) dl = s_dl[(g - g_first) & (kFRows - 1)];
+      else if (g >= 0 && p.avg) sc = 1.0f / (float)(p.gp[g + 1] - p.gp[g]);
+#pragma unroll
+      for (int q = 0; q < CPL / 4; ++q) {
+        const int c = sub * CPL + 4 * q;
+        float4 d = make_float4(0.f, 0.f, 0.f, 0.f);
+        if (g >= 0 && (dbg & 32)) d = make_float4(1.f, 1.f, 1.f, 1.f);
+        else if (g >= 0 && p.hd_part) {
+          const float4 w0 = *reinterpret_cast<const float4*>(&s_w3[0][c]), w1 = *reinterpret_cast<const float4*>(&s_w3[1][c]);
+          d = make_float4(fmaf(dl.y, w1.x, dl.x * w0.x), fmaf(dl.y, w1.y, dl.x * w0.y), fmaf(dl.y, w1.z, dl.x * w0.z),
+                          fmaf(dl.y, w1.w, dl.x * w0.w));
+        } else if (g >= 0) {
+          d = *reinterpret_cast<const float4*>(p.dp + (int64_t)g * p.lddp + c);
+          if (p.avg) { d.x *= sc; d.y *= sc; d.z *= sc; d.w *= sc; }
+        }
+        if (p.dz2 && r < nr && !(dbg & 8)) {
+          const unsigned ow = ownm[q];
+          *reinterpret_cast<float4*>(p.dz2 + (int64_t)(r0 + r) * p.lddz2 + c) =
+              make_float4((float)(ow & 0xffu) * d.x, (float)((ow >> 8) & 0xffu) * d.y, (float)((ow >> 16) & 0xffu) * d.z,
+                          (float)(ow >> 24) * d.w);
+        }
+        *reinterpret_cast<float4*>(&tile[r][c]) = make_float4(am[4 * q] * d.x, am[4 * q + 1] * d.y, am[4 * q + 2] * d.z, am[4 * q + 3] * d.w);
+      }
+    }
+  } else
   if (gid < kFRows) {
 #pragma unroll
     for (int j = 0; j < RPG; ++j) {
@@ -379,7 +463,8 @@
     float v = r < 4 ? c0[r & 3] : c1[r & 3];
     if (BWD) v = mk[r] > 0.f ? v : 0.f;
     else { v += bcol; if (p.act == GCNX_ACT_RELU) v = fmaxf(v, 0.f); }
-    if (row < nr) p.out[(int64_t)(r0 + row) * p.ldo + col] = v;
+    if (row < nr && (BWD || p.out)) p.out[(int64_t)(r0 + row) * p.ldo + col] = v;
+    if (!BWD && p.m8_out && row < nr) p.m8_out[(int64_t)(r0 + row) * p.ldm8 + col] = v > 0.f ? (unsigned char)1 : (unsigned char)0;
     cs += v;
     vout[r] = v;
   }
@@ -422,6 +507,14 @@
 #ifdef GCNX_TUNING
   if (const char* e = getenv("GCNX_FUSED_LDS")) dyn = atoi(e);
 #endif
+#define GCNX_FUSED_LAUNCH_M8(K_)                                                                                      \
+  do {                                                                                                                \
+    if (x3) {                                                                                                         \
+      if (a.vals) hipLaunchKernelGGL((gcn_conv_fused_kernel<K_, true, BWD, true, BWD>), dim3(tiles), dim3(512), dyn, ctx->stream, a); \
+      else hipLaunchKernelGGL((gcn_conv_fused_kernel<K_, false, BWD, true, BWD>), dim3(tiles), dim3(512), dyn, ctx->stream, a);      \
+    } else if (a.vals) hipLaunchKernelGGL((gcn_conv_fused_kernel<K_, true, BWD, false, BWD>), dim3(tiles), dim3(512), dyn, ctx->stream, a); \
+    else hipLaunchKernelGGL((gcn_conv_fused_kernel<K_, false, BWD, false, BWD>), dim3(tiles), dim3(512), dyn, ctx->stream, a);      \
+  } while (0)
 #define GCNX_FUSED_LAUNCH(K_)                                                                                         \
   do {                                                                                                                \
     if (x3) {                                                                                                         \
@@ -430,10 +523,15 @@
     } else if (a.vals) hipLaunchKernelGGL((gcn_conv_fused_kernel<K_, true, BWD>), dim3(tiles), dim3(512), dyn, ctx->stream, a); \
     else hipLaunchKernelGGL((gcn_conv_fused_kernel<K_, false, BWD>), dim3(tiles), dim3(512), dyn, ctx->stream, a);      \
   } while (0)
-  if (k == 128) GCNX_FUSED_LAUNCH(128);
+  if (BWD && a.m8) {
+    if (k == 128) GCNX_FUSED_LAUNCH_M8(128);
+    else if (k == 64) GCNX_FUSED_LAUNCH_M8(64);
+    else GCNX_FUSED_LAUNCH_M8(32);
+  } else if (k == 128) GCNX_FUSED_LAUNCH(128);
   else if (k == 64) GCNX_FUSED_LAUNCH(64);
   else GCNX_FUSED_LAUNCH(32);
 #undef GCNX_FUSED_LAUNCH
+#undef GCNX_FUSED_LAUNCH_M8
   GCNX_LAUNCH_OK(ctx);
   return GCNX_OK;
 }
@@ -452,11 +550,14 @@
 
 int gcnx_gcn_conv_fused_ok(int64_t n, int32_t fi, int32_t fo, int64_t ldx) { return fused_shape_ok(n, fi, fo, ldx) ? 1 : 0; }
 
-int gcnx_gcn_conv_fwd_pool(gcnx_ctx* ctx, const int32_t* rowptr, const int32_t* colidx, const float* vals, const float* x,
-                           int64_t ldx, int32_t n, int32_t fi, const float* w, int32_t fo, const float* bias, int act, float* s,
-                           int64_t lds, float* out, int64_t ldo, float* wt_out, int prec, const int32_t* node_graph, int32_t b,
-                           float* tile_part, float* tile_cnt) {
+int gcnx_gcn_conv_fwd_mask8(gcnx_ctx* ctx, const int32_t* rowptr, const int32_t* colidx, const float* vals, const float* x,
+                            int64_t ldx, int32_t n, int32_t fi, const float* w, int32_t fo, const float* bias, int act, float* s,
+                            int64_t lds, float* out, int64_t ldo, float* wt_out, int prec, const int32_t* node_graph, int32_t b,
+                            float* tile_part, float* tile_cnt, uint8_t* mask8, int64_t ldmask8) {
   GCNX_CHECK_CTX(ctx);
+  GCNX_REQUIRE(ctx, !mask8 || act == GCNX_ACT_RELU, "gcnx_gcn_conv_fwd_mask8: the byte mask is that of a ReLU output");
+  GCNX_REQUIRE(ctx, !mask8 || (ldmask8 >= fo && ldmask8 % 16 == 0 && fal16(mask8)),
+               "gcnx_gcn_conv_fwd_mask8: mask8 must be 16-byte aligned with a leading dimension in multiples of 16 bytes");
   GCNX_RANGE(ctx, "GCNConv forward (one launch)");
   GCNX_REQUIRE(ctx, (!tile_part && !tile_cnt) || (tile_part && tile_cnt && node_graph && b > 0 && fal16(tile_part) && fal16(tile_cnt)),
                "gcnx_gcn_conv_fwd_pool: the pool's partial sums need node_graph, b > 0 and two 16-byte aligned outputs");
@@ -468,16 +569,24 @@
   if (!fused_shape_ok(n, fi, fo, ldx))
     return gcnx_fail(ctx, GCNX_ERR_UNSUPPORTED, "gcnx_gcn_conv_fwd: needs fi in {32, 64, 128}, fo a multiple of 16 up to 128 and "
                      "n * ldx * 4 < 2^32 (got n=%d fi=%d fo=%d): use gcnx_gemm + gcnx_spmm_csr", n, fi, fo);
-  GCNX_REQUIRE(ctx, rowptr && colidx && x && w && out, "gcnx_gcn_conv_fwd: NULL pointer");
-  GCNX_REQUIRE(ctx, ldo >= fo && ldo % 4 == 0 && fal16(x) && fal16(out) && (!bias || fal16(bias)) &&
+  GCNX_REQUIRE(ctx, rowptr && colidx && x && w && (out || mask8), "gcnx_gcn_conv_fwd: NULL pointer");
+  GCNX_REQUIRE(ctx, (!out || (ldo >= fo && ldo % 4 == 0 && fal16(out))) && fal16(x) && (!bias || fal16(bias)) &&
                         (!s || (lds >= fi && lds % 4 == 0 && fal16(s))),
                "gcnx_gcn_conv_fwd: operands must be 16-byte aligned with leading dimensions in multiples of 4 floats");
   GCNX_REQUIRE(ctx, x != out && x != s, "gcnx_gcn_conv_fwd: in-place aggregation is not possible");
   FusedArgs a{};
   a.rowptr = rowptr; a.colidx = colidx; a.vals = vals; a.x = x; a.ldx = ldx; a.n = n; a.w = w; a.ldw = fo; a.nc = fo;
   a.bias = bias; a.act = act; a.s = s; a.lds = lds; a.out = out; a.ldo = ldo; a.wt_out = wt_out;
-  a.node_graph = node_graph; a.tp_part = tile_part; a.tp_cnt = tile_cnt; a.hd_b = b;
+  a.node_graph = node_graph; a.tp_part = tile_part; a.tp_cnt = tile_cnt; a.hd_b = b; a.m8_out = mask8; a.ldm8 = ldmask8;
   return launch_fused<false>(ctx, a, fi, prec == GCNX_PREC_BF16X3);
+}
+
+int gcnx_gcn_conv_fwd_pool(gcnx_ctx* ctx, const int32_t* rowptr, const int32_t* colidx, const float* vals, const float* x,
+                           int64_t ldx, int32_t n, int32_t fi, const float* w, int32_t fo, const float* bias, int act, float* s,
+                           int64_t lds, float* out, int64_t ldo, float* wt_out, int prec, const int32_t* node_graph, int32_t b,
+                           float* tile_part, float* tile_cnt) {
+  return gcnx_gcn_conv_fwd_mask8(ctx, rowptr, colidx, vals, x, ldx, n, fi, w, fo, bias, act, s, lds, out, ldo, wt_out, prec,
+                                 node_graph, b, tile_part, tile_cnt, nullptr, 0);
 }
 
 int gcnx_gcn_conv_fwd(gcnx_ctx* ctx, const int32_t* rowptr, const int32_t* colidx, const float* vals, const float* x,
@@ -489,8 +598,12 @@
 
 int64_t gcnx_gcn_conv_bwd_scratch_floats(int64_t n, int32_t f1) { return n <= 0 || f1 <= 0 ? 0 : (int64_t)gcnx_cdiv(n, kFRows) * f1; }
 
-int gcnx_gcn_conv_bwd_pool(gcnx_ctx* ctx, const int32_t* rowptr_t, const int32_t* colidx_t, const float* vals_t,
-                           const float* y2, int64_t ldy2, const int32_t* node_graph, const int32_t* graph_ptr, int32_t b,
+}
+
+namespace {
+
+int conv_bwd_pool(gcnx_ctx* ctx, const int32_t* rowptr_t, const int32_t* colidx_t, const float* vals_t,
+                           const float* y2, const uint8_t* y2m, int64_t ldy2, const int32_t* node_graph, const int32_t* graph_ptr, int32_t b,
                            const float* dpooled, int64_t lddp, int mode, int32_t n, int32_t f2, const float* w2, int32_t f1,
                            int w2_transposed, const float* y1, int64_t ldy1, float* dz2, int64_t lddz2, float* dz1, int64_t lddz1, float* db1,
                            float* scratch, int64_t scratch_floats, gcnx_pending_reduce* pending, int prec,
@@ -507,13 +620,15 @@
     if (db1 && f1 > 0) GCNX_HIP(ctx, hipMemsetAsync(db1, 0, (size_t)f1 * 4, ctx->stream));
     return GCNX_OK;
   }
-  if (!fused_shape_ok(n, f2, f1, ldy2))
-    return gcnx_fail(ctx, GCNX_ERR_UNSUPPORTED, "gcnx_gcn_conv_bwd_pool: needs f2 in {32, 64, 128}, f1 a multiple of 16 up to 128 "
-                     "and n * ldy2 * 4 < 2^32 (got n=%d f1=%d f2=%d)", n, f1, f2);
-  GCNX_REQUIRE(ctx, b > 0 && rowptr_t && colidx_t && y2 && node_graph && graph_ptr && (dpooled || head) && w2 && y1 && dz1,
+  if (!fused_shape_ok(n, f2, f1, y2m ? f2 : ldy2) || (y2m && (ldy2 < f2 || (uint64_t)n * (uint64_t)ldy2 >= 0xFFFFFFF0ull)))
+    return gcnx_fail(ctx, GCNX_ERR_UNSUPPORTED, "%s: needs f2 in {32, 64, 128}, f1 a multiple of 16 up to 128 and %s (got n=%d f1=%d f2=%d)",
+                     y2m ? "gcnx_gcn_conv_bwd_pool_mask8" : "gcnx_gcn_conv_bwd_pool",
+                     y2m ? "ldmask8 >= f2, n * ldmask8 < 2^32 - 16" : "n * ldy2 * 4 < 2^32", n, f1, f2);
+  GCNX_REQUIRE(ctx, !y2m || ldy2 % 16 == 0, "gcnx_gcn_conv_bwd_pool_mask8: the mask's leading dimension must be a multiple of 16 bytes");
+  GCNX_REQUIRE(ctx, b > 0 && rowptr_t && colidx_t && (y2 || y2m) && node_graph && graph_ptr && (dpooled || head) && w2 && y1 && dz1,
                "gcnx_gcn_conv_bwd_pool: NULL pointer");
   GCNX_REQUIRE(ctx, (head || (lddp >= f2 && lddp % 4 == 0 && fal16(dpooled))) && ldy1 >= f1 && ldy1 % 4 == 0 && lddz1 >= f1 &&
-                        lddz1 % 4 == 0 && fal16(y2) && fal16(y1) && fal16(dz1) &&
+                        lddz1 % 4 == 0 && fal16(y2) && fal16(y2m) && fal16(y1) && fal16(dz1) &&
                         (!dz2 || (fal16(dz2) && lddz2 >= f2 && lddz2 % 4 == 0)),
                "gcnx_gcn_conv_bwd_pool: operands must be 16-byte aligned with leading dimensions in multiples of 4 floats");
   if (head) {
@@ -526,7 +641,8 @@
     if (head->c > 2)
       return gcnx_fail(ctx, GCNX_ERR_UNSUPPORTED, "gcnx_gcn_conv_bwd_pool: the in-kernel head serves one or two classes (got %d)", head->c);
   }
-  GCNX_REQUIRE(ctx, y2 != dz1 && y2 != dz2 && y1 != dz1, "gcnx_gcn_conv_bwd_pool: outputs must not alias the saved activations");
+  GCNX_REQUIRE(ctx, (y2m ? ((const void*)y2m != (const void*)dz1 && (const void*)y2m != (const void*)dz2) : (y2 != dz1 && y2 != dz2)) && y1 != dz1,
+               "gcnx_gcn_conv_bwd_pool: outputs must not alias the saved activations");
   const int64_t tiles = gcnx_cdiv(n, kFRows);
   float* colpart = nullptr;
   bool defer = false;
@@ -541,7 +657,7 @@
     }
   }
   FusedArgs a{};
-  a.rowptr = rowptr_t; a.colidx = colidx_t; a.vals = vals_t; a.x = y2; a.ldx = ldy2; a.n = n; a.w = w2; a.ldw = w2_transposed ? f1 : f2; a.w_t = w2_transposed ? 1 : 0; a.nc = f1;
+  a.rowptr = rowptr_t; a.colidx = colidx_t; a.vals = vals_t; a.x = y2; a.ldx = y2m ? f2 : ldy2; a.m8 = y2m; a.ldm8 = y2m ? ldy2 : 0; a.n = n; a.w = w2; a.ldw = w2_transposed ? f1 : f2; a.w_t = w2_transposed ? 1 : 0; a.nc = f1;
   a.out = dz1; a.ldo = lddz1; a.node_graph = node_graph; a.gp = graph_ptr; a.dp = dpooled; a.lddp = lddp;
   a.avg = mode == GCNX_POOL_AVG ? 1 : 0; a.mask = y1; a.ldmask = ldy1; a.dz2 = dz2; a.lddz2 = lddz2; a.colpart = colpart;
   if (head) {
@@ -559,3 +675,28 @@
 }
 
 }
+
+extern "C" {
+
+int gcnx_gcn_conv_bwd_pool(gcnx_ctx* ctx, const int32_t* rowptr_t, const int32_t* colidx_t, const float* vals_t,
+                           const float* y2, int64_t ldy2, const int32_t* node_graph, const int32_t* graph_ptr, int32_t b,
+                           const float* dpooled, int64_t lddp, int mode, int32_t n, int32_t f2, const float* w2, int32_t f1,
+                           int w2_transposed, const float* y1, int64_t ldy1, float* dz2, int64_t lddz2, float* dz1, int64_t lddz1, float* db1,
+                           float* scratch, int64_t scratch_floats, gcnx_pending_reduce* pending, int prec,
+                           const gcnx_head_args* head) {
+  return conv_bwd_pool(ctx, rowptr_t, colidx_t, vals_t, y2, nullptr, ldy2, node_graph, graph_ptr, b, dpooled, lddp, mode, n, f2, w2, f1,
+                       w2_transposed, y1, ldy1, dz2, lddz2, dz1, lddz1, db1, scratch, scratch_floats, pending, prec, head);
+}
+
+int gcnx_gcn_conv_bwd_pool_mask8(gcnx_ctx* ctx, const int32_t* rowptr_t, const int32_t* colidx_t, const float* vals_t,
+                                 const uint8_t* y2_mask8, int64_t ldmask8, const int32_t* node_graph, const int32_t* graph_ptr, int32_t b,
+                                 const float* dpooled, int64_t lddp, int mode, int32_t n, int32_t f2, const float* w2, int32_t f1,
+                                 int w2_transposed, const float* y1, int64_t ldy1, float* dz2, int64_t lddz2, float* dz1, int64_t lddz1,
+                                 float* db1, float* scratch, int64_t scratch_floats, gcnx_pending_reduce* pending, int prec,
+                                 const gcnx_head_args* head) {
+  if (ctx && !y2_mask8 && n > 0 && f1 > 0) return gcnx_fail(ctx, GCNX_ERR_INVALID, "gcnx_gcn_conv_bwd_pool_mask8: NULL pointer");
+  return conv_bwd_pool(ctx, rowptr_t, colidx_t, vals_t, nullptr, y2_mask8, ldmask8, node_graph, graph_ptr, b, dpooled, lddp, mode, n, f2, w2,
+                       f1, w2_transposed, y1, ldy1, dz2, lddz2, dz1, lddz1, db1, scratch, scratch_floats, pending, prec, head);
+}
+
+}
diff --git a/gcn-string_amd/gcnx/_lib.py b/gcn-string_amd/gcnx/_lib.py
--- a/gcn-string_amd/gcnx/_lib.py
+++ b/gcn-string_amd/gcnx/_lib.py
@@ -137,6 +137,10 @@
     "gcnx_bf16_to_f32": [_vp, _vp, _vp, _i64],
     "gcnx_gcn_conv_fwd_pool": [_vp, _vp, _vp, _vp, _vp, _i64, _i32, _i32, _vp, _i32, _vp, _int, _vp, _i64, _vp, _i64, _vp, _int,
                                _vp, _i32, _vp, _vp],
+    "gcnx_gcn_conv_fwd_mask8": [_vp, _vp, _vp, _vp, _vp, _i64, _i32, _i32, _vp, _i32, _vp, _int, _vp, _i64, _vp, _i64, _vp, _int,
+                                _vp, _i32, _vp, _vp, _vp, _i64],
+    "gcnx_gcn_conv_bwd_pool_mask8": [_vp, _vp, _vp, _vp, _vp, _i64, _vp, _vp, _i32, _vp, _i64, _int, _i32, _i32, _vp, _i32, _int, _vp, _i64,
+                                     _vp, _i64, _vp, _i64, _vp, _vp, _i64, _vp, _int, _vp],
     "gcnx_gemm_dw2": [_vp, _vp, _i64, _vp, _i64, _vp, _i32, _i32, _vp, _i64, _vp, _i64, _vp, _i32, _i32, _i64, _int, _vp, _vp,
                       _i64, _f32, _vp, _vp],
     "gcnx_comm_unique_id": [C.c_char_p],
diff --git a/gcn-string_amd/gcnx/device.py b/gcn-string_amd/gcnx/device.py
--- a/gcn-string_amd/gcnx/device.py
+++ b/gcn-string_amd/gcnx/device.py
@@ -628,10 +628,21 @@
     return bool(ctx.lib.gcnx_gcn_conv_fused_ok(int(n), int(fi), int(fo), int(ldx if ldx is not None else fi)))
 
 
-def gcn_conv_fwd(ctx, a, x, w, bias, out, act="relu", s=None, wt=None, prec="f32", pool=None):
+def gcn_conv_fwd(ctx, a, x, w, bias, out, act="relu", s=None, wt=None, prec="f32", pool=None, mask8=None):
     n, fi = x.shape
     fo = w.shape[1]
-    assert a.n == n and w.shape[0] == fi and w.contiguous and out.shape == (n, fo) and (s is None or s.shape == (n, fi))
+    assert a.n == n and w.shape[0] == fi and w.contiguous and (s is None or s.shape == (n, fi))
+    assert (out is None and mask8 is not None) or out.shape == (n, fo)
+    if mask8 is not None:
+        assert mask8.dtype == np.uint8 and mask8.shape == (n, fo)
+        seg, tp, tc = pool if pool is not None else (None, None, None)
+        assert pool is None or (tp.shape == tc.shape == (pool_tile_rows(n, seg.n_graphs), fo) and tp.contiguous and tc.contiguous)
+        ctx._ck(ctx.lib.gcnx_gcn_conv_fwd_mask8(ctx.h, a.rowptr.ptr, a.colidx.ptr, _p(a.vals), _p(x), x.ld, n, fi, _p(w), fo, _p(bias),
+                                                L.ACTS[act], _p(s), s.ld if s is not None else 0, _p(out),
+                                                out.ld if out is not None else 0, _p(wt), L.PRECS[prec],
+                                                seg.ids.ptr if seg is not None else None, seg.n_graphs if seg is not None else 0,
+                                                _p(tp), _p(tc), mask8.ptr, mask8.ld))
+        return out
     if pool is None:
         ctx._ck(ctx.lib.gcnx_gcn_conv_fwd(ctx.h, a.rowptr.ptr, a.colidx.ptr, _p(a.vals), _p(x), x.ld, n, fi, _p(w), fo, _p(bias),
                                           L.ACTS[act], _p(s), s.ld if s is not None else 0, _p(out), out.ld, _p(wt), L.PRECS[prec]))
@@ -689,13 +700,17 @@
 
 
 def gcn_conv_bwd_pool(ctx, at, y2, seg, dpooled, w2, y1, dz2, dz1, db1=None, mode="sum", scratch=None, w2t=None, prec="f32",
-                      head=None):
+                      head=None, mask8=None):
+    if mask8 is not None:
+        assert mask8.dtype == np.uint8 and (y2 is None or y2.shape == mask8.shape)
+        y2 = mask8
     n, f2 = y2.shape
     f1 = w2.shape[0]
     assert at.n == n and w2.shape == (f1, f2) and w2.contiguous and y1.shape == (n, f1) and dz1.shape == (n, f1)
     assert (head is not None or dpooled.shape == (seg.n_graphs, f2)) and (dz2 is None or dz2.shape == (n, f2))
     pend = L.PendingReduce()
-    ctx._ck(ctx.lib.gcnx_gcn_conv_bwd_pool(ctx.h, at.rowptr.ptr, at.colidx.ptr, _p(at.vals), _p(y2), y2.ld, seg.ids.ptr,
+    fn = ctx.lib.gcnx_gcn_conv_bwd_pool_mask8 if mask8 is not None else ctx.lib.gcnx_gcn_conv_bwd_pool
+    ctx._ck(fn(ctx.h, at.rowptr.ptr, at.colidx.ptr, _p(at.vals), y2.ptr if mask8 is not None else _p(y2), y2.ld, seg.ids.ptr,
                                            seg.dev.ptr, seg.n_graphs, _p(dpooled), dpooled.ld if dpooled is not None else 0,
                                            L.POOLS[mode], n, f2,
                                            _p(w2t if w2t is not None else w2), f1, 1 if w2t is not None else 0, _p(y1), y1.ld, _p(dz2), dz2.ld if dz2 is not None else 0, _p(dz1), dz1.ld, _p(db1),
diff --git a/gcn-string_amd/gcnx/models.py b/gcn-string_amd/gcnx/models.py
--- a/gcn-string_amd/gcnx/models.py
+++ b/gcn-string_amd/gcnx/models.py
@@ -158,7 +158,8 @@
                       "s_order": os.environ.get("GCNX_S_ORDER", "1") != "0",
                       "buckets": os.environ.get("GCNX_COMM_BUCKETS", "1") != "0",
                       "act16": os.environ.get("GCNX_ACT16", "1") != "0",
-                      "pool_in_spmm": os.environ.get("GCNX_POOL_IN_SPMM", "1") != "0"}
+                      "pool_in_spmm": os.environ.get("GCNX_POOL_IN_SPMM", "1") != "0",
+                      "mask8": os.environ.get("GCNX_MASK8", "1") != "0"}
         self._rng = np.random.default_rng(seed)
         self.built = False
         self._bufs = None
@@ -218,6 +219,8 @@
         if self._fused(batch):
             self._bufs["s1"], self._bufs["s2"] = v("s1", n, self.f_in), v("s2", n, h)
             self._bufs["w2t"] = v("w2t", h, h)
+            if self._knob["mask8"]:
+                self._bufs["y2m8"] = v("y2m8", n, h, np.uint8)
             tr = D.pool_tile_rows(n, b)
             self._bufs["tp_part"], self._bufs["tp_cnt"] = v("tp_part", tr, h), v("tp_cnt", tr, h)
             self._bufs["pool_sum"], self._bufs["pool_cnt"] = v("pool_sum", b, h), v("pool_cnt", b, h)
@@ -228,16 +231,19 @@
         self._bufs["arg"] = v("arg", b, h, np.int32) if self.pool == "max" else None
         return self._bufs
 
-    def _forward(self, batch, bufs, with_loss, denom):
+    def _forward(self, batch, bufs, with_loss, denom, train=False):
         ctx, p, prec = self.ctx, self.p, self.prec
+        bufs["_mask8"] = None
         if self._fused(batch):
             keep = with_loss == "grads"
             late = keep and self._head_late(batch)
             D.gcn_conv_fwd(ctx, batch.a, batch.x, p["w1"], p["b1"], bufs["y1"], act="relu", s=bufs["s1"] if keep else None,
                            prec=prec)
-            D.gcn_conv_fwd(ctx, batch.a, bufs["y1"], p["w2"], p["b2"], bufs["y2"], act="relu", s=bufs["s2"] if keep else None,
-                           wt=bufs["w2t"] if keep else None, prec=prec,
-                           pool=(batch.seg, bufs["tp_part"], bufs["tp_cnt"]) if late else None)
+            m8 = bufs["y2m8"] if keep and self._knob["mask8"] else None
+            bufs["_mask8"] = m8
+            D.gcn_conv_fwd(ctx, batch.a, bufs["y1"], p["w2"], p["b2"], None if (m8 is not None and train and late) else bufs["y2"],
+                           act="relu", s=bufs["s2"] if keep else None, wt=bufs["w2t"] if keep else None, prec=prec,
+                           pool=(batch.seg, bufs["tp_part"], bufs["tp_cnt"]) if late else None, mask8=m8)
         else:
             bufs["act16"] = False
             if self._s_order() and self._act16_try(batch, with_loss):
@@ -314,7 +320,7 @@
             ha = bufs.get("_head_late")
             pend = D.gcn_conv_bwd_pool(ctx, at, bufs["y2"], batch.seg, None if ha is not None else bufs["dpooled"], p["w2"], bufs["y1"],
                                        bufs["dz"], bufs["dz2"], db1=g["b1"], mode=self.pool, scratch=self._defer_scratch(batch),
-                                       w2t=bufs["w2t"], prec=prec, head=ha)
+                                       w2t=bufs["w2t"], prec=prec, head=ha, mask8=bufs.get("_mask8"))
             if lr is None:
                 D.gemm_dw2(ctx, bufs["s1"], bufs["dz2"], g["w1"], bufs["s2"], bufs["dz"], g["w2"], prec="f32",
                            grads=self.flat_g.flat(0, self.n_params), pending=pend, leaf=ha)
@@ -490,7 +496,7 @@
         buckets = multi and self._knob["buckets"] and (fused_comm or not self.use_graph)
 
         def seq():
-            self._forward(batch, bufs, "grads", denom)
+            self._forward(batch, bufs, "grads", denom, train=_lr is not None)
             if self._backward(batch, bufs, None if multi else _lr, buckets=buckets):
                 return
             if fused_comm and not self._reduced_in_backward:
diff --git a/include/gcnx.h b/include/gcnx.h
--- a/include/gcnx.h
+++ b/include/gcnx.h
@@ -288,6 +288,11 @@
                       const float* x, int64_t ldx, int32_t n, int32_t fi, const float* w, int32_t fo,
                       const float* bias, int act, float* s, int64_t lds, float* out, int64_t ldo, float* wt_out,
                       int prec, const int32_t* node_graph, int32_t b, float* tile_part, float* tile_cnt);
+GCNX_API int gcnx_gcn_conv_fwd_mask8(gcnx_ctx* ctx, const int32_t* rowptr, const int32_t* colidx, const float* vals,
+                      const float* x, int64_t ldx, int32_t n, int32_t fi, const float* w, int32_t fo,
+                      const float* bias, int act, float* s, int64_t lds, float* out, int64_t ldo, float* wt_out,
+                      int prec, const int32_t* node_graph, int32_t b, float* tile_part, float* tile_cnt,
+                      uint8_t* mask8, int64_t ldmask8);
 typedef struct gcnx_head_args {
   const float* tile_part; const float* tile_cnt; int64_t tile_rows;
   float* pool_sum; float* pool_cnt;
@@ -299,6 +304,12 @@
 GCNX_API int64_t gcnx_gcn_conv_bwd_scratch_floats(int64_t n, int32_t f1);
 GCNX_API int gcnx_gcn_conv_bwd_pool(gcnx_ctx* ctx, const int32_t* rowptr_t, const int32_t* colidx_t, const float* vals_t,
                       const float* y2, int64_t ldy2, const int32_t* node_graph, const int32_t* graph_ptr, int32_t b,
+                      const float* dpooled, int64_t lddp, int mode, int32_t n, int32_t f2, const float* w2, int32_t f1,
+                      int w2_transposed, const float* y1, int64_t ldy1, float* dz2, int64_t lddz2, float* dz1, int64_t lddz1, float* db1,
+                      float* scratch, int64_t scratch_floats, gcnx_pending_reduce* pending, int prec,
+                      const gcnx_head_args* head);
+GCNX_API int gcnx_gcn_conv_bwd_pool_mask8(gcnx_ctx* ctx, const int32_t* rowptr_t, const int32_t* colidx_t, const float* vals_t,
+                      const uint8_t* y2_mask8, int64_t ldmask8, const int32_t* node_graph, const int32_t* graph_ptr, int32_t b,
                       const float* dpooled, int64_t lddp, int mode, int32_t n, int32_t f2, const float* w2, int32_t f1,
                       int w2_transposed, const float* y1, int64_t ldy1, float* dz2, int64_t lddz2, float* dz1, int64_t lddz1, float* db1,
                       float* scratch, int64_t scratch_floats, gcnx_pending_reduce* pending, int prec,
```

Result: faster. 342,700 graphs/s (median of 6 runs) (+2.0%).
